# Mario5Gray/Stable-Diffusion-1.5-LCM-ONNX-RKNN2

Hardware: AMD Instinct MI355X
Metric: 512x512 4-step LCM images/sec (higher is better)
Workload: dtype f16; 1 GPU; SD1.5 LCM 512x512, 4 steps, guidance 1.0 (no CFG), batch 1 per GPU, fp16 (fp32 accumulate), hipGraph replay; seeded synthetic SD1.5-architecture weights; batch_per_gpu=1, global_batch=1, image=512x512, lcm_steps=4, parallelism=independent requests x1 (RCCL broadcast of prompt embeddings only)

## Files before the change

include/lcm_hip.h:

```cpp
#ifndef LCM_HIP_H
#define LCM_HIP_H
#include <stdint.h>
#ifdef __cplusplus
extern "C" {
#endif

#define LCM_OK 0
#define LCM_EINVAL (-1)
#define LCM_ENODEV (-2)
#define LCM_EUNSUPPORTED (-3)

#define LCM_EPI_NONE 0
#define LCM_EPI_GEGLU 1
#define LCM_EPI_QUICK_GELU 2
#define LCM_EPI_GELU 3

const char* lcm_last_error(void);
int lcm_version(void);
int lcm_device_info(int dev, char* arch_buf, int buf_len, int* cu_count, uint64_t* hbm_bytes);

int lcm_gemm_f16(const void* A, int lda, const void* A2, int lda2, int K1,
                 const void* W, const void* bias, const void* rowadd, int ld_rowadd, int rows_per_batch,
                 const void* res, int ldr, void* out, int ldo,
                 int M, int N, int K, int epilogue, float out_scale,
                 int batch, int64_t strideA, int64_t strideW, int64_t strideO, int img_rows,
                 void* stats_out, int64_t stats_bytes, int* slabs_per_image, void* stream);
int64_t lcm_stats_bytes(int M, int N, int img_rows);

int lcm_set_workspace(void* ptr, int64_t bytes);
int lcm_set_stream_workspace(void* stream, void* ptr, int64_t bytes);
int lcm_stream_create(void** stream_out);
int lcm_stream_destroy(void* stream);

int lcm_set_tuning(int target_wgs, int max_splits, int min_wgs);
int lcm_set_split_policy(int max_rows_per_image, int max_parts);
int lcm_set_seg_mode(int mode);

int lcm_plan_set(int kind, int M, int N, int K, int aux, int bm, int bn, int splits, int variant);
int lcm_plan_clear(void);
int lcm_canonical_splits(int kind, int m_img, int N, int K, int aux, int ph);

int lcm_gemm_ln_f16(const void* A, int lda, const void* W, const void* ln_g, const void* ln_c, float eps,
                    void* out, int ldo, int M, int N, int K, int epilogue, int img_rows, void* stream);

int lcm_mlp_geglu_f16(const void* x, int ldx, const void* W1, const void* ln_g, const void* ln_c, float eps,
                      const void* W2, const void* b2, void* out, int ldo, int M, int C, int img_rows, void* stream);
int lcm_ln_fold_refresh(const void* W, int N, int K, const void* c_base, const void* c_delta, float alpha,
                        void* g_out, void* c_out, void* stream);

int lcm_set_persist_n(int on);

int lcm_set_kernel_variant(int variant);

int lcm_gemm_tile_config(int M, int N, int batch);

int lcm_conv3x3_f16(const void* in, const void* W, const void* bias,
                    const void* rowadd, int ld_rowadd, const void* res, void* out,
                    int B, int Hin, int Win, int Cin, int Cout, int stride, int ups,
                    void* stats_out, int64_t stats_bytes, int* slabs_per_image, void* stream);

int lcm_conv3x3_down_f16(const void* in, const void* W, const void* bias, void* out, int B, int Hin, int Win, int Cin, int Cout,
                         void* stats_out, int64_t stats_bytes, int* slabs_per_image, void* stream);

int lcm_conv3x3_gn_f16(const void* in, int C1, const void* in2, int C2, const void* gn_scale, const void* gn_shift,
                       int silu, const void* W, const void* bias, const void* rowadd, int ld_rowadd, const void* res,
                       void* out, int B, int Hin, int Win, int Cout, int ups, void* stats_out, int64_t stats_bytes,
                       int* slabs_per_image, void* stream);
int lcm_groupnorm_affine_f16(const void* x, int C1, const void* x2, int C2, const void* gamma, const void* beta,
                             void* scale_out, void* shift_out, int B, int HW, int groups, float eps, void* ws,
                             void* stream);
int lcm_set_halo_pipe_threshold(int wgs);
int lcm_set_halo_prefetch(int on);
int lcm_set_staged_epilogue(int on);
int lcm_set_conv_impl(int impl);

int lcm_conv3x3_c4_f32in(const void* in, const void* pre_w, const void* pre_b, float in_scale,
                         const void* W, const void* bias, void* out, int B, int H, int Wd, int Cout, void* stream);

int lcm_conv3x3_c4_res_f32in(const void* in, const void* W, const void* bias, const void* res, void* out, int B, int H,
                             int Wd, int Cout, void* stream);

int lcm_hint_conv_u8(const void* in, const void* W, const void* bias, void* out, int B, int H, int Wd, int Cout, int silu,
                     void* stream);
int lcm_hint_conv_f16(const void* in, const void* W, const void* bias, void* out, int B, int H, int Wd, int Cin, int Cout,
                      int stride, int silu, void* stream);

int lcm_conv3x3_smalln(const void* in, const void* W, const void* bias, void* out, void* out_f32,
                       int B, int H, int Wd, int Cin, int Cout, int mode, void* stream);
int lcm_conv3x3_smalln_gn(const void* in, const void* gn_scale, const void* gn_shift, int silu, const void* W,
                          const void* bias, void* out, void* out_f32, int B, int H, int Wd, int Cin, int Cout,
                          int mode, void* stream);

int64_t lcm_groupnorm_ws_bytes(int B, int HW, int C, int groups);
int lcm_groupnorm_f16(const void* x, int C1, const void* x2, int C2, const void* gamma, const void* beta,
                      void* out, int B, int HW, int groups, float eps, int silu, void* ws, void* stream);

int lcm_set_gn_fused_bytes(int64_t bytes);
int lcm_groupnorm_from_stats_f16(const void* x, int C1, const void* x2, int C2, const void* stats1, int P1,
                                 const void* stats2, int P2, const void* gamma, const void* beta, void* out,
                                 int B, int HW, int groups, float eps, int silu, void* ws, void* stream);

int lcm_layernorm_f16(const void* x, const void* gamma, const void* beta, void* out, int M, int C, float eps,
                      void* stream);

int lcm_attention_f16(const void* Q, int ldq, const void* K, int ldk, const void* V, int ldv, void* out, int ldo,
                      int B, int heads, int Sq, int Sk, int d, float scale, int causal, void* stream);
int lcm_set_attention_waves(int waves);
int lcm_set_attention_impl(int impl);
int lcm_set_attention_ksplit(int on);

int lcm_embed_tokens_f16(const void* ids, const void* tok_emb, const void* pos_emb, void* out, int B, int S, int D,
                         int vocab, void* stream);

int lcm_softmax_rows_f16(void* x, int rows, int n, int ld, void* stream);
int lcm_transpose_f16(const void* in, int ldi, void* out, int ldo, int R, int C, int batch,
                      int64_t stride_in, int64_t stride_out, void* stream);

int lcm_linear_smallm_f16(const void* x, int ldx, const void* W, const void* bias, const void* res, int ldr,
                          void* out, int ldo, int M, int N, int K, int silu_in, int silu_out, void* stream);
int lcm_linear_rows_f16(const void* x, int ldx, int x_rows, const void* W, const void* bias, const void* res, int ldr,
                        int res_rows, void* out, int ldo, int M, int N, int K, int silu_in, int silu_out, void* stream);

int lcm_timestep_embedding(float t, void* out, int B, int dim, void* stream);
int lcm_timestep_embedding_steps(const float* t_host, int nsteps, void* out, int B, int dim, void* stream);

int lcm_scheduler_step(const void* eps, const void* eps_uncond, float guidance, void* lat, const void* noise,
                       const float* coef6, int last, int B, int h, int w, void* stream);
// ... 109 lines not shown
```

stable-diffusion-1.5-lcm-onnx-rknn2_amd/csrc/conv_halo.hip:

```cpp
#include "igemm_common.h"

struct HaloParams {
    IgemmParams g;
    int C1;
    const float* gn_scale;
    const float* gn_shift;
    int silu;
    int H, W;
    int tiles_y, tiles_x;
    int staged_epi;
};

static __device__ __attribute__((aligned(256))) half_t g_zero_page_h[128];

template <int TH, int TW, int PH>
__device__ __forceinline__ void halo_slabs(int (&slab_of)[TH * TW / 64], int wm, int bimg, int y0, int x0, int IH, int IW, int phase) {
    constexpr int RS = 32 / TW;
    const int sx = (IW + TW - 1) / TW, sy = (IH + RS - 1) / RS;
#pragma unroll
    for (int bp = 0; bp < TH * TW / 64; ++bp) {
        const int y = y0 + wm * (TH / 2) + bp * RS;
        const int idx = (bimg * sy + y / RS) * sx + x0 / TW;
        slab_of[bp] = y < IH ? (PH ? idx * 4 + phase : idx) : -1;
    }
// ... 133 lines not shown
            }
            {
                const half_t* wsrc = wptr + (long long)tap * p.Cin + cb;
#pragma unroll
                for (int i = 0; i < RW; ++i)
                    __builtin_amdgcn_global_load_lds((const __attribute__((address_space(1))) void*)(wsrc + (long long)(32 * i) * p.K),
                                                     (__attribute__((address_space(3))) void*)(wsm + (i * 32 + wave * 8) * 128),
                                                     16, 0, 0);
            }
            __syncthreads();

            const int dy = PH ? (tap >> 1) + py : tap / 3, dx = PH ? (tap & 1) + px : tap - (tap / 3) * 3;
            const int tapoff = dy * HWD + dx;
            const char* wsr = wsm + (wn * (BN / 2)) * 128;
#pragma unroll
            for (int kk = 0; kk < 2; ++kk) {
                h8 xf[TM], wf[TN];
                const int c = kk * 4 + fq;
#pragma unroll
                for (int b = 0; b < TM; ++b) {
                    const int r = rb0 + b * RB_STEP + tapoff;
                    xf[b] = *reinterpret_cast<const h8*>(xs + r * 128 + ((c ^ (r & 7)) << 4));
                }
#pragma unroll
                for (int a = 0; a < TN; ++a) {
                    const int r = a * 16 + frow;
                    wf[a] = *reinterpret_cast<const h8*>(wsr + r * 128 + ((c ^ (r & 7)) << 4));
                }
#pragma unroll
                for (int a = 0; a < TN; ++a)
#pragma unroll
                    for (int b = 0; b < TM; ++b)
                        acc[a][b] = __builtin_amdgcn_mfma_f32_16x16x32_f16(wf[a], xf[b], acc[a][b], 0, 0, 0);
            }
        }
    }

    int m_of[TM];
#pragma unroll
    for (int b = 0; b < TM; ++b) {
        const int q = (wm * TM + b) * 16 + frow;
        const int y = y0 + q / TW, x = x0 + q % TW;
        m_of[b] = (y < IH && x < IW) ? (PH ? (bimg * hp.H + 2 * y + py) * hp.W + 2 * x + px : (bimg * hp.H + y) * hp.W + x) : -1;
    }
    int slab_of[BM / 64];
    halo_slabs<TH, TW, PH>(slab_of, wm, bimg, y0, x0, IH, IW, phase);
    static_assert(XBYTES + BN * 128 >= BM * BN * 2, "the staged epilogue lays the output tile over the halo + weight buffers");
    if constexpr (EPI != 0) {
        tile_epilogue_staged<BM, BN>(p, acc, m_of, n_base, wm, wn, fq, slab_of, smem, [&](int q) {
            const int y = y0 + q / TW, x = x0 + q % TW;
            return (y < IH && x < IW) ? (PH ? (bimg * hp.H + 2 * y + py) * hp.W + 2 * x + px : (bimg * hp.H + y) * hp.W + x) : -1;
        });
    } else {
        igemm_epilogue<BM, BN>(p, acc, m_of, n_base + wn * (BN / 2), fq, 0, slab_of);
    }
}

template <int N>
__device__ __forceinline__ void halo_wait_vmcnt() {
    asm volatile("s_waitcnt vmcnt(%0)" ::"n"(N) : "memory");
}

template <int TH, int TW, int BN, int WS, int PH, int TPS, int SEG = 0, int EPI = 0>
__global__ __launch_bounds__(256, 2) void conv_halo_pipe_kernel(HaloParams hp) {
    constexpr int NT = PH ? 4 : 9;
    constexpr int G = NT / TPS;
    static_assert(TPS == 1 || TPS == (PH ? 2 : 3), "taps per step: 1 or one kernel row");
    constexpr int BM = TH * TW;
    constexpr int TM = BM / 32, TN = BN / 32, RW = BN / 32;
    constexpr int HWD = TW + 2, HROWS = (TH + 2) * HWD, HROWS_PAD = (HROWS + 7) / 8 * 8;
    constexpr int NV = (HROWS_PAD * 8 + 255) / 256;
    constexpr int XBYTES = HROWS_PAD * 128, WBYTES = BN * 128, SBYTES = TPS * WBYTES;
    extern __shared__ __attribute__((aligned(16))) char smem[];
    char* xs0 = smem;
    char* wsm0 = smem + 2 * XBYTES;

    const IgemmParams& p = hp.g;
    const int tid = threadIdx.x, lane = tid & 63;
    const int wave = __builtin_amdgcn_readfirstlane(tid >> 6);
    const int wm = wave & 1, wn = wave >> 1;
    const int tile = xcd_remap(blockIdx.x, p.mtiles * p.ntiles);
    const int mt4 = tile / p.ntiles, nt = tile - mt4 * p.ntiles;
    const int phase = PH ? (mt4 & 3) : 0, mt = PH ? (mt4 >> 2) : mt4;
    const int py = phase >> 1, px = phase & 1;
    const int IH = PH ? p.Hin : hp.H, IW = PH ? p.Win : hp.W;
    const int per_img = hp.tiles_y * hp.tiles_x;
    const int bimg = mt / per_img, tr = mt - bimg * per_img;
    const int ty = tr / hp.tiles_x, tx = tr - ty * hp.tiles_x;
    const int y0 = ty * TH, x0 = tx * TW;
    const int n_base = nt * BN;
    const int C2 = p.Cin - hp.C1;

    int h_pix[NV];
    const int pos = tid & 7;
#pragma unroll
    for (int i = 0; i < NV; ++i) {
        const int hr = (tid + 256 * i) >> 3;
        const int hy = hr / HWD, hx = hr - hy * HWD;
        int ly = y0 - 1 + hy, lx = x0 - 1 + hx;
        const bool ok = hr < HROWS && ly >= 0 && ly < IH && lx >= 0 && lx < IW;
        if (!PH && p.ups) { ly >>= 1; lx >>= 1; }
        h_pix[i] = ok ? (bimg * p.Hin + ly) * p.Win + lx : -1;
    }
    const int w_row0 = tid >> 3;
    const int w_schunk = (pos ^ (w_row0 & 7)) * 8;
    const half_t* wptr = p.W + (PH ? (long long)phase * p.N * p.K : 0ll) + (long long)(n_base + w_row0) * p.K + w_schunk;

    const int frow = lane & 15, fq = lane >> 4;
    const int q0 = wm * TM * 16 + frow;
    const int rb0 = (q0 / TW) * HWD + (q0 % TW);
    constexpr int RB_STEP = (16 / TW) * HWD;

    f4 acc[TN][TM];
#pragma unroll
    for (int a = 0; a < TN; ++a)
#pragma unroll
        for (int b = 0; b < TM; ++b) acc[a][b] = (f4){0.f, 0.f, 0.f, 0.f};

    const int nchunks = p.Cin >> 6;
    const int c_begin = (int)((long long)blockIdx.y * nchunks / p.splits);
    const int c_end = (int)((long long)(blockIdx.y + 1) * nchunks / p.splits);
    const int T = (c_end - c_begin) * G;

    auto issue_halo = [&](int c64, int hb) {
        const int cb = c64 << 6;
        const bool second = cb >= hp.C1;
        const half_t* src_base = second ? p.A2 : p.A;
        const int src_ld = second ? C2 : hp.C1;
        const int src_c = second ? cb - hp.C1 : cb;
        char* xs = xs0 + hb * XBYTES;
#pragma unroll
        for (int i = 0; i < NV; ++i) {
            if ((wave + 4 * i) * 64 < HROWS_PAD * 8) {
                const int hr = (tid + 256 * i) >> 3;
                const half_t* src = h_pix[i] >= 0
                    ? src_base + (long long)h_pix[i] * src_ld + src_c + ((pos ^ (hr & 7)) << 3)
                    : g_zero_page_h;
                __builtin_amdgcn_global_load_lds((const __attribute__((address_space(1))) void*)src,
                                                 (__attribute__((address_space(3))) void*)(xs + (wave + 4 * i) * 1024), 16, 0, 0);
            }
        }
    };
    auto issue_w = [&](int t, int wb) {
        const int c64 = c_begin + t / G, tg = t - (t / G) * G;
#pragma unroll
        for (int tp = 0; tp < TPS; ++tp) {
            const half_t* wsrc = wptr + (long long)(tg * TPS + tp) * p.Cin + (c64 << 6);
            char* wsm = wsm0 + wb * SBYTES + tp * WBYTES;
#pragma unroll
            for (int i = 0; i < RW; ++i)
                __builtin_amdgcn_global_load_lds((const __attribute__((address_space(1))) void*)(wsrc + (long long)(32 * i) * p.K),
                                                 (__attribute__((address_space(3))) void*)(wsm + (i * 32 + wave * 8) * 128), 16, 0, 0);
        }
    };

    if (T > 0) issue_halo(c_begin, 0);
#pragma unroll
    for (int s = 0; s < WS - 1; ++s)
        if (s < T) issue_w(s, s);

    f4 tot[SEG ? TN : 1][SEG ? TM : 1];
    int part = 0, kstep = 0, plen = T;
    if constexpr (SEG) {
#pragma unroll
        for (int a = 0; a < TN; ++a)
#pragma unroll
            for (int b = 0; b < TM; ++b) tot[a][b] = (f4){0.f, 0.f, 0.f, 0.f};
        plen = (int)((long long)nchunks / p.seg_parts) * G;
    }
    int wb = 0;
    constexpr int LPS = RW * TPS;
    for (int t = 0; t < T; ++t) {
        const int chunk = t / G, tg = t - chunk * G;
        const int newer = T - 1 - t;
// ... 47 lines not shown
                    const int r = a * 16 + frow;
                    wf[buf][a] = *reinterpret_cast<const h8*>(wsr + r * 128 + ((c ^ (r & 7)) << 4));
                }
            };
            load_half(0, 0);
#pragma unroll
            for (int h = 0; h < 2 * TPS; ++h) {
                if (h + 1 < 2 * TPS) load_half(h + 1, (h + 1) & 1);
                __builtin_amdgcn_sched_barrier(0);
#pragma unroll
                for (int a = 0; a < TN; ++a)
#pragma unroll
                    for (int b = 0; b < TM; ++b)
                        acc[a][b] = __builtin_amdgcn_mfma_f32_16x16x32_f16(wf[h & 1][a], xf[h & 1][b], acc[a][b], 0, 0, 0);
                __builtin_amdgcn_sched_barrier(0);
            }
        }
        wb = (wb + 1 == WS) ? 0 : wb + 1;
        if constexpr (SEG) {
            if (++kstep == plen) {
                kstep = 0;
#pragma unroll
                for (int a = 0; a < TN; ++a)
#pragma unroll
                    for (int b = 0; b < TM; ++b) {
                        tot[a][b][0] += acc[a][b][0]; tot[a][b][1] += acc[a][b][1];
                        tot[a][b][2] += acc[a][b][2]; tot[a][b][3] += acc[a][b][3];
                        acc[a][b] = (f4){0.f, 0.f, 0.f, 0.f};
                    }
                ++part;
                plen = ((int)((long long)(part + 1) * nchunks / p.seg_parts) - (int)((long long)part * nchunks / p.seg_parts)) * G;
            }
        }
    }

    int m_of[TM];
#pragma unroll
    for (int b = 0; b < TM; ++b) {
        const int q = (wm * TM + b) * 16 + frow;
        const int y = y0 + q / TW, x = x0 + q % TW;
        m_of[b] = (y < IH && x < IW) ? (PH ? (bimg * hp.H + 2 * y + py) * hp.W + 2 * x + px : (bimg * hp.H + y) * hp.W + x) : -1;
    }
    int slab_of[BM / 64];
    halo_slabs<TH, TW, PH>(slab_of, wm, bimg, y0, x0, IH, IW, phase);
    if constexpr (EPI != 0) {
        static_assert(2 * XBYTES + WS * SBYTES >= BM * BN * 2, "staged epilogue: the ring holds the tile");
        auto row_of = [&](int q) {
            const int y = y0 + q / TW, x = x0 + q % TW;
            return (y < IH && x < IW) ? (PH ? (bimg * hp.H + 2 * y + py) * hp.W + 2 * x + px : (bimg * hp.H + y) * hp.W + x) : -1;
        };
        if constexpr (SEG) tile_epilogue_staged<BM, BN>(p, tot, m_of, n_base, wm, wn, fq, slab_of, smem, row_of);
        else tile_epilogue_staged<BM, BN>(p, acc, m_of, n_base, wm, wn, fq, slab_of, smem, row_of);
    } else {
        if constexpr (SEG) igemm_epilogue<BM, BN>(p, tot, m_of, n_base + wn * (BN / 2), fq, 0, slab_of);
        else igemm_epilogue<BM, BN>(p, acc, m_of, n_base + wn * (BN / 2), fq, 0, slab_of);
    }
}

extern void lcm_launch_splitk_reduce(IgemmParams& p, hipStream_t s);
extern float* lcm_splitk_workspace(long long* bytes, hipStream_t s);
extern void lcm_tuning(int* target_wgs, int* max_splits, int* min_wgs);
extern int lcm_split_policy(int m_img, int sp);
extern bool lcm_plan_get(int kind, int M, int N, int K, int aux, int* bm, int* bn, int* splits, int* variant);

static int g_halo_pipe_below = 768;

extern "C" int lcm_set_halo_pipe_threshold(int wgs) { g_halo_pipe_below = wgs; return LCM_OK; }
static int g_halo_prefetch = 0;
extern "C" int lcm_set_halo_prefetch(int on) { g_halo_prefetch = on ? 1 : 0; return LCM_OK; }

template <int TH, int TW, int BN, int XFORM, int PH>
static void launch_halo(HaloParams& hp, hipStream_t s, int force) {
    constexpr int HROWS_PAD = ((TH + 2) * (TW + 2) + 7) / 8 * 8;
    hp.tiles_y = ((PH ? hp.g.Hin : hp.H) + TH - 1) / TH;
    hp.tiles_x = ((PH ? hp.g.Win : hp.W) + TW - 1) / TW;
    hp.g.ntiles = hp.g.N / BN;
    dim3 grid(hp.g.mtiles * hp.g.ntiles, hp.g.splits, 1);
    if constexpr (!XFORM) if (hp.g.seg_parts > 1) {
        constexpr int TPS = (BN <= 64) ? (PH ? 2 : 3) : 1;
        constexpr int WS = 3;
        constexpr int smem = 2 * HROWS_PAD * 128 + WS * TPS * BN * 128;
        static_assert(smem <= 160 * 1024, "halo ring exceeds LDS");
        static LcmDevOnce attr_once;
        if (auto once_guard = attr_once.first()) {
            once_guard.check(hipFuncSetAttribute(reinterpret_cast<const void*>(&conv_halo_pipe_kernel<TH, TW, BN, WS, PH, TPS, 1>),
                                      hipFuncAttributeMaxDynamicSharedMemorySize, smem));
        }
        char nm[80];
        if (hp.staged_epi && hp.g.res && hp.g.splits == 1) {
            static LcmDevOnce attr_once_e;
            if (auto once_guard = attr_once_e.first()) {
                once_guard.check(hipFuncSetAttribute(reinterpret_cast<const void*>(&conv_halo_pipe_kernel<TH, TW, BN, WS, PH, TPS, 1, 1>),
                                          hipFuncAttributeMaxDynamicSharedMemorySize, smem));
            }
            snprintf(nm, sizeof(nm), "conv_halo_pipe_kernel<%d, %d, %d, %d, %d, %d, 1, 1>", TH, TW, BN, WS, PH, TPS);
            lcm_prof_start(nm, s);
            hipLaunchKernelGGL((conv_halo_pipe_kernel<TH, TW, BN, WS, PH, TPS, 1, 1>), grid, dim3(256), smem, s, hp);
            lcm_prof_stop(s);
            return;
        }
        snprintf(nm, sizeof(nm), "conv_halo_pipe_kernel<%d, %d, %d, %d, %d, %d, 1>", TH, TW, BN, WS, PH, TPS);
        lcm_prof_start(nm, s);
        hipLaunchKernelGGL((conv_halo_pipe_kernel<TH, TW, BN, WS, PH, TPS, 1>), grid, dim3(256), smem, s, hp);
        lcm_prof_stop(s);
        return;
    }
    if constexpr (!XFORM && BN <= 128) if (force == 3) {
        constexpr int TPS = PH ? 2 : 3;
// ... 38 lines not shown
    }
    const bool staged = hp.staged_epi && hp.g.splits == 1 && hp.g.res != nullptr;
    snprintf(nm, sizeof(nm), "conv_halo_kernel<%d, %d, %d, %d, %d, 0, %d>%s", TH, TW, BN, XFORM, PH, staged ? 1 : 0, hp.g.splits > 1 ? " +splitk" : "");
    lcm_prof_start(nm, s);
    if (staged) hipLaunchKernelGGL((conv_halo_kernel<TH, TW, BN, XFORM, PH, 0, 1>), grid, dim3(256), smem, s, hp);
    else hipLaunchKernelGGL((conv_halo_kernel<TH, TW, BN, XFORM, PH>), grid, dim3(256), smem, s, hp);
    lcm_prof_stop(s);
}

struct HaloPick { int bm, bn, splits; };
static HaloPick halo_pick(int B, int IH, int IW, int PHM, int TW, long long M, int N, int nchunks, int fixed_splits) {
    int target, max_splits, min_wgs;
    lcm_tuning(&target, &max_splits, &min_wgs);
    const int cand[4][2] = {{128, 128}, {128, 64}, {64, 128}, {64, 64}};
    HaloPick best = {0, 0, fixed_splits > 0 ? fixed_splits : 1};
    long long best_wgs = -1;
    for (int c = 0; c < 4; ++c) {
        const int cbm = cand[c][0], cbn = cand[c][1];
        if (N % cbn) continue;
        if (TW == 8 && cbm == 128) continue;
        const int th = cbm / TW;
        const long long mt = (long long)B * ((IH + th - 1) / th) * ((IW + TW - 1) / TW) * PHM;
        if ((long long)mt * cbm > 2ll * M && cbm == 128) continue;
        const long long tiles = mt * (N / cbn);
        int sp = fixed_splits > 0 ? fixed_splits : 1;
        if (fixed_splits < 0 && tiles < min_wgs && nchunks >= 2) {
            sp = (int)((target + tiles - 1) / tiles);
            if (sp > nchunks) sp = nchunks;
            if (sp > max_splits) sp = max_splits;
        }
        const long long wgs = tiles * sp;
        if (wgs >= min_wgs) return {cbm, cbn, sp};
        if (wgs > best_wgs) { best_wgs = wgs; best = {cbm, cbn, sp}; }
    }
    return best;
}

static inline int halo_tw(int IW) { return (IW % 16 == 0 || IW > 16) ? 16 : 8; }

int lcm_canonical_splits_halo(int m_img, int N, int K, int IH, int IW, int W, int ph, int xform) {
    const int nchunks = (K / (ph ? 4 : 9)) >> 6;
    int pbm, pbn, psp, pv;
    (void)xform;
    int sp = lcm_plan_get(2, m_img, N, K, W << 1, &pbm, &pbn, &psp, &pv)
                 ? psp : halo_pick(1, IH, IW, ph ? 4 : 1, halo_tw(IW), m_img, N, nchunks, -1).splits;
    if (sp > nchunks) sp = nchunks;
    return lcm_split_policy(m_img, sp);
}

static int g_staged_epi = 1;
extern int g_staged_epi_gemm;
extern "C" int lcm_set_staged_epilogue(int on) { g_staged_epi = (on & 1) ? 1 : 0; g_staged_epi_gemm = (on & 2) ? 1 : 0; return LCM_OK; }

int lcm_conv_halo_launch(HaloParams& hp, int B, hipStream_t s, int* slabs_per_image) {
    IgemmParams& p = hp.g;
    hp.staged_epi = g_staged_epi;
    const bool ph = p.ups == 2;
    const int IH = ph ? p.Hin : hp.H, IW = ph ? p.Win : hp.W, PHM = ph ? 4 : 1;
    const int TW = halo_tw(IW);
    long long ws_bytes = 0;
    p.ws = lcm_splitk_workspace(&ws_bytes, s);
    const int nchunks = p.Cin >> 6;
    const int m_img = p.M / B;
    p.img_rows = m_img;
    const int splits = p.ws ? lcm_canonical_splits_halo(m_img, p.N, p.K, IH, IW, hp.W, ph ? 1 : 0, hp.gn_scale ? 1 : 0) : 1;
    HaloPick hk = halo_pick(B, IH, IW, PHM, TW, p.M, p.N, nchunks, splits);
    int bm = hk.bm, bn = hk.bn, force = 0;
    {
        int pbm, pbn, psp, pv;
        if (lcm_plan_get(2, p.M, p.N, p.K, (hp.W << 1) | (hp.gn_scale ? 1 : 0), &pbm, &pbn, &psp, &pv) && p.N % pbn == 0 &&
            !(TW == 8 && pbm == 128)) {
            bm = pbm; bn = pbn;
            force = (pv >= 1 && pv <= 3) ? pv : 0;
        }
    }
    if (!bm) return 1;
    const int th = bm / TW;
    p.mtiles = B * ((IH + th - 1) / th) * ((IW + TW - 1) / TW) * PHM;
    p.splits = splits;
    p.seg_parts = 1;
    if (splits > 1 && !hp.gn_scale) {
        extern int g_seg_mode;
        int tgt, mxs, min_wgs;
        lcm_tuning(&tgt, &mxs, &min_wgs);
        if (g_seg_mode == 1 || (g_seg_mode == 0 && (long long)p.mtiles * (p.N / bn) >= min_wgs)) { p.seg_parts = splits; p.splits = 1; }
    }
    if (p.splits > 1 && (long long)p.splits * p.M * p.N * 4 > ws_bytes) {
        lcm_set_error("split-K workspace too small: %d x %d x %d fp32 slabs need %lld MB, have %lld MB "
                      "(lcm_set_workspace / LCM_SPLITK_WS_MB)", p.splits, p.M, p.N,
                      ((long long)p.splits * p.M * p.N * 4 + (1 << 20) - 1) >> 20, ws_bytes >> 20);
        return LCM_EINVAL;
    }
    p.rg_kind = TW == 16 ? 1 : 2; p.rg_ph = ph ? 1 : 0; p.rg_IH = IH; p.rg_IW = IW; p.rg_OH = hp.H; p.rg_OW = hp.W;
    if (p.stats) {
        if (p.N > 2048) p.stats = nullptr;
        else {
            if (slabs_per_image) *slabs_per_image = halo_slabs_per_image(IH, IW, TW, ph);
            LCM_STATS_FIT(p, halo_slabs_per_image(IH, IW, TW, ph), B, "conv3x3");
        }
    }
    const bool xf = hp.gn_scale != nullptr;
    if (ph && xf) return 1;
#define HALO_CASE(TH_, TW_, BN_)                                                           \
    if (th == TH_ && TW == TW_ && bn == BN_) {                                             \
        if (ph) launch_halo<TH_, TW_, BN_, 0, 1>(hp, s, force);                            \
        else if (xf) launch_halo<TH_, TW_, BN_, 1, 0>(hp, s, force);                       \
        else launch_halo<TH_, TW_, BN_, 0, 0>(hp, s, force);                               \
    } else
    HALO_CASE(8, 16, 128) HALO_CASE(8, 16, 64) HALO_CASE(4, 16, 128) HALO_CASE(4, 16, 64)
    HALO_CASE(8, 8, 128) HALO_CASE(8, 8, 64) HALO_CASE(8, 16, 160) HALO_CASE(4, 16, 160) HALO_CASE(8, 8, 160) { return 1; }
#undef HALO_CASE
    if (p.splits > 1) lcm_launch_splitk_reduce(p, s);
    return 0;
}
```

stable-diffusion-1.5-lcm-onnx-rknn2_amd/csrc/igemm.hip:

```cpp
#include "igemm_common.h"

template <int BM, int BN, int MODE, int LN = 0>
__global__ __launch_bounds__(256, 2) void igemm_kernel(IgemmParams p) {
    constexpr int RA = BM / 32, RW = BN / 32;
    constexpr int TM = BM / 32, TN = BN / 32;
    constexpr int XBYTES = BM * 128, WBYTES = BN * 128, BUF = XBYTES + WBYTES;
    extern __shared__ __attribute__((aligned(16))) char smem[];

    const int tid = threadIdx.x, lane = tid & 63, wave = tid >> 6;
    const int wm = wave & 1, wn = wave >> 1;
    const int tile = xcd_remap(blockIdx.x, p.mtiles * p.ntiles);
    const int mt = tile / p.ntiles, nt = tile - mt * p.ntiles;
    const int m_base = mt * BM, n_base = nt * BN;
    const int z = blockIdx.z;

    const half_t* __restrict__ Ab = p.A + z * p.strideA;
    const half_t* __restrict__ A2b = p.A2 ? p.A2 + z * p.strideA : nullptr;
    const half_t* __restrict__ Wb = p.W + z * p.strideW;

    const int chunk = tid & 7, row0 = tid >> 3;
    const int swz = (chunk ^ (row0 & 7)) << 4;

    bool a_ok[RA];
    long long a_off[RA];
// ... 75 lines not shown
    for (int b = 0; b < TM; ++b) { ln_s[b] = 0.f; ln_q[b] = 0.f; }

    load_tile(kt0);
    store_tile(0);
    __syncthreads();

    for (int kt = kt0; kt < kt1; ++kt) {
        const int cur = (kt - kt0) & 1;
        if (kt + 1 < kt1) load_tile(kt + 1);
        const char* xs = smem + cur * BUF + (wm * (BM / 2)) * 128;
        const char* ws = smem + cur * BUF + XBYTES + (wn * (BN / 2)) * 128;
#pragma unroll
        for (int kk = 0; kk < 2; ++kk) {
            h8 xf[TM], wf[TN];
            const int c = kk * 4 + fq;
#pragma unroll
            for (int b = 0; b < TM; ++b) {
                const int r = b * 16 + frow;
                xf[b] = *reinterpret_cast<const h8*>(xs + r * 128 + ((c ^ (r & 7)) << 4));
            }
#pragma unroll
            for (int a = 0; a < TN; ++a) {
                const int r = a * 16 + frow;
                wf[a] = *reinterpret_cast<const h8*>(ws + r * 128 + ((c ^ (r & 7)) << 4));
            }
            if constexpr (ln) {
#pragma unroll
                for (int b = 0; b < TM; ++b) ln_accum(xf[b], ln_s[b], ln_q[b]);
            }
#pragma unroll
            for (int a = 0; a < TN; ++a)
#pragma unroll
                for (int b = 0; b < TM; ++b)
                    acc[a][b] = __builtin_amdgcn_mfma_f32_16x16x32_f16(wf[a], xf[b], acc[a][b], 0, 0, 0);
        }
        if (kt + 1 < kt1) store_tile(cur ^ 1);
        __syncthreads();
    }

    int m_of[TM];
#pragma unroll
    for (int b = 0; b < TM; ++b) {
        const int m = m_base + wm * (BM / 2) + b * 16 + frow;
        m_of[b] = m < p.M ? m : -1;
    }
    int slab_of[BM / 64];
#pragma unroll
    for (int bp = 0; bp < BM / 64; ++bp) {
        const int r = m_base + wm * (BM / 2) + bp * 32;
        slab_of[bp] = r < p.M ? (r >> 5) : -1;
    }
    if constexpr (ln) {
        ln_finish<TM>(ln_s, ln_q, p.K, p.ln_eps);
        igemm_epilogue<BM, BN>(p, acc, m_of, n_base + wn * (BN / 2), fq, z, slab_of, ln_s, ln_q);
    } else {
        igemm_epilogue<BM, BN>(p, acc, m_of, n_base + wn * (BN / 2), fq, z, slab_of);
    }
}

__device__ __attribute__((aligned(256))) half_t g_zero_page[128];

template <int N>
__device__ __forceinline__ void wait_vmcnt() {
    asm volatile("s_waitcnt vmcnt(%0)" ::"n"(N) : "memory");
}

template <int BM, int BN, int MODE, int S, int LN = 0, int SEG = 0, int EPI = 0>
__global__ __launch_bounds__(256, S == 1 ? (BM + BN < 256 ? 4 : 3) : 2) void igemm2_kernel(IgemmParams p) {
    static_assert(!EPI || (MODE == 0 && !LN && !SEG && S * (BM + BN) * 128 >= BM * BN * 2), "staged epilogue: plain GEMM whose ring holds the tile");
    static_assert(!SEG || (S >= 2 && !LN), "segmented accumulation: ring variants of the plain kernel");
    constexpr int RA = BM / 32, RW = BN / 32;
    constexpr int TM = BM / 32, TN = BN / 32;
    constexpr int XBYTES = BM * 128, WBYTES = BN * 128, BUF = XBYTES + WBYTES;
    constexpr int LPT = RA + RW;
    extern __shared__ __attribute__((aligned(16))) char smem[];

    const int tid = threadIdx.x, lane = tid & 63;
    const int wave = __builtin_amdgcn_readfirstlane(tid >> 6);
    const int wm = wave & 1, wn = wave >> 1;
    const int ngroups = p.ntiles / p.n_iters;
    const int tile = xcd_remap(blockIdx.x, p.mtiles * ngroups);
    const int mt = tile / ngroups, nt0 = (tile - mt * ngroups) * p.n_iters;
    const int m_base = mt * BM;
    const int z = blockIdx.z;

    const half_t* __restrict__ Ab = p.A + z * p.strideA;
    const half_t* __restrict__ A2b = p.A2 ? p.A2 + z * p.strideA : nullptr;
    const half_t* __restrict__ Wb = p.W + z * p.strideW;

    const int pos = tid & 7, row0 = tid >> 3;
    const int schunk = (pos ^ (row0 & 7)) * 8;

    bool a_ok[RA];
    long long a_off[RA];
    int a_b[RA], a_y[RA], a_x[RA];
#pragma unroll
    for (int i = 0; i < RA; ++i) {
        const int m = m_base + row0 + 32 * i;
        a_ok[i] = m < p.M;
        if (MODE == 0) {
            a_off[i] = (long long)m;
        } else {
            const int hw = p.Hout * p.Wout;
            const int b = m / hw, rem = m - b * hw;
            const int oy = rem / p.Wout;
            a_b[i] = b; a_y[i] = oy * p.stride - 1; a_x[i] = (rem - oy * p.Wout) * p.stride - 1;
        }
    }
    const half_t* wptr = Wb + (long long)row0 * p.K + schunk;
    const int nk_all = p.K >> 6;
    const int kt0 = (int)((long long)blockIdx.y * nk_all / p.splits);
    const int kt1 = (int)((long long)(blockIdx.y + 1) * nk_all / p.splits);
    const int nkr = kt1 - kt0;
    const int T = nkr * p.n_iters;

    auto issue_tile = [&](int t, int buf) {
        const int ni = t / nkr;
        const int kt = kt0 + (t - ni * nkr);
        const int n_base_i = (nt0 + ni) * BN;
        char* xs = smem + buf * BUF + wave * 8 * 128;
        char* ws = xs + XBYTES;
        if (MODE == 0) {
            const int k0 = kt << 6;
            const bool second = (A2b != nullptr) && (k0 >= p.K1);
            const half_t* base = second ? A2b : Ab;
            const long long ld = second ? p.lda2 : p.lda;
            const int kk = (second ? k0 - p.K1 : k0) + schunk;
#pragma unroll
            for (int i = 0; i < RA; ++i) {
                const half_t* src = a_ok[i] ? base + a_off[i] * ld + kk : g_zero_page;
                __builtin_amdgcn_global_load_lds((const __attribute__((address_space(1))) void*)src,
                                                 (__attribute__((address_space(3))) void*)(xs + i * 32 * 128), 16, 0, 0);
            }
        } else {
            const int cpt = p.Cin >> 6;
            const int tap = kt / cpt;
            const int c0 = ((kt - tap * cpt) << 6) + schunk;
            const int dy = tap / 3, dx = tap - dy * 3;
            const int Hl = p.ups ? p.Hin * 2 : p.Hin, Wl = p.ups ? p.Win * 2 : p.Win;
#pragma unroll
            for (int i = 0; i < RA; ++i) {
                int iy = a_y[i] + dy, ix = a_x[i] + dx;
                const bool ok = a_ok[i] && iy >= 0 && iy < Hl && ix >= 0 && ix < Wl;
                if (p.ups) { iy >>= 1; ix >>= 1; }
                const long long off = ((long long)(a_b[i] * p.Hin + iy) * p.Win + ix) * p.Cin + c0;
                const half_t* src = ok ? Ab + off : g_zero_page;
                __builtin_amdgcn_global_load_lds((const __attribute__((address_space(1))) void*)src,
                                                 (__attribute__((address_space(3))) void*)(xs + i * 32 * 128), 16, 0, 0);
            }
        }
#pragma unroll
        for (int i = 0; i < RW; ++i) {
            const half_t* src = wptr + (long long)(n_base_i + 32 * i) * p.K + (kt << 6);
            __builtin_amdgcn_global_load_lds((const __attribute__((address_space(1))) void*)src,
                                             (__attribute__((address_space(3))) void*)(ws + i * 32 * 128), 16, 0, 0);
        }
    };

    f4 acc[TN][TM];
#pragma unroll
    for (int a = 0; a < TN; ++a)
#pragma unroll
        for (int b = 0; b < TM; ++b) acc[a][b] = (f4){0.f, 0.f, 0.f, 0.f};

    const int frow = lane & 15, fq = lane >> 4;
    constexpr bool ln = LN != 0;
    float ln_s[TM], ln_q[TM];
#pragma unroll
    for (int b = 0; b < TM; ++b) { ln_s[b] = 0.f; ln_q[b] = 0.f; }

#pragma unroll
    for (int s = 0; s < S - 1; ++s)
        if (s < T) issue_tile(s, s);
    const __attribute__((address_space(3))) float* ln_lds = nullptr;
    if constexpr (ln) {
        float* t = reinterpret_cast<float*>(smem + S * BUF);
        if (tid < BN) { t[tid] = p.ln_g[nt0 * BN + tid]; t[BN + tid] = p.ln_c[nt0 * BN + tid]; }
        __syncthreads();
        ln_lds = (const __attribute__((address_space(3))) float*)t;
    }

    f4 tot[SEG ? TN : 1][SEG ? TM : 1];
    int part = 0, nkp = nkr;
    if constexpr (SEG) {
#pragma unroll
        for (int a = 0; a < TN; ++a)
#pragma unroll
            for (int b = 0; b < TM; ++b) tot[a][b] = (f4){0.f, 0.f, 0.f, 0.f};
        nkp = (int)((long long)nk_all / p.seg_parts);
    }
    int buf = 0, kstep = 0, ni_cur = 0;
    for (int t = 0; t < T; ++t) {
        const int newer = T - 1 - t;
        if (S == 1) {
            if (t > 0) __builtin_amdgcn_s_barrier();
            issue_tile(t, 0);
            wait_vmcnt<0>();
            __builtin_amdgcn_s_barrier();
        } else {
            if (S >= 6 && newer >= 4) wait_vmcnt<(S >= 6 ? 4 : 0) * LPT>();
            else if (S >= 5 && newer >= 3) wait_vmcnt<(S >= 5 ? 3 : 0) * LPT>();
            else if (S >= 4 && newer >= 2) wait_vmcnt<(S >= 4 ? 2 : 0) * LPT>();
            else if (S >= 3 && newer >= 1) wait_vmcnt<(S >= 3 ? 1 : 0) * LPT>();
            else wait_vmcnt<0>();
            __builtin_amdgcn_s_barrier();
            if (t + S - 1 < T) issue_tile(t + S - 1, (buf + S - 1) % S);
        }

        const char* xs = smem + buf * BUF + (wm * (BM / 2)) * 128;
        const char* ws = smem + buf * BUF + XBYTES + (wn * (BN / 2)) * 128;
#pragma unroll
        for (int kk = 0; kk < 2; ++kk) {
            h8 xf[TM], wf[TN];
            const int c = kk * 4 + fq;
#pragma unroll
            for (int b = 0; b < TM; ++b) {
                const int r = b * 16 + frow;
                xf[b] = *reinterpret_cast<const h8*>(xs + r * 128 + ((c ^ (r & 7)) << 4));
            }
#pragma unroll
            for (int a = 0; a < TN; ++a) {
                const int r = a * 16 + frow;
                wf[a] = *reinterpret_cast<const h8*>(ws + r * 128 + ((c ^ (r & 7)) << 4));
            }
            if constexpr (ln) {
#pragma unroll
                for (int b = 0; b < TM; ++b) ln_accum(xf[b], ln_s[b], ln_q[b]);
            }
#pragma unroll
            for (int a = 0; a < TN; ++a)
#pragma unroll
                for (int b = 0; b < TM; ++b)
                    acc[a][b] = __builtin_amdgcn_mfma_f32_16x16x32_f16(wf[a], xf[b], acc[a][b], 0, 0, 0);
        }
        buf = (buf + 1 == S) ? 0 : buf + 1;
        if constexpr (SEG) {
            if (++kstep == nkp) {
                kstep = 0;
#pragma unroll
                for (int a = 0; a < TN; ++a)
#pragma unroll
                    for (int b = 0; b < TM; ++b) {
                        tot[a][b][0] += acc[a][b][0]; tot[a][b][1] += acc[a][b][1];
                        tot[a][b][2] += acc[a][b][2]; tot[a][b][3] += acc[a][b][3];
                        acc[a][b] = (f4){0.f, 0.f, 0.f, 0.f};
                    }
                ++part;
                nkp = (int)((long long)(part + 1) * nk_all / p.seg_parts) - (int)((long long)part * nk_all / p.seg_parts);
            }
            continue;
        }
        if (++kstep == nkr) {
            kstep = 0;
            int m_of[TM];
#pragma unroll
            for (int b = 0; b < TM; ++b) {
                const int m = m_base + wm * (BM / 2) + b * 16 + frow;
                m_of[b] = m < p.M ? m : -1;
            }
            int slab_of[BM / 64];
#pragma unroll
            for (int bp = 0; bp < BM / 64; ++bp) {
                const int r = m_base + wm * (BM / 2) + bp * 32;
                slab_of[bp] = r < p.M ? (r >> 5) : -1;
            }
            if constexpr (ln) {
                ln_finish<TM>(ln_s, ln_q, p.K, p.ln_eps);
                igemm_epilogue<BM, BN, 0, (S >= 3)>(p, acc, m_of, (nt0 + ni_cur) * BN + wn * (BN / 2), fq, z, slab_of, ln_s, ln_q, ln_lds, nt0 * BN);
            } else if constexpr (EPI != 0) {
                tile_epilogue_staged<BM, BN>(p, acc, m_of, (nt0 + ni_cur) * BN, wm, wn, fq, slab_of, smem,
                                             [&](int q) { return m_base + q < p.M ? m_base + q : -1; });
            } else {
                igemm_epilogue<BM, BN, 0, (S >= 3)>(p, acc, m_of, (nt0 + ni_cur) * BN + wn * (BN / 2), fq, z, slab_of);
            }
            ++ni_cur;
#pragma unroll
            for (int a = 0; a < TN; ++a)
#pragma unroll
                for (int b = 0; b < TM; ++b) acc[a][b] = (f4){0.f, 0.f, 0.f, 0.f};
        }
    }
    if constexpr (SEG) {
        int m_of[TM];
#pragma unroll
        for (int b = 0; b < TM; ++b) {
            const int m = m_base + wm * (BM / 2) + b * 16 + frow;
            m_of[b] = m < p.M ? m : -1;
        }
        int slab_of[BM / 64];
#pragma unroll
        for (int bp = 0; bp < BM / 64; ++bp) {
            const int r = m_base + wm * (BM / 2) + bp * 32;
            slab_of[bp] = r < p.M ? (r >> 5) : -1;
        }
        igemm_epilogue<BM, BN, 0, (S >= 3)>(p, tot, m_of, nt0 * BN + wn * (BN / 2), fq, z, slab_of);
    }
}

__device__ __forceinline__ int reduce_pixel(const IgemmParams& p, int slab, int b, int l) {
    if (p.rg_kind == 0) {
        const int m = slab * 32 + b * 16 + l;
        return m < p.M ? m : -1;
    }
    const int TW = p.rg_kind == 1 ? 16 : 8, RS = 32 / TW;
    const int sx = (p.rg_IW + TW - 1) / TW, sy = (p.rg_IH + RS - 1) / RS;
    int phase = 0;
    if (p.rg_ph) { phase = slab & 3; slab >>= 2; }
    const int bimg = slab / (sy * sx), r = slab - bimg * (sy * sx);
    const int syi = r / sx, sxi = r - syi * sx;
    const int q = b * 16 + l;
    const int y = syi * RS + q / TW, x = sxi * TW + q % TW;
    if (y >= p.rg_IH || x >= p.rg_IW) return -1;
    if (p.rg_ph) return (bimg * p.rg_OH + 2 * y + (phase >> 1)) * p.rg_OW + 2 * x + (phase & 1);
    return (bimg * p.rg_OH + y) * p.rg_OW + x;
}

#define RED_BATCH 8
__global__ __launch_bounds__(256) void splitk_reduce_kernel(IgemmParams p, int total_slabs) {
#pragma clang fp contract(off)
    const int lane = threadIdx.x & 63, ncg = p.N >> 4;
    const long long wv = (long long)blockIdx.x * 4 + (threadIdx.x >> 6);
    const int slab = (int)(wv / ncg), cg = (int)(wv - (long long)slab * ncg);
    if (slab >= total_slabs) return;
    const int l = lane & 15, fq = lane >> 4;
    const int n = cg * 16 + fq * 4;
    const long long slab_stride = (long long)p.M * p.N;
    const int splits = p.splits;
    int m[2];
    bool live[2];
    const float* src[2];
#pragma unroll
    for (int b = 0; b < 2; ++b) {
        const int mm = reduce_pixel(p, slab, b, l);
        live[b] = mm >= 0;
        m[b] = live[b] ? mm : 0;
        src[b] = p.ws + (long long)m[b] * p.N + n;
    }
    f4 t[2][RED_BATCH];
#pragma unroll
    for (int b = 0; b < 2; ++b)
#pragma unroll
        for (int k = 0; k < RED_BATCH; ++k)
            if (k < splits) t[b][k] = *reinterpret_cast<const f4*>(src[b] + k * slab_stride);
    h4 hb = {}, ha[2] = {}, hr[2] = {};
    if (p.bias) hb = *reinterpret_cast<const h4*>(p.bias + n);
    if (p.rowadd) {
#pragma unroll
        for (int b = 0; b < 2; ++b) ha[b] = *reinterpret_cast<const h4*>(p.rowadd + (long long)(m[b] / p.rows_per_batch) * p.ld_rowadd + n);
    }
    if (p.res) {
#pragma unroll
        for (int b = 0; b < 2; ++b) hr[b] = *reinterpret_cast<const h4*>(p.res + (long long)m[b] * p.ldr + n);
    }
    f4 v[2];
    for (int s0 = 0;;) {
#pragma unroll
        for (int b = 0; b < 2; ++b)
#pragma unroll
            for (int k = 0; k < RED_BATCH; ++k) {
                if (s0 + k >= splits) continue;
                if (k == 0 && s0 == 0) { v[b] = t[b][0]; continue; }
                v[b][0] += t[b][k][0]; v[b][1] += t[b][k][1]; v[b][2] += t[b][k][2]; v[b][3] += t[b][k][3];
            }
        s0 += RED_BATCH;
        if (s0 >= splits) break;
#pragma unroll
        for (int b = 0; b < 2; ++b)
#pragma unroll
            for (int k = 0; k < RED_BATCH; ++k)
                if (s0 + k < splits) t[b][k] = *reinterpret_cast<const f4*>(src[b] + (s0 + k) * slab_stride);
    }
    const f4 bias4 = {(float)hb[0], (float)hb[1], (float)hb[2], (float)hb[3]};
    float ssum[4] = {0.f, 0.f, 0.f, 0.f}, ssq[4] = {0.f, 0.f, 0.f, 0.f};
#pragma unroll
    for (int b = 0; b < 2; ++b) {
        f4 w = v[b];
        w[0] += bias4[0]; w[1] += bias4[1]; w[2] += bias4[2]; w[3] += bias4[3];
        if (p.rowadd) { w[0] += (float)ha[b][0]; w[1] += (float)ha[b][1]; w[2] += (float)ha[b][2]; w[3] += (float)ha[b][3]; }
        w[0] *= p.out_scale; w[1] *= p.out_scale; w[2] *= p.out_scale; w[3] *= p.out_scale;
        if (p.res) { w[0] += (float)hr[b][0]; w[1] += (float)hr[b][1]; w[2] += (float)hr[b][2]; w[3] += (float)hr[b][3]; }
        h4 o = {(half_t)w[0], (half_t)w[1], (half_t)w[2], (half_t)w[3]};
        if (live[b]) {
            *reinterpret_cast<h4*>(p.out + (long long)m[b] * p.ldo + n) = o;
#pragma unroll
            for (int j = 0; j < 4; ++j) { const float f = (float)o[j]; ssum[j] += f; ssq[j] += f * f; }
        }
    }
    if (p.stats) {
row16_sum8(ssum, ssq);
        if (l == 0) {
            float* dst = p.stats + ((long long)slab * p.N + n) * 2;
            *reinterpret_cast<f4*>(dst) = (f4){ssum[0], ssq[0], ssum[1], ssq[1]};
            *reinterpret_cast<f4*>(dst + 4) = (f4){ssum[2], ssq[2], ssum[3], ssq[3]};
        }
    }
}

#include <map>
#include <mutex>
static float* g_ws[16] = {};
static long long g_ws_bytes[16] = {};
struct StreamWs { float* ptr; long long bytes; };
static std::map<hipStream_t, StreamWs> g_stream_ws;
static std::mutex g_ws_mu;

extern "C" int lcm_set_workspace(void* ptr, int64_t bytes) {
    int dev = 0;
    if (hipGetDevice(&dev) != hipSuccess || dev < 0 || dev >= 16) { lcm_set_error("set_workspace: no device"); return LCM_ENODEV; }
    std::lock_guard<std::mutex> lk(g_ws_mu);
    g_ws[dev] = (float*)ptr;
    g_ws_bytes[dev] = ptr ? bytes : 0;
    return LCM_OK;
}

extern "C" int lcm_set_stream_workspace(void* stream, void* ptr, int64_t bytes) {
    std::lock_guard<std::mutex> lk(g_ws_mu);
    auto it = g_stream_ws.find((hipStream_t)stream);
    if (ptr && bytes > 0) {
        if (it != g_stream_ws.end() && it->second.ptr != (float*)ptr) {
            lcm_set_error("set_stream_workspace: stream %p already carries the workspace %p of another owner (new %p): "
                          "every lane needs a stream of its own", stream, (void*)it->second.ptr, ptr);
            return LCM_EINVAL;
        }
        g_stream_ws[(hipStream_t)stream] = StreamWs{(float*)ptr, (long long)bytes};
    } else if (it != g_stream_ws.end() && (!ptr || it->second.ptr == (float*)ptr)) {
        g_stream_ws.erase(it);
    }
    return LCM_OK;
}

float* lcm_splitk_workspace(long long* bytes, hipStream_t s) {
    std::lock_guard<std::mutex> lk(g_ws_mu);
    auto it = g_stream_ws.find(s);
    if (it != g_stream_ws.end()) { *bytes = it->second.bytes; return it->second.ptr; }
    int dev = 0;
    (void)hipGetDevice(&dev);
    if (dev < 0 || dev >= 16) { *bytes = 0; return nullptr; }
    *bytes = g_ws[dev] ? g_ws_bytes[dev] : 0;
    return g_ws[dev];
}
int lcm_total_slabs(const IgemmParams& p) {
    if (p.rg_kind == 0) return (p.M + 31) / 32;
    const int TW = p.rg_kind == 1 ? 16 : 8, RS = 32 / TW;
    const int per_img = ((p.rg_IH + RS - 1) / RS) * ((p.rg_IW + TW - 1) / TW) * (p.rg_ph ? 4 : 1);
    return (p.M / (p.rg_OH * p.rg_OW)) * per_img;
}

void lcm_launch_splitk_reduce(IgemmParams& p, hipStream_t s) {
    const int total = lcm_total_slabs(p);
    const long long waves = (long long)total * (p.N >> 4);
    hipLaunchKernelGGL(splitk_reduce_kernel, dim3((unsigned)((waves + 3) / 4)), dim3(256), 0, s, p, total);
}

#include <tuple>
struct PlanVal { int bm, bn, splits, variant; };
static std::map<std::tuple<int, int, int, int, int>, PlanVal> g_plans;
static std::mutex g_plans_mu;

extern "C" int lcm_plan_set(int kind, int M, int N, int K, int aux, int bm, int bn, int splits, int variant) {
    if (!((bm == 128 || bm == 64) && (bn == 128 || bn == 64 || bn == 160) && splits >= 1 && splits <= 64 && variant >= -1 && variant <= 4)) {
        lcm_set_error("plan_set: bad plan %dx%d splits %d variant %d", bm, bn, splits, variant);
        return LCM_EINVAL;
    }
    std::lock_guard<std::mutex> lk(g_plans_mu);
    g_plans[std::make_tuple(kind, M, N, K, aux)] = PlanVal{bm, bn, splits, variant};
    return LCM_OK;
}

extern "C" int lcm_plan_clear(void) {
    std::lock_guard<std::mutex> lk(g_plans_mu);
    g_plans.clear();
    return LCM_OK;
}

bool lcm_plan_get(int kind, int M, int N, int K, int aux, int* bm, int* bn, int* splits, int* variant) {
    std::lock_guard<std::mutex> lk(g_plans_mu);
    auto it = g_plans.find(std::make_tuple(kind, M, N, K, aux));
    if (it == g_plans.end()) return false;
    *bm = it->second.bm; *bn = it->second.bn; *splits = it->second.splits; *variant = it->second.variant;
    return true;
}

struct TilePick { int bm, bn, splits; };
static int g_target_wgs = 384, g_max_splits = 16, g_min_wgs = 256;
static int g_split_max_rows = 4096, g_split_cap = 8;
int g_seg_mode = 0;
static int g_variant = -1;

void lcm_tuning(int* target_wgs, int* max_splits, int* min_wgs) {
    *target_wgs = g_target_wgs; *max_splits = g_max_splits; *min_wgs = g_min_wgs;
}

static int g_conv_impl = 1;

extern "C" int lcm_set_conv_impl(int impl) {
    if (impl != 0 && impl != 1) { lcm_set_error("conv_impl: %d", impl); return LCM_EINVAL; }
    g_conv_impl = impl;
    return LCM_OK;
}

extern "C" int lcm_set_kernel_variant(int variant) {
    if (variant < -1 || variant > 6) { lcm_set_error("kernel_variant: %d", variant); return LCM_EINVAL; }
    g_variant = variant;
    return LCM_OK;
// ... 120 lines not shown
        int ni = p.ntiles;
        while (ni > 1 && (p.ntiles % ni != 0 || (long long)p.mtiles * (p.ntiles / ni) < 384)) --ni;
        p.n_iters = ni;
    }
    dim3 grid(p.mtiles * (p.ntiles / p.n_iters), splits, batch);
    if (variant == 5) variant = (BM + BN <= 128) ? 4 : -1;
    if (variant == 6) variant = (BM + BN <= 128) ? 6 : -1;
    if (variant < 0) {
        const long long wgs = (long long)grid.x * grid.y * grid.z;
        variant = (wgs >= 1024 && p.n_iters == 1) ? 1 : ((BM + BN <= 128) ? 4 : 2);
    }
    if (p.n_iters > 1 && variant == 1) variant = 2;
    if (variant == 4 && BM + BN > 192) variant = 3;
    if constexpr (!LN) if (p.seg_parts > 1) {
        if (variant < 2 || variant > 4) variant = (BM + BN <= 128) ? 4 : 2;
        if (variant == 2) launch_v2<BM, BN, MODE, 2, 0, 1>(p, grid, s);
        else if (variant == 3) launch_v2<BM, BN, MODE, 3, 0, 1>(p, grid, s);
        else if constexpr (BM + BN <= 192) launch_v2<BM, BN, MODE, 4, 0, 1>(p, grid, s);
        else launch_v2<BM, BN, MODE, 3, 0, 1>(p, grid, s);
        LCM_CHECK_LAUNCH("igemm");
        return LCM_OK;
    }
    if (variant == 0) {
        const int smem = 2 * (BM + BN) * 128;
        static LcmDevOnce attr_once;
        if (auto once_guard = attr_once.first()) {
            once_guard.check(hipFuncSetAttribute(reinterpret_cast<const void*>(&igemm_kernel<BM, BN, MODE, LN>),
                                      hipFuncAttributeMaxDynamicSharedMemorySize, smem));
        }
        char nm[64];
        snprintf(nm, sizeof(nm), "igemm_kernel<%d, %d, %d, %d>%s", BM, BN, MODE, LN, p.splits > 1 ? " +splitk" : "");
        lcm_prof_start(nm, s);
        hipLaunchKernelGGL((igemm_kernel<BM, BN, MODE, LN>), grid, dim3(256), smem, s, p);
        lcm_prof_stop(s);
    } else if (variant == 1) {
        launch_v2<BM, BN, MODE, 1, LN>(p, grid, s);
    } else if (variant == 2) {
        launch_v2<BM, BN, MODE, 2, LN>(p, grid, s);
    } else if (variant == 3) {
        launch_v2<BM, BN, MODE, 3, LN>(p, grid, s);
    } else if (variant == 6) {
        if constexpr (BM + BN <= 128) launch_v2<BM, BN, MODE, 6, LN>(p, grid, s);
    } else {
        launch_v2<BM, BN, MODE, 4, LN>(p, grid, s);
    }
    LCM_CHECK_LAUNCH("igemm");
    if (splits > 1) {
        lcm_launch_splitk_reduce(p, s);
        LCM_CHECK_LAUNCH("splitk_reduce");
    }
    return LCM_OK;
}

template <int MODE>
static int launch_igemm(IgemmParams& p, int batch, hipStream_t s, int img_rows, bool allow_split, bool want_stats,
                        int* slabs_per_image) {
    long long wsb = 0;
    p.ws = lcm_splitk_workspace(&wsb, s);
    if (img_rows <= 0 || p.M % img_rows) img_rows = p.M;
    p.img_rows = img_rows;
    int splits = 1;
    if (allow_split && p.ws && p.epi == 0 && batch == 1) {
        splits = canonical_splits_gemm(MODE, img_rows, p.N, p.K);
    }
    TilePick t = pick_tile(p.M, p.N, p.K, batch, splits);
    int variant = -1, pbm, pbn, psp, pv;
    if (lcm_plan_get(MODE, p.M, p.N, p.K, batch, &pbm, &pbn, &psp, &pv) && p.N % pbn == 0 &&
        !(pbn == 160 && (MODE != 0 || p.epi == 1)) && !(pbm == 128 && p.M < 128)) {
        t.bm = pbm; t.bn = pbn;
        variant = pv;
    }
    if (slabs_per_image) *slabs_per_image = 0;
    p.stats = want_stats ? p.stats : nullptr;
    p.rg_kind = 0;
    if (p.stats) {
        const bool ok = p.epi == 0 && batch == 1 && p.N <= 2048 && img_rows % 32 == 0;
        if (ok && slabs_per_image) *slabs_per_image = img_rows / 32;
        if (!ok) p.stats = nullptr;
        else LCM_STATS_FIT(p, img_rows / 32, p.M / img_rows, "gemm");
    }
    p.seg_parts = 1;
    if (splits > 1) {
        const long long tiles = (long long)((p.M + t.bm - 1) / t.bm) * (p.N / t.bn) * batch;
        if (g_seg_mode == 1 || (g_seg_mode == 0 && tiles >= g_min_wgs)) { p.seg_parts = splits; splits = 1; }
    }
    if (splits > 1 && (long long)splits * p.M * p.N * 4 > wsb) {
        lcm_set_error("split-K workspace too small: %d x %d x %d fp32 slabs need %lld MB, have %lld MB "
                      "(lcm_set_workspace / LCM_SPLITK_WS_MB)", splits, p.M, p.N,
                      ((long long)splits * p.M * p.N * 4 + (1 << 20) - 1) >> 20, wsb >> 20);
        return LCM_EINVAL;
    }
    const int code = t.bm * 1000 + t.bn;
    if constexpr (MODE == 0) if (p.ln_g) {
        switch (code) {
            case 128128: return launch_cfg<128, 128, 0, 1>(p, batch, splits, variant, s);
            case 128064: return launch_cfg<128, 64, 0, 1>(p, batch, splits, variant, s);
            case 64128: return launch_cfg<64, 128, 0, 1>(p, batch, splits, variant, s);
            case 128160: return launch_cfg<128, 160, 0, 1>(p, batch, splits, variant, s);
            case 64160: return launch_cfg<64, 160, 0, 1>(p, batch, splits, variant, s);
            default: return launch_cfg<64, 64, 0, 1>(p, batch, splits, variant, s);
        }
    }
    switch (code) {
        case 128128: return launch_cfg<128, 128, MODE>(p, batch, splits, variant, s);
        case 128064: return launch_cfg<128, 64, MODE>(p, batch, splits, variant, s);
        case 64128: return launch_cfg<64, 128, MODE>(p, batch, splits, variant, s);
        case 128160: if constexpr (MODE == 0) return launch_cfg<128, 160, MODE>(p, batch, splits, variant, s);
        case 64160: if constexpr (MODE == 0) return launch_cfg<64, 160, MODE>(p, batch, splits, variant, s);
        default: return launch_cfg<64, 64, MODE>(p, batch, splits, variant, s);
    }
}

extern "C" int lcm_gemm_f16(const void* A, int lda, const void* A2, int lda2, int K1,
                            const void* W, const void* bias, const void* rowadd, int ld_rowadd, int rows_per_batch,
                            const void* res, int ldr, void* out, int ldo,
                            int M, int N, int K, int epilogue, float out_scale,
                            int batch, int64_t strideA, int64_t strideW, int64_t strideO, int img_rows,
                            void* stats_out, int64_t stats_bytes, int* slabs_per_image, void* stream) {
    LCM_REQUIRE(A && W && out, "gemm: null pointer");
    LCM_REQUIRE(M > 0 && N > 0 && K > 0 && batch > 0, "gemm: bad shape M=%d N=%d K=%d batch=%d", M, N, K, batch);
    LCM_REQUIRE(K % 64 == 0, "gemm: K=%d must be a multiple of 64", K);
    LCM_REQUIRE(N % 64 == 0, "gemm: N=%d must be a multiple of 64", N);
    LCM_REQUIRE(lda % 8 == 0 && ldo % 4 == 0, "gemm: lda=%d (%%8) / ldo=%d (%%4) misaligned", lda, ldo);
    if (A2) LCM_REQUIRE(K1 > 0 && K1 < K && K1 % 64 == 0 && lda2 % 8 == 0, "gemm: bad split K1=%d lda2=%d", K1, lda2);
    if (res) LCM_REQUIRE(ldr % 4 == 0, "gemm: ldr=%d misaligned", ldr);
    if (rowadd) LCM_REQUIRE(rows_per_batch > 0 && ld_rowadd % 4 == 0, "gemm: bad rowadd");
    LCM_REQUIRE(epilogue >= 0 && epilogue <= 3, "gemm: unknown epilogue %d", epilogue);
    if (epilogue == 1) LCM_REQUIRE(!rowadd && !res && !A2, "gemm: GEGLU epilogue takes bias only");
    IgemmParams p = {};
    p.A = (const half_t*)A; p.A2 = (const half_t*)A2; p.W = (const half_t*)W;
    p.bias = (const half_t*)bias; p.rowadd = (const half_t*)rowadd; p.res = (const half_t*)res;
    p.out = (half_t*)out;
    p.M = M; p.N = N; p.K = K; p.lda = lda; p.lda2 = lda2; p.K1 = A2 ? K1 : K;
    p.ldo = ldo; p.ldr = ldr; p.ld_rowadd = ld_rowadd; p.rows_per_batch = rows_per_batch > 0 ? rows_per_batch : 1;
    p.epi = epilogue; p.out_scale = out_scale;
    p.strideA = strideA; p.strideW = strideW; p.strideO = strideO;
    p.stats = (float*)stats_out; p.stats_cap = stats_bytes;
    LCM_REQUIRE(!stats_out || slabs_per_image, "gemm: stats_out needs slabs_per_image");
    const bool allow_split = batch == 1 && strideA == 0 && strideW == 0 && strideO == 0;
    return launch_igemm<0>(p, batch, (hipStream_t)stream, img_rows, allow_split, stats_out != nullptr, slabs_per_image);
}

extern "C" int lcm_gemm_ln_f16(const void* A, int lda, const void* W, const void* ln_g, const void* ln_c, float eps,
                               void* out, int ldo, int M, int N, int K, int epilogue, int img_rows, void* stream) {
    LCM_REQUIRE(A && W && out && ln_g && ln_c, "gemm_ln: null pointer");
    LCM_REQUIRE(M > 0 && N > 0 && K > 0, "gemm_ln: bad shape M=%d N=%d K=%d", M, N, K);
    LCM_REQUIRE(K % 64 == 0 && N % 64 == 0, "gemm_ln: N=%d K=%d must be multiples of 64", N, K);
    LCM_REQUIRE(lda % 8 == 0 && ldo % 4 == 0, "gemm_ln: lda=%d (%%8) / ldo=%d (%%4) misaligned", lda, ldo);
    LCM_REQUIRE(epilogue == 0 || epilogue == 1, "gemm_ln: epilogue %d (0 = none, 1 = GEGLU)", epilogue);
    IgemmParams p = {};
    p.A = (const half_t*)A; p.W = (const half_t*)W; p.out = (half_t*)out;
    p.M = M; p.N = N; p.K = K; p.lda = lda; p.K1 = K; p.ldo = ldo; p.rows_per_batch = 1;
    p.epi = epilogue; p.out_scale = 1.0f;
    p.ln_g = (const float*)ln_g; p.ln_c = (const float*)ln_c; p.ln_eps = eps;
    return launch_igemm<0>(p, 1, (hipStream_t)stream, img_rows, false, false, nullptr);
}

extern "C" int64_t lcm_stats_bytes(int M, int N, int img_rows) {
    if (M <= 0 || N <= 0) return 0;
    if (img_rows <= 0 || M % img_rows) img_rows = M;
    const long long per_img = (img_rows / 16 > 256 ? img_rows / 16 : 256) + 64;
    return (int64_t)(per_img * (M / img_rows) * N * 2 * (long long)sizeof(float));
}

struct HaloParams {
    IgemmParams g;
    int C1;
    const float* gn_scale;
    const float* gn_shift;
    int silu;
    int H, W;
    int tiles_y, tiles_x;
    int staged_epi;
};
int lcm_conv_halo_launch(HaloParams& hp, int B, hipStream_t s, int* slabs_per_image);

extern "C" int lcm_conv3x3_gn_f16(const void* in, int C1, const void* in2, int C2, const void* gn_scale,
                                  const void* gn_shift, int silu, const void* W, const void* bias, const void* rowadd,
                                  int ld_rowadd, const void* res, void* out, int B, int Hin, int Win, int Cout, int ups,
                                  void* stats_out, int64_t stats_bytes, int* slabs_per_image, void* stream) {
    LCM_REQUIRE(in && W && out, "conv3x3_gn: null pointer");
    if (!in2) C2 = 0;
    const int Cin = C1 + C2;
    LCM_REQUIRE(B > 0 && Hin > 0 && Win > 0, "conv3x3_gn: bad shape");
    LCM_REQUIRE(C1 % 64 == 0 && C2 % 64 == 0 && Cout % 64 == 0, "conv3x3_gn: C1=%d C2=%d Cout=%d must be multiples of 64", C1, C2, Cout);
    LCM_REQUIRE((gn_scale == nullptr) == (gn_shift == nullptr), "conv3x3_gn: scale/shift must come together");
    if (rowadd) LCM_REQUIRE(ld_rowadd % 4 == 0, "conv3x3_gn: ld_rowadd misaligned");
    HaloParams hp = {};
    IgemmParams& p = hp.g;
    p.A = (const half_t*)in; p.A2 = (const half_t*)in2; p.W = (const half_t*)W; p.bias = (const half_t*)bias;
    p.rowadd = (const half_t*)rowadd; p.res = (const half_t*)res; p.out = (half_t*)out;
    const int crop_h = (ups >> 2) & 1, crop_w = (ups >> 3) & 1;
    ups &= 3;
    LCM_REQUIRE(ups >= 0 && ups <= 2 && !(ups == 2 && gn_scale), "conv3x3_gn: ups=%d (2 = phase-packed weights, no fused GroupNorm)", ups);
    LCM_REQUIRE(ups == 1 || (!crop_h && !crop_w), "conv3x3_gn: an odd output size needs ups=1 (plain 3x3 weights), got ups=%d", ups);
    p.Hin = Hin; p.Win = Win; p.Cin = Cin; p.stride = 1; p.ups = ups;
    hp.H = ups ? 2 * Hin - crop_h : Hin; hp.W = ups ? 2 * Win - crop_w : Win;
    p.Hout = hp.H; p.Wout = hp.W;
    p.M = B * hp.H * hp.W; p.N = Cout; p.K = (ups == 2 ? 4 : 9) * Cin;
    p.ldo = Cout; p.ldr = Cout; p.ld_rowadd = ld_rowadd; p.rows_per_batch = hp.H * hp.W;
    p.epi = 0; p.out_scale = 1.0f; p.splits = 1;
    hp.C1 = C1; hp.gn_scale = (const float*)gn_scale; hp.gn_shift = (const float*)gn_shift; hp.silu = silu;
    p.stats = (float*)stats_out; p.stats_cap = stats_bytes;
    LCM_REQUIRE(!stats_out || slabs_per_image, "conv3x3_gn: stats_out needs slabs_per_image");
    if (slabs_per_image) *slabs_per_image = 0;
    const int hrc = lcm_conv_halo_launch(hp, B, (hipStream_t)stream, slabs_per_image);
    if (hrc < 0) return hrc;
    if (hrc != 0) {
        lcm_set_error("conv3x3_gn: no tile configuration for B=%d %dx%d Cin=%d Cout=%d", B, hp.H, hp.W, Cin, Cout);
        return LCM_EINVAL;
    }
    LCM_CHECK_LAUNCH("conv_halo");
    return LCM_OK;
}

extern "C" int lcm_conv3x3_f16(const void* in, const void* W, const void* bias,
                               const void* rowadd, int ld_rowadd, const void* res, void* out,
                               int B, int Hin, int Win, int Cin, int Cout, int stride, int ups,
                               void* stats_out, int64_t stats_bytes, int* slabs_per_image, void* stream) {
    LCM_REQUIRE(in && W && out, "conv3x3: null pointer");
    LCM_REQUIRE(B > 0 && Hin > 0 && Win > 0, "conv3x3: bad shape");
    LCM_REQUIRE(Cin % 64 == 0 && Cout % 64 == 0, "conv3x3: Cin=%d Cout=%d must be multiples of 64", Cin, Cout);
    LCM_REQUIRE(stride == 1 || stride == 2, "conv3x3: stride %d", stride);
    LCM_REQUIRE(!(ups && stride != 1), "conv3x3: upsample needs stride 1");
    if (rowadd) LCM_REQUIRE(ld_rowadd % 4 == 0, "conv3x3: ld_rowadd misaligned");
    if (stride == 1 && (g_conv_impl == 1 || (ups & 3) == 2 || (ups & 12)))
        return lcm_conv3x3_gn_f16(in, Cin, nullptr, 0, nullptr, nullptr, 0, W, bias, rowadd, ld_rowadd, res, out, B, Hin, Win,
                                  Cout, ups, stats_out, stats_bytes, slabs_per_image, stream);
    const int Hl = ups ? 2 * Hin : Hin, Wl = ups ? 2 * Win : Win;
    IgemmParams p = {};
    p.A = (const half_t*)in; p.W = (const half_t*)W; p.bias = (const half_t*)bias;
    p.rowadd = (const half_t*)rowadd; p.res = (const half_t*)res; p.out = (half_t*)out;
    p.Hin = Hin; p.Win = Win; p.Cin = Cin; p.stride = stride; p.ups = ups;
    p.Hout = (Hl + 2 - 3) / stride + 1; p.Wout = (Wl + 2 - 3) / stride + 1;
    p.M = B * p.Hout * p.Wout; p.N = Cout; p.K = 9 * Cin;
    p.ldo = Cout; p.ldr = Cout; p.ld_rowadd = ld_rowadd; p.rows_per_batch = p.Hout * p.Wout;
    p.epi = 0; p.out_scale = 1.0f;
    p.stats = (float*)stats_out; p.stats_cap = stats_bytes;
    LCM_REQUIRE(!stats_out || slabs_per_image, "conv3x3: stats_out needs slabs_per_image");
    return launch_igemm<1>(p, 1, (hipStream_t)stream, p.Hout * p.Wout, true, stats_out != nullptr, slabs_per_image);
}
```

stable-diffusion-1.5-lcm-onnx-rknn2_amd/csrc/igemm_common.h:

```cpp
#pragma once
#include "common.h"

struct IgemmParams {
    const half_t* A;
    const half_t* A2;
    const half_t* W;
    const half_t* bias;
    const half_t* rowadd;
    const half_t* res;
    half_t* out;
    int M, N, K;
    int lda, lda2, K1;
    int ldo, ldr, ld_rowadd, rows_per_batch;
    int epi;
    float out_scale;
    long long strideA, strideW, strideO;
    int Hin, Win, Cin, Hout, Wout, stride, ups;
    int mtiles, ntiles;
    int splits;
    float* ws;
    float* stats;
    int reduce_rows;
    int rg_kind, rg_ph, rg_IH, rg_IW, rg_OH, rg_OW;
    int seg_parts;
// ... 14 lines not shown
            return LCM_EINVAL;                                                                                             \
        }                                                                                                                  \
    } while (0)

__device__ __forceinline__ int xcd_remap(int bid, int nwg) {
    const int q = nwg >> 3, r = nwg & 7, xcd = bid & 7;
    return (xcd < r ? xcd * (q + 1) : r * (q + 1) + (xcd - r) * q) + (bid >> 3);
}

__device__ __forceinline__ void ln_accum(const h8& x, float& s, float& q) {
    const h2 one = {(half_t)1.0f, (half_t)1.0f};
#pragma unroll
    for (int i = 0; i < 4; ++i) {
        const h2 pr = {x[2 * i], x[2 * i + 1]};
        s = __builtin_amdgcn_fdot2(pr, one, s, false);
        q = __builtin_amdgcn_fdot2(pr, pr, q, false);
    }
}
template <int TM>
__device__ __forceinline__ void ln_finish(float (&s)[TM], float (&q)[TM], int K, float eps) {
    const float inv = 1.0f / (float)K;
#pragma unroll
    for (int b = 0; b < TM; ++b) {
        float ss = s[b], qq = q[b];
        ss += __shfl_xor(ss, 16, 64); qq += __shfl_xor(qq, 16, 64);
        ss += __shfl_xor(ss, 32, 64); qq += __shfl_xor(qq, 32, 64);
        const float mean = ss * inv;
        s[b] = mean;
        q[b] = rsqrtf(fmaxf(__builtin_fmaf(-mean, mean, qq * inv), 0.f) + eps);
    }
}

__device__ __forceinline__ h4 geglu_ln_quad(f4 x, f4 g, float ln_r, float ln_mu, const f4& gx, const f4& cx, const f4& gg, const f4& cg) {
#pragma clang fp contract(off)
    h4 o;
#pragma unroll
    for (int j = 0; j < 4; ++j) {
        const float xv = __builtin_fmaf(ln_r, __builtin_fmaf(-ln_mu, gx[j], x[j]), cx[j]);
        const float gv = __builtin_fmaf(ln_r, __builtin_fmaf(-ln_mu, gg[j], g[j]), cg[j]);
        o[j] = (half_t)(xv * gelu_erf_f(gv));
    }
    return o;
}

__device__ __forceinline__ int geglu_store_col(int P, int fq) { return 32 * (P >> 1) + 8 * fq + 4 * (P & 1); }

template <int CH>
__device__ __forceinline__ int stage_pos(int c, int q) { return (c + q) % CH; }
template <int CH>
__device__ __forceinline__ int stage_src(int cpos, int q) { return (cpos + CH - q % CH) % CH; }

template <int BM, int BN, int STAGED = 0, int BATCHED = 0>
__device__ __forceinline__ void igemm_epilogue(const IgemmParams& p, f4 (&acc)[BN / 32][BM / 32], const int (&m_of)[BM / 32],
                                               int n_wave, int fq, int z, const int (&slab_of)[BM / 64],
                                               const float* ln_mu = nullptr, const float* ln_r = nullptr,
                                               const __attribute__((address_space(3))) float* ln_lds = nullptr, int n_tile0 = 0,
                                               char* stage = nullptr, int q_wave = 0, int nl_wave = 0) {
#pragma clang fp contract(off)
    constexpr int TM = BM / 32, TN = BN / 32;
    if (p.splits > 1) {
        float* __restrict__ wsb = p.ws + (long long)blockIdx.y * p.M * p.N;
#pragma unroll
        for (int b = 0; b < TM; ++b) {
            const int m = m_of[b];
            if (m < 0) continue;
#pragma unroll
            for (int a = 0; a < TN; ++a) {
                const int n = n_wave + a * 16 + fq * 4;
                *reinterpret_cast<f4*>(wsb + (long long)m * p.N + n) = acc[a][b];
            }
        }
        return;
    }

    half_t* __restrict__ outb = p.out + z * p.strideO;
    const bool do_stats = p.stats != nullptr && p.epi == 0;
    const int lane = threadIdx.x & 63;
    if (p.epi != 1) {
        constexpr bool PRE = BATCHED != 0 && STAGED == 0;
        constexpr int NB = PRE ? (TM * TN <= 4 ? TN : 1) : 1;
        h4 pre_bias[NB], pre_add[NB][PRE ? TM : 1], pre_res[NB][PRE ? TM : 1];
        int mc[TM];
#pragma unroll
        for (int b = 0; b < TM; ++b) mc[b] = m_of[b] < 0 ? 0 : m_of[b];
#pragma unroll
        for (int a = 0; a < TN; ++a) {
            const int n = n_wave + a * 16 + fq * 4;
            if constexpr (PRE) {
                if (a % NB == 0) {
                    if (p.bias) {
#pragma unroll
                        for (int i = 0; i < NB; ++i) pre_bias[i] = *reinterpret_cast<const h4*>(p.bias + n + i * 16);
                    }
                    if (p.rowadd) {
#pragma unroll
                        for (int b = 0; b < TM; ++b) {
                            const half_t* row = p.rowadd + (long long)(mc[b] / p.rows_per_batch) * p.ld_rowadd + n;
#pragma unroll
                            for (int i = 0; i < NB; ++i) pre_add[i][b] = *reinterpret_cast<const h4*>(row + i * 16);
                        }
                    }
                    if (p.res) {
#pragma unroll
                        for (int b = 0; b < TM; ++b) {
                            const half_t* row = p.res + (long long)mc[b] * p.ldr + n;
#pragma unroll
                            for (int i = 0; i < NB; ++i) pre_res[i][b] = *reinterpret_cast<const h4*>(row + i * 16);
                        }
                    }
                }
            }
            f4 bias4 = {0.f, 0.f, 0.f, 0.f};
            if (p.bias) {
                h4 t;
// ... 79 lines not shown
            if (ln_mu) {
                if (ln_lds) {
                    const __attribute__((address_space(3))) float* gl = ln_lds + (n - n_tile0);
                    gx = *reinterpret_cast<const __attribute__((address_space(3))) f4*>(gl);
                    cx = *reinterpret_cast<const __attribute__((address_space(3))) f4*>(gl + BN);
                    gg = *reinterpret_cast<const __attribute__((address_space(3))) f4*>(gl + 16);
                    cg = *reinterpret_cast<const __attribute__((address_space(3))) f4*>(gl + BN + 16);
                } else {
                    gx = *reinterpret_cast<const f4*>(p.ln_g + n); cx = *reinterpret_cast<const f4*>(p.ln_c + n);
                    gg = *reinterpret_cast<const f4*>(p.ln_g + n + 16); cg = *reinterpret_cast<const f4*>(p.ln_c + n + 16);
                }
            }
#pragma unroll
            for (int b = 0; b < TM; ++b) {
                const int m = m_of[b];
                if (m < 0) continue;
                h4 o;
                if (ln_mu) {
                    o = geglu_ln_quad(acc[a][b], acc[a + 1][b], ln_r[b], ln_mu[b], gx, cx, gg, cg);
                } else {
                    const f4 x = acc[a][b], g = acc[a + 1][b];
#pragma unroll
                    for (int j = 0; j < 4; ++j) o[j] = (half_t)((x[j] + bx[j]) * gelu_erf_f(g[j] + bg[j]));
                }
                *reinterpret_cast<h4*>(outb + (long long)m * p.ldo + nout) = o;
            }
        }
    }
}

static __device__ __attribute__((aligned(256))) half_t g_zero_page_epi[128];

template <int BM, int BN, class RowOf>
__device__ __forceinline__ void tile_epilogue_staged(const IgemmParams& p, f4 (&acc)[BN / 32][BM / 32], const int (&m_of)[BM / 32],
                                                     int n_base, int wm, int wn, int fq, const int (&slab_of)[BM / 64],
                                                     char* stage, RowOf row_of) {
    constexpr int CH = BN / 8, PIECES = BM * CH, NV = (PIECES + 255) / 256;
    const int tid = threadIdx.x;
    const int wave = __builtin_amdgcn_readfirstlane(tid >> 6);
    __syncthreads();
    if (p.res) {
#pragma unroll
        for (int i = 0; i < NV; ++i) {
            if ((wave + 4 * i) * 64 < PIECES) {
                const int v = tid + 256 * i, q = v / CH, cpos = v - q * CH;
                const int m = row_of(q);
                const half_t* src = m >= 0 ? p.res + (long long)m * p.ldr + n_base + stage_src<CH>(cpos, q) * 8 : g_zero_page_epi;
                __builtin_amdgcn_global_load_lds((const __attribute__((address_space(1))) void*)src,
                                                 (__attribute__((address_space(3))) void*)(stage + (wave + 4 * i) * 1024), 16, 0, 0);
            }
        }
        __syncthreads();
    }
    igemm_epilogue<BM, BN, 1>(p, acc, m_of, n_base + wn * (BN / 2), fq, 0, slab_of, nullptr, nullptr, nullptr, 0,
                              stage, wm * (BM / 2), wn * (BN / 2));
    __syncthreads();
#pragma unroll
    for (int i = 0; i < NV; ++i) {
        const int v = tid + 256 * i;
        if (v < PIECES) {
            const int q = v / CH, cpos = v - q * CH;
            const int m = row_of(q);
            if (m >= 0) *reinterpret_cast<h8*>(p.out + (long long)m * p.ldo + n_base + stage_src<CH>(cpos, q) * 8) =
                            *reinterpret_cast<const h8*>(stage + v * 16);
        }
    }
}
```

stable-diffusion-1.5-lcm-onnx-rknn2_amd/csrc/mlp_fused.hip:

```cpp
#include "igemm_common.h"
#include <stdlib.h>

struct MlpParams {
    IgemmParams g;
    const half_t* X;
    int ldx;
    const half_t* W1;
    const float* ln_g;
    const float* ln_c;
    float eps;
    const half_t* W2;
};

template <int N>
__device__ __forceinline__ void mlp_wait_vmcnt() {
    asm volatile("s_waitcnt vmcnt(%0)" ::"n"(N) : "memory");
}

template <int C, int ABL = 0>
__global__ __launch_bounds__(512, 2) void mlp_geglu_kernel(MlpParams p) {
    static_assert(C % 64 == 0 && C <= 320, "register budget: C/16 accumulator tiles + C/32 x 2 operand fragments per lane");
    constexpr int KT1 = C / 64;
    constexpr int F = 4 * C;
    constexpr int NCH = F / 64;
// ... 141 lines not shown
            const f4 gg = *reinterpret_cast<const __attribute__((address_space(3))) f4*>(ln_lds + n + 16);
            const f4 cg = *reinterpret_cast<const __attribute__((address_space(3))) f4*>(ln_lds + 8 * C + n + 16);
#pragma unroll
            for (int b = 0; b < 2; ++b) {
                h4 o;
                if (ABL == 1) { for (int e = 0; e < 4; ++e) o[e] = (half_t)(acc1[2 * qq][b][e] * acc1[2 * qq + 1][b][e] + gx[e] + cg[e]); }
                else o = geglu_ln_quad(acc1[2 * qq][b], acc1[2 * qq + 1][b], ln_r[b], ln_mu[b], gx, cx, gg, cg);
#pragma unroll
                for (int e = 0; e < 4; ++e) gf[b][4 * qq + e] = o[e];
            }
        }
        *reinterpret_cast<h8*>(gmine) = gf[0];
        *reinterpret_cast<h8*>(gmine + 1024) = gf[1];
        __builtin_amdgcn_sched_barrier(0);
#pragma unroll
        for (int i = 0; i < 4; ++i) cur[i] = frag(w2s, i, 0);
        if (last) mlp_wait_vmcnt<0>(); else mlp_wait_vmcnt<3 * LPT1>();
        asm volatile("s_waitcnt lgkmcnt(0)" ::: "memory");
        __builtin_amdgcn_s_barrier();
        __builtin_amdgcn_sched_barrier(0);
        {
            const h8 q0 = *reinterpret_cast<const h8*>(gcell), q1 = *reinterpret_cast<const h8*>(gcell + 1024);
            const h8 r0 = *reinterpret_cast<const h8*>(gcell + 2048), r1 = *reinterpret_cast<const h8*>(gcell + 3072);
            h8 wv[2 * TN2 + 4];
#pragma unroll
            for (int i = 0; i < 4; ++i) wv[i] = cur[i];
#pragma unroll
            for (int i = 4; i < 2 * TN2; ++i) wv[i] = frag(w2s, i % TN2, i / TN2);
            if (!last) {
#pragma unroll
                for (int i = 0; i < 4; ++i) wv[2 * TN2 + i] = frag(w1tile(0), i, 0);
            }
#pragma unroll
            for (int i = 0; i < 2 * TN2; ++i) {
                const int a2 = i % TN2;
                if (ABL == 4) { acc2[a2][0][0] += (float)wv[i][0] * (float)q0[1]; acc2[a2][1][1] += (float)wv[i][1] * (float)r1[0]; continue; }
                acc2[a2][0] = __builtin_amdgcn_mfma_f32_16x16x32_f16(wv[i], i < TN2 ? q0 : r0, acc2[a2][0], 0, 0, 0);
                acc2[a2][1] = __builtin_amdgcn_mfma_f32_16x16x32_f16(wv[i], i < TN2 ? q1 : r1, acc2[a2][1], 0, 0, 0);
            }
            __builtin_amdgcn_sched_group_barrier(0x100, 4, 0);
#pragma unroll
            for (int i = 0; i < 2 * TN2; ++i) {
                __builtin_amdgcn_sched_group_barrier(0x008, 2, 0);
                __builtin_amdgcn_sched_group_barrier(0x100, 1, 0);
            }
            if (!last) {
#pragma unroll
                for (int i = 0; i < 4; ++i) cur[i] = wv[2 * TN2 + i];
            }
        }
    }
    __builtin_amdgcn_sched_barrier(0);
    const int slab_of[1] = {-1};
    igemm_epilogue<64, C>(p.g, acc2, m_of, (C / 2) * wn, fq, 0, slab_of);
}

extern "C" int lcm_canonical_splits(int kind, int m_img, int N, int K, int aux, int ph);

extern "C" int lcm_mlp_geglu_f16(const void* x, int ldx, const void* W1, const void* ln_g, const void* ln_c, float eps,
                                 const void* W2, const void* b2, void* out, int ldo, int M, int C, int img_rows, void* stream) {
    LCM_REQUIRE(x && W1 && ln_g && ln_c && W2 && out, "mlp_geglu: null pointer");
    LCM_REQUIRE(M > 0, "mlp_geglu: bad M=%d", M);
    LCM_REQUIRE(C == 320, "mlp_geglu: C=%d (register budget of the kernel: C = 320 only)", C);
    LCM_REQUIRE(ldx % 8 == 0 && ldo % 4 == 0, "mlp_geglu: ldx=%d (%%8) / ldo=%d (%%4) misaligned", ldx, ldo);
    if (img_rows <= 0 || M % img_rows) img_rows = M;
    const int parts = lcm_canonical_splits(0, img_rows, C, 4 * C, 1, 0);
    LCM_REQUIRE(parts == 1, "mlp_geglu: the canonical K partition of ff.net.2 at %d rows per image has %d parts; the fused "
                "kernel accumulates one (use the two-launch form)", img_rows, parts);
    MlpParams p = {};
    p.X = (const half_t*)x; p.ldx = ldx; p.W1 = (const half_t*)W1; p.ln_g = (const float*)ln_g; p.ln_c = (const float*)ln_c;
    p.eps = eps; p.W2 = (const half_t*)W2;
    p.g.out = (half_t*)out; p.g.ldo = ldo; p.g.bias = (const half_t*)b2; p.g.res = (const half_t*)x; p.g.ldr = ldx;
    p.g.M = M; p.g.N = C; p.g.K = 4 * C; p.g.splits = 1; p.g.epi = 0; p.g.out_scale = 1.0f; p.g.rows_per_batch = 1;
    constexpr int smem = 5 * 128 * 128 + 320 * 128 + 2 * 8 * 320 * 4 + 16 * 1024;
    static LcmDevOnce attr_once;
    if (auto once_guard = attr_once.first()) {
        once_guard.check(hipFuncSetAttribute(reinterpret_cast<const void*>(&mlp_geglu_kernel<320>),
                                             hipFuncAttributeMaxDynamicSharedMemorySize, smem));
    }
    hipStream_t s = (hipStream_t)stream;
    lcm_prof_start("mlp_geglu_kernel<320>", s);
    static const int abl = getenv("LCM_MLP_ABLATE") ? atoi(getenv("LCM_MLP_ABLATE")) : 0;
    const dim3 grid((M + 127) / 128);
    if (abl) {
        auto set = [&](const void* f) { (void)hipFuncSetAttribute(f, hipFuncAttributeMaxDynamicSharedMemorySize, smem); };
        if (abl == 1) { set((const void*)&mlp_geglu_kernel<320, 1>); hipLaunchKernelGGL((mlp_geglu_kernel<320, 1>), grid, dim3(512), smem, s, p); }
        else if (abl == 2) { set((const void*)&mlp_geglu_kernel<320, 2>); hipLaunchKernelGGL((mlp_geglu_kernel<320, 2>), grid, dim3(512), smem, s, p); }
        else if (abl == 3) { set((const void*)&mlp_geglu_kernel<320, 3>); hipLaunchKernelGGL((mlp_geglu_kernel<320, 3>), grid, dim3(512), smem, s, p); }
        else { set((const void*)&mlp_geglu_kernel<320, 4>); hipLaunchKernelGGL((mlp_geglu_kernel<320, 4>), grid, dim3(512), smem, s, p); }
    } else
    hipLaunchKernelGGL((mlp_geglu_kernel<320>), grid, dim3(512), smem, s, p);
    lcm_prof_stop(s);
    LCM_CHECK_LAUNCH("mlp_geglu");
    return LCM_OK;
}
```

stable-diffusion-1.5-lcm-onnx-rknn2_amd/csrc/vae_enc.hip:

```cpp
#include "igemm_common.h"

__global__ __launch_bounds__(256) void vae_enc_conv_in_u8_kernel(const uint8_t* __restrict__ in, const half_t* __restrict__ W,
                                                                 const half_t* __restrict__ bias, half_t* __restrict__ out,
                                                                 int B, int H, int Wd, int Cout) {
#pragma clang fp contract(off)
    extern __shared__ __attribute__((aligned(16))) char smem[];
    for (int i = threadIdx.x; i < Cout * 8; i += 256) {
        const int sg = i / Cout, co = i - sg * Cout;
        half_t e[8];
#pragma unroll
        for (int j = 0; j < 8; ++j) {
            const int k = sg * 8 + j;
            e[j] = k < 54 ? W[co * 27 + (k >= 27 ? k - 27 : k)] : (half_t)0;
        }
        *reinterpret_cast<h8*>(smem + (sg * Cout + co) * 16) = (h8){e[0], e[1], e[2], e[3], e[4], e[5], e[6], e[7]};
    }
    __syncthreads();
    const int lane = threadIdx.x & 63, wave = threadIdx.x >> 6;
    const int n = lane & 15, q = lane >> 4;
    const long long npix = (long long)B * H * Wd;
    const int ntile = (int)((npix + 15) >> 4), plane = H * Wd;
    for (int t = blockIdx.x * 4 + wave; t < ntile; t += gridDim.x * 4) {
        const long long pix = (long long)t * 16 + n;
        const bool live = pix < npix;
// ... 171 lines not shown
    };

    f4 acc[TN][TM];
#pragma unroll
    for (int a = 0; a < TN; ++a)
#pragma unroll
        for (int b = 0; b < TM; ++b) acc[a][b] = (f4){0.f, 0.f, 0.f, 0.f};

    const int frow = lane & 15, fq = lane >> 4;
    load_tile(kt0);
    store_tile(0);
    __syncthreads();
    for (int kt = kt0; kt < kt1; ++kt) {
        const int cur = (kt - kt0) & 1;
        if (kt + 1 < kt1) load_tile(kt + 1);
        const char* xs = smem + cur * BUF + (wm * (BM / 2)) * 128;
        const char* ws = smem + cur * BUF + XBYTES + (wn * (BN / 2)) * 128;
#pragma unroll
        for (int kk = 0; kk < 2; ++kk) {
            h8 xf[TM], wf[TN];
            const int c = kk * 4 + fq;
#pragma unroll
            for (int b = 0; b < TM; ++b) {
                const int r = b * 16 + frow;
                xf[b] = *reinterpret_cast<const h8*>(xs + r * 128 + ((c ^ (r & 7)) << 4));
            }
#pragma unroll
            for (int a = 0; a < TN; ++a) {
                const int r = a * 16 + frow;
                wf[a] = *reinterpret_cast<const h8*>(ws + r * 128 + ((c ^ (r & 7)) << 4));
            }
#pragma unroll
            for (int a = 0; a < TN; ++a)
#pragma unroll
                for (int b = 0; b < TM; ++b)
                    acc[a][b] = __builtin_amdgcn_mfma_f32_16x16x32_f16(wf[a], xf[b], acc[a][b], 0, 0, 0);
        }
        if (kt + 1 < kt1) store_tile(cur ^ 1);
        __syncthreads();
    }

    int m_of[TM];
#pragma unroll
    for (int b = 0; b < TM; ++b) {
        const int m = m_base + wm * (BM / 2) + b * 16 + frow;
        m_of[b] = m < p.M ? m : -1;
    }
    int slab_of[BM / 64];
#pragma unroll
    for (int bp = 0; bp < BM / 64; ++bp) {
        const int r = m_base + wm * (BM / 2) + bp * 32;
        slab_of[bp] = r < p.M ? (r >> 5) : -1;
    }
    igemm_epilogue<BM, BN>(p, acc, m_of, n_base + wn * (BN / 2), fq, 0, slab_of);
}

template <int BM, int BN>
static int launch_conv_down(IgemmParams& p, hipStream_t s) {
    constexpr int smem = 2 * (BM + BN) * 128;
    static LcmDevOnce attr_once;
    if (auto once_guard = attr_once.first()) {
        once_guard.check(hipFuncSetAttribute(reinterpret_cast<const void*>(&conv_down_kernel<BM, BN>),
                                             hipFuncAttributeMaxDynamicSharedMemorySize, smem));
    }
    p.mtiles = (p.M + BM - 1) / BM;
    p.ntiles = p.N / BN;
    char nm[64];
    snprintf(nm, sizeof(nm), "conv_down_kernel<%d, %d>%s", BM, BN, p.splits > 1 ? " +splitk" : "");
    lcm_prof_start(nm, s);
    hipLaunchKernelGGL((conv_down_kernel<BM, BN>), dim3(p.mtiles * p.ntiles, p.splits, 1), dim3(256), smem, s, p);
    lcm_prof_stop(s);
    LCM_CHECK_LAUNCH("conv3x3_down");
    if (p.splits > 1) {
        lcm_launch_splitk_reduce(p, s);
        LCM_CHECK_LAUNCH("splitk_reduce");
    }
    return LCM_OK;
}

extern "C" int lcm_conv3x3_down_f16(const void* in, const void* W, const void* bias, void* out, int B, int Hin, int Win, int Cin,
                                    int Cout, void* stats_out, int64_t stats_bytes, int* slabs_per_image, void* stream) {
    LCM_REQUIRE(in && W && out, "conv3x3_down: null pointer");
    LCM_REQUIRE(B > 0 && Hin >= 2 && Win >= 2, "conv3x3_down: bad shape B=%d %dx%d (each side >= 2)", B, Hin, Win);
    LCM_REQUIRE(Cin % 64 == 0 && Cout % 64 == 0 && Cin > 0 && Cout > 0, "conv3x3_down: Cin=%d Cout=%d must be multiples of 64", Cin, Cout);
    LCM_REQUIRE((long long)B * Hin * Win < (1ll << 30), "conv3x3_down: input too large");
    LCM_REQUIRE(!stats_out || slabs_per_image, "conv3x3_down: stats_out needs slabs_per_image");
    hipStream_t s = (hipStream_t)stream;
    IgemmParams p = {};
    p.A = (const half_t*)in; p.W = (const half_t*)W; p.bias = (const half_t*)bias; p.out = (half_t*)out;
    p.Hin = Hin; p.Win = Win; p.Cin = Cin; p.stride = 2; p.ups = 0;
    p.Hout = (Hin + 1 - 3) / 2 + 1; p.Wout = (Win + 1 - 3) / 2 + 1;
    const int img_rows = p.Hout * p.Wout;
    p.M = B * img_rows; p.N = Cout; p.K = 9 * Cin;
    p.ldo = Cout; p.ldr = Cout; p.rows_per_batch = img_rows; p.img_rows = img_rows;
    p.epi = 0; p.out_scale = 1.0f; p.n_iters = 1; p.seg_parts = 1; p.rg_kind = 0;
    long long wsb = 0;
    p.ws = lcm_splitk_workspace(&wsb, s);
    p.splits = 1;
    if (p.ws) {
        const int sp = lcm_canonical_splits(1, img_rows, p.N, p.K, 1, 0);
        if (sp < 0) return sp;
        p.splits = sp;
    }
    if (p.splits > 1 && (long long)p.splits * p.M * p.N * 4 > wsb) {
        lcm_set_error("conv3x3_down: split-K workspace too small: %d x %d x %d fp32 slabs need %lld MB, have %lld MB "
                      "(lcm_set_workspace / LCM_SPLITK_WS_MB)", p.splits, p.M, p.N,
                      ((long long)p.splits * p.M * p.N * 4 + (1 << 20) - 1) >> 20, wsb >> 20);
// ... 16 lines not shown
```

stable-diffusion-1.5-lcm-onnx-rknn2_amd/lib.py:

```python
from __future__ import annotations

import ctypes as C
import os
import subprocess

_HERE = os.path.dirname(os.path.abspath(__file__))
LIB_PATH = os.path.join(_HERE, "liblcmhip.so")


class LcmHipError(RuntimeError):
    pass


def build(verbose: bool = False) -> str:
    r = subprocess.run(["make", "-C", os.path.join(_HERE, "csrc"), "-j8"], capture_output=True, text=True)
    if verbose or r.returncode != 0:
        print(r.stdout[-4000:], r.stderr[-4000:])
    if r.returncode != 0:
        raise LcmHipError("building liblcmhip.so failed")
    return LIB_PATH


_vp, _i, _f, _i64 = C.c_void_p, C.c_int, C.c_float, C.c_int64

# ... 29 lines not shown
    "lcm_conv3x3_down_f16": [_vp, _vp, _vp, _vp, _i, _i, _i, _i, _i, _vp, _i64, C.POINTER(_i), _vp],
    "lcm_vae_enc_conv_in_u8": [_vp, _vp, _vp, _vp, _i, _i, _i, _i, _vp],
    "lcm_vae_posterior_renoise": [_vp, _vp, _vp, _vp, _vp, _vp, _f, _f, _f, _vp, _vp, _vp, _i, _i, _i, _i, _vp],
    "lcm_scheduler_step_handover": [_vp, _vp, _f, _vp, _vp, _vp, C.POINTER(C.c_float), _f, _f, _i, _i, _i, _i, _i, _vp],
    "lcm_inpaint_mask_prepare": [_vp, _vp, _i, _vp, _vp, _vp, _i, _i, _i, _vp],
    "lcm_scheduler_step_inpaint": [_vp, _vp, _f, _vp, _vp, _vp, _vp, _vp, C.POINTER(C.c_float), _i, _f, _f, _i, _i, _i, _i, _i, _vp],
    "lcm_inpaint_composite_rgb8": [_vp, _vp, _vp, _i, _i, _i, _vp],
    "lcm_canny_classes_u8": [_vp, _vp, _i, _i, _i, _i, _i, _vp],
    "lcm_canny_link": [_vp, _vp, _vp, C.c_longlong, _i, _i, _i, _vp],
    "lcm_canny_rgb8": [_vp, _vp, _vp, C.c_longlong, _i, _i, _i, _f, _f, _vp],
    "lcm_invert_u8": [_vp, _vp, C.c_longlong, _vp],
    "lcm_resize_lanczos_u8": [_vp, C.c_longlong, _i, _i, _i, _i, _i, _i, _i, _i, _i, _vp, C.c_longlong, _vp, C.c_longlong, _vp],
    "lcm_resize_tables": [_i, _i, _i, _i, _vp, C.c_longlong],
    "lcm_resize_plan_tables": [_i] * 8 + [_vp, C.c_longlong],
    "lcm_resize_span": [_i, _i, _i, _i, C.POINTER(_i), C.POINTER(_i)],
    "lcm_resize_ksize": [_i, _i],
    "lcm_resize_passes": [_i, _i, _i, _i],
    "lcm_resize_max_span": [_i, _i, _i, _i, _i],
    "lcm_png_encode_rgb8": [_vp, _i, _i, C.c_longlong, _i, _vp, C.c_longlong, C.POINTER(C.c_longlong)],
    "lcm_stream_create": [C.POINTER(_vp)],
    "lcm_stream_destroy": [_vp],
    "lcm_graph_begin": [_vp],
    "lcm_graph_end": [_vp, C.POINTER(_vp)],
    "lcm_graph_launch": [_vp, _vp],
    "lcm_graph_destroy": [_vp],
    "lcm_gemm_tile_config": [_i, _i, _i],
    "lcm_debug_spin": [_i, _vp],
    "lcm_debug_grid_barrier": [_i, _i, _vp, _vp],
    "lcm_axpy_f16": [_vp, _vp, _f, _vp, _i64, _vp],
    "lcm_vae_blend_f32": [_vp, _i, _i, _vp, _i, _i, _i, _i, _i, _vp],
    "lcm_vae_place_tile": [_vp, _i, _i, _vp, _vp, _i, _i, _i, _i, _i, _i, _i, _vp],
    "lcm_profile_begin": [_i],
    "lcm_profile_end": [C.c_char_p, _i64],
    "lcm_set_workspace": [_vp, _i64],
    "lcm_set_stream_workspace": [_vp, _vp, _i64],
    "lcm_set_tuning": [_i, _i, _i],
    "lcm_set_split_policy": [_i, _i],
    "lcm_set_seg_mode": [_i],
    "lcm_set_attention_waves": [_i],
    "lcm_set_attention_impl": [_i],
    "lcm_set_attention_ksplit": [_i],
    "lcm_set_kernel_variant": [_i],
    "lcm_set_conv_impl": [_i],
    "lcm_set_persist_n": [_i],
    "lcm_set_halo_pipe_threshold": [_i],
    "lcm_set_halo_prefetch": [_i],
    "lcm_set_staged_epilogue": [_i],
    "lcm_set_gn_fused_bytes": [_i64],
    "lcm_plan_set": [_i] * 9,
    "lcm_plan_clear": [],
    "lcm_canonical_splits": [_i] * 6,
    "lcm_conv3x3_gn_f16": [_vp, _i, _vp, _i, _vp, _vp, _i, _vp, _vp, _vp, _i, _vp, _vp, _i, _i, _i, _i, _i, _vp, _i64,
                           C.POINTER(_i), _vp],
    "lcm_groupnorm_affine_f16": [_vp, _i, _vp, _i, _vp, _vp, _vp, _vp, _i, _i, _i, _f, _vp, _vp],
    "lcm_device_info": [_i, C.c_char_p, _i, C.POINTER(_i), C.POINTER(C.c_uint64)],
    "lcm_sr_conv1": [_vp, _i, _i, _i, _i, _i, _i, _vp, _vp, _vp, _vp],
    "lcm_sr_conv3x3": [_vp, _i, _i, _i, _i, _vp, _vp, _vp, _vp],
    "lcm_sr_conv4_shuffle": [_vp, _i, _i, _i, _i, _i, _i, _vp, _vp, _i, _vp, _vp],
    "lcm_sr_chroma_h": [_vp, _i, _i, _i, _vp, _vp],
    "lcm_sr_merge": [_vp, _vp, _i, _i, _i, _vp, _vp],
    "lcm_jpeg_quant_tables": [_i, _vp],
    "lcm_jpeg_dct_rgb8": [_vp, _i, _i, C.c_longlong, _i, _vp, C.c_longlong, _vp],
    "lcm_jpeg_encode_coefs": [_vp, _i, _i, _i, _i, _vp, C.c_longlong, C.POINTER(C.c_longlong)],
    "lcm_jpeg_dec_info": [_vp, C.c_longlong, _vp],
    "lcm_jpeg_dec_coefs": [_vp, C.c_longlong, _i, _vp, C.c_longlong],
    "lcm_jpeg_idct_rgb8": [_vp, C.c_longlong, _vp, _vp, C.c_longlong, _vp, C.c_longlong, _vp],
}
EXPORTS = tuple(sorted(list(_SIGS) + ["lcm_last_error", "lcm_version", "lcm_groupnorm_ws_bytes", "lcm_stats_bytes", "lcm_png_bound",
                              "lcm_canny_ws_bytes", "lcm_jpeg_coef_bytes", "lcm_jpeg_bound", "lcm_resize_ws_bytes",
                              "lcm_resize_table_bytes", "lcm_resize_plan_table_bytes"]))

EUNSUPPORTED = -3


class JpegInfo(C.Structure):
    _fields_ = [("width", _i), ("height", _i), ("ncomp", _i), ("sampling", _i), ("restart_interval", _i), ("mcus_x", _i),
                ("mcus_y", _i), ("blocks_per_mcu", _i), ("coefs_bytes", C.c_longlong), ("work_bytes", C.c_longlong),
                ("qt", C.c_uint8 * 192)]


_lib = None


def load():
    global _lib
    if _lib is not None:
        return _lib
    if not os.path.exists(LIB_PATH):
        raise LcmHipError(f"{LIB_PATH} not built: run __graft_entry__.build() (make -C csrc); "
                          "there is no CPU fallback for the HIP path")
    import torch
    lib = C.CDLL(LIB_PATH)
    for name, sig in _SIGS.items():
        fn = getattr(lib, name)
        fn.argtypes = sig
        fn.restype = _i
    lib.lcm_last_error.restype = C.c_char_p
    lib.lcm_last_error.argtypes = []
    lib.lcm_version.restype = _i
    lib.lcm_groupnorm_ws_bytes.restype = _i64
    lib.lcm_groupnorm_ws_bytes.argtypes = [_i, _i, _i, _i]
    lib.lcm_stats_bytes.restype = _i64
    lib.lcm_png_bound.restype = C.c_longlong
    lib.lcm_png_bound.argtypes = [_i, _i, _i]
    lib.lcm_stats_bytes.argtypes = [_i, _i, _i]
    lib.lcm_canny_ws_bytes.restype = C.c_longlong
# ... 53 lines not shown
```

stable-diffusion-1.5-lcm-onnx-rknn2_amd/model.py:

```python
from __future__ import annotations

import torch

from . import ops
from .config import TEXT_SEQ_LEN, depth_at, heads_at, unet_config, vae_config
from .packing import pack_conv1x1, pack_conv3x3, pack_conv3x3_up2, pack_ff2_cols, pack_geglu


import os

VAE_FLASH_ATTN = os.environ.get("LCM_VAE_FLASH_ATTN", "1") != "0"
FUSE_GN_MIN_BYTES = int(os.environ.get("LCM_FUSE_GN_MIN_BYTES", str(64 << 20)))


def _fuse_gn_into_conv(M, Cin, Cout):
    if Cin % 64 or Cout % 64:
        return False
    ntiles = Cout // 160 if Cout % 160 == 0 else -(-Cout // 128)
    return M * Cin * 2 >= FUSE_GN_MIN_BYTES and ntiles <= (4 if Cout % 160 == 0 else 3)


class _Buffers:
    def __init__(self, device):
        self.device = device
# ... 37 lines not shown
        st = self._stats.get(key)
        if st is None:
            st = ops.Stats(torch.zeros(ops.stats_floats(M, C, hw), dtype=torch.float32, device=self.device))
            self._stats[key] = st
        return st

    def norm(self, x, gamma, beta, out, B, HW, C1, *, x_st=None, x2=None, C2=0, x2_st=None, eps=1e-5, silu=True):
        C = C1 + C2
        ws = self.gn_ws(B, HW, C)
        if x_st is not None and x_st.P > 0 and (x2 is None or (x2_st is not None and x2_st.P > 0)):
            ops.groupnorm_from_stats(x, gamma, beta, out, B, HW, C1, x_st, ws, x2=x2, C2=C2, st2=x2_st, eps=eps, silu=silu)
        else:
            ops.groupnorm(x, gamma, beta, out, B, HW, C1, ws, x2=x2, C2=C2, eps=eps, silu=silu)
        return out

    def _norm_conv_out(self, x, norm, st, hn, out, B, H, W, ch, cout, eps, *, mode, out_f32=None):
        wt = self.w
        if st is not None and st.P > 0 and ch % 64 == 0:
            sc_t, sh_t = ops.groupnorm_tables_from_stats(wt[norm + ".g"], wt[norm + ".b"], B, H * W, ch, st, self.gn_ws(B, H * W, ch), eps=eps)
            ops.conv3x3_smalln(x, wt["conv_out.w"], out, B, H, W, ch, cout, bias=wt["conv_out.b"], mode=mode, out_f32=out_f32,
                               gn_scale=sc_t, gn_shift=sh_t, silu=True)
        else:
            self.norm(x, wt[norm + ".g"], wt[norm + ".b"], hn, B, H * W, ch, x_st=st, eps=eps)
            ops.conv3x3_smalln(hn, wt["conv_out.w"], out, B, H, W, ch, cout, bias=wt["conv_out.b"], mode=mode, out_f32=out_f32)

    def gn_ws(self, B, HW, C):
        key = ("gn_ws", B, HW, C)
        t = self._stats.get(key)
        if t is None:
            t = torch.empty(max(ops.groupnorm_ws_bytes(B, HW, C) // 4, 1024), dtype=torch.float32, device=self.device)
            self._stats[key] = t
        return t

    def weight_bytes(self):
        return sum(t.numel() * t.element_size() for t in self.w.values())

    def _pack_resnet(self, sd, p, temb_list=None):
        for n in ("norm1", "norm2"):
            self._put(f"{p}.{n}.g", sd[f"{p}.{n}.weight"])
            self._put(f"{p}.{n}.b", sd[f"{p}.{n}.bias"])
        for n in ("conv1", "conv2"):
            self._put(f"{p}.{n}.w", pack_conv3x3(sd[f"{p}.{n}.weight"]))
            self._put(f"{p}.{n}.b", sd[f"{p}.{n}.bias"])
        if f"{p}.conv_shortcut.weight" in sd:
            self._put(f"{p}.sc.w", pack_conv1x1(sd[f"{p}.conv_shortcut.weight"]))
            self._put(f"{p}.sc.b", sd[f"{p}.conv_shortcut.bias"])
        if temb_list is not None:
            temb_list.append((p, sd[f"{p}.time_emb_proj.weight"], sd[f"{p}.time_emb_proj.bias"]))

    def resnet(self, p, x, C1, Cout, B, H, W, eps, x2=None, C2=0, rowadd=None, out_role="res_out", x_st=None, x2_st=None):
        HW, M, Cin = H * W, B * H * W, C1 + C2
        w = self.w
        have1 = x_st is not None and x_st.P > 0 and (x2 is None or (x2_st is not None and x2_st.P > 0))
        sc = x
        if (p + ".sc.w") in w:
            sc = self.buf.get("shortcut", M, Cout)
            ops.gemm(x, w[p + ".sc.w"], sc, bias=w[p + ".sc.b"], a2=x2, img_rows=HW)
        h1 = self.buf.get("conv1", M, Cout)
        h1_st = self.stats("conv1", M, Cout, HW)
        if have1 and C1 % 64 == 0 and C2 % 64 == 0 and _fuse_gn_into_conv(M, Cin, Cout):
            sc_t, sh_t = ops.groupnorm_tables_from_stats(w[p + ".norm1.g"], w[p + ".norm1.b"], B, HW, C1, x_st, self.gn_ws(B, HW, Cin),
                                                         C2=C2, st2=x2_st if x2 is not None else None, eps=eps)
            ops.conv3x3_gn(x, w[p + ".conv1.w"], h1, B, H, W, C1, Cout, x2=x2, C2=C2, gn_scale=sc_t, gn_shift=sh_t, silu=True,
                           bias=w[p + ".conv1.b"], rowadd=rowadd, stats=h1_st)
        else:
            hn = self.buf.get("gn", M, Cin)
            self.norm(x, w[p + ".norm1.g"], w[p + ".norm1.b"], hn, B, HW, C1, x_st=x_st, x2=x2, C2=C2, x2_st=x2_st, eps=eps)
            ops.conv3x3(hn, w[p + ".conv1.w"], h1, B, H, W, Cin, Cout, bias=w[p + ".conv1.b"], rowadd=rowadd, stats=h1_st)
        out = self.buf.get(out_role, M, Cout)
        out_st = self.stats(out_role, M, Cout, HW)
        if h1_st.P > 0 and _fuse_gn_into_conv(M, Cout, Cout):
            sc_t, sh_t = ops.groupnorm_tables_from_stats(w[p + ".norm2.g"], w[p + ".norm2.b"], B, HW, Cout, h1_st,
                                                         self.gn_ws(B, HW, Cout), eps=eps)
            ops.conv3x3_gn(h1, w[p + ".conv2.w"], out, B, H, W, Cout, Cout, gn_scale=sc_t, gn_shift=sh_t, silu=True,
                           bias=w[p + ".conv2.b"], res=sc, stats=out_st)
        else:
            hn2 = self.buf.get("gn", M, Cout)
            self.norm(h1, w[p + ".norm2.g"], w[p + ".norm2.b"], hn2, B, HW, Cout, x_st=h1_st, eps=eps)
            ops.conv3x3(hn2, w[p + ".conv2.w"], out, B, H, W, Cout, Cout, bias=w[p + ".conv2.b"], res=sc, stats=out_st)
        return out, out_st


class _UNetEncoder(_Net):

    def _init_encoder(self, cfg):
        self.cfg = cfg
        boc = cfg["block_out_channels"]
        self.ctx_dim = cfg["cross_attention_dim"]
        self.temb_dim = boc[0] * 4
        self.qs = {}
        self.has_cond = bool(cfg.get("time_cond_proj_dim"))
        self.has_added = bool(cfg.get("addition_time_embed_dim"))

    def _pack_head(self, sd):
        self._put("conv_in.w", pack_conv3x3(sd["conv_in.weight"]))
        self._put("conv_in.b", sd["conv_in.bias"])
        for n in ("linear_1", "linear_2"):
            self._put(f"te.{n}.w", sd[f"time_embedding.{n}.weight"])
            self._put(f"te.{n}.b", sd[f"time_embedding.{n}.bias"])
        if self.has_cond:
            self._put("te.cond.w", sd["time_embedding.cond_proj.weight"])

    def _pack_down_mid(self, sd, temb_list, kv_list):
        cfg = self.cfg
        nb = len(cfg["block_out_channels"])
        for i in range(nb):
            for j in range(cfg["layers_per_block"]):
                self._pack_resnet(sd, f"down_blocks.{i}.resnets.{j}", temb_list)
                if cfg["down_attn"][i]:
                    self._pack_transformer(sd, f"down_blocks.{i}.attentions.{j}", kv_list, depth_at(cfg, i), heads_at(cfg, i))
            if i < nb - 1:
                p = f"down_blocks.{i}.downsamplers.0.conv"
                self._put(p + ".w", pack_conv3x3(sd[p + ".weight"]))
                self._put(p + ".b", sd[p + ".bias"])
        self._pack_resnet(sd, "mid_block.resnets.0", temb_list)
        self._pack_transformer(sd, "mid_block.attentions.0", kv_list, depth_at(cfg, nb - 1), heads_at(cfg, nb - 1))
        self._pack_resnet(sd, "mid_block.resnets.1", temb_list)

    def _pack_tables(self, temb_list, kv_list):
        self.temb_off, off = {}, 0
        for p, wt, bt in temb_list:
# ... 615 lines not shown
```

stable-diffusion-1.5-lcm-onnx-rknn2_amd/ops.py:

```python
from __future__ import annotations

import ctypes as C

import torch

from . import lib as _lib


def _p(t):
    return None if t is None else C.c_void_p(t.data_ptr())


def _stream():
    return C.c_void_p(torch.cuda.current_stream().cuda_stream)


import contextlib
import functools
import threading

_hooks = threading.local()


def _record_list():
# ... 138 lines not shown
        return False
    m_img = img_rows if img_rows and M % img_rows == 0 else M
    return canonical_splits(0, m_img, C, 4 * C, 1, 0) == 1


def mlp_geglu(x, w1, ln_g, ln_c, w2, b2, out, *, eps=1e-5, img_rows=0):
    L = _lib.load()
    M, Cc = x.shape
    F = w2.shape[1]
    RECORD = _record_list()
    if RECORD is not None:
        RECORD.append((None, None, lambda: mlp_geglu(x, w1, ln_g, ln_c, w2, b2, out, eps=eps, img_rows=img_rows)))
    with _Timed("mlp", 2.0 * M * (2 * F) * Cc + 2.0 * M * Cc * F, 2.0 * (2 * M * Cc + 2 * F * Cc + Cc * F)):
        rc = L.lcm_mlp_geglu_f16(_p(x), x.stride(0), _p(w1), _p(ln_g), _p(ln_c), float(eps), _p(w2), _p(b2), _p(out),
                                 out.stride(0), M, Cc, int(img_rows), _stream())
    _lib.check(rc, "lcm_mlp_geglu_f16")
    return out


def ln_fold_refresh(w, g_out, c_base=None, c_delta=None, alpha=0.0, c_out=None):
    _lib.check(_lib.load().lcm_ln_fold_refresh(_p(w), w.shape[0], w.shape[1], _p(c_base), _p(c_delta), float(alpha), _p(g_out),
                                               _p(c_out), _stream()), "lcm_ln_fold_refresh")


def conv3x3(x, w, out, B, H, W, Cin, Cout, *, bias=None, rowadd=None, res=None, stride=1, ups=0, stats=None, out_hw=None):
    L = _lib.load()
    sbuf, sbytes, sp = _stats_args(stats)
    Ho, Wo = ((2 * H, 2 * W) if ups else ((H + 1) // 2, (W + 1) // 2) if stride == 2 else (H, W))
    flags = ups
    if out_hw is not None and tuple(out_hw) != (Ho, Wo):
        if ups != 1 or out_hw[0] not in (2 * H, 2 * H - 1) or out_hw[1] not in (2 * W, 2 * W - 1):
            raise _lib.LcmHipError(f"conv3x3: output size {tuple(out_hw)} from {H}x{W} needs ups=1 (plain 3x3 weights) and 2n / 2n-1 "
                                   f"targets, got ups={ups}")
        flags = ups | (4 if out_hw[0] == 2 * H - 1 else 0) | (8 if out_hw[1] == 2 * W - 1 else 0)
        Ho, Wo = out_hw
    Mo = B * Ho * Wo
    taps = 4 if ups == 2 else 9
    RECORD = _record_list()
    if RECORD is not None:
        kw = dict(bias=bias, rowadd=rowadd, res=res, stride=stride, ups=ups, stats=stats, out_hw=out_hw)
        key = (1, Mo, Cout, 9 * Cin, 1) if stride == 2 else (2, Mo, Cout, taps * Cin, (Wo << 1))
        RECORD.append((key, dict(halo=stride == 1, W=(W if ups == 2 else Wo), phases=4 if ups == 2 else 1, m_img=Mo // B, splittable=True),
                       lambda: conv3x3(x, w, out, B, H, W, Cin, Cout, **kw)))
    with _Timed("conv3x3", 2.0 * Mo * Cout * taps * Cin, 2.0 * (B * H * W * Cin + 9 * Cin * Cout + Mo * Cout)):
        rc = L.lcm_conv3x3_f16(_p(x), _p(w), _p(bias), _p(rowadd), rowadd.stride(0) if rowadd is not None else 0,
                               _p(res), _p(out), B, H, W, Cin, Cout, stride, flags, sbuf, sbytes,
                               C.byref(sp) if sp is not None else None, _stream())
    if stats is not None:
        stats.P = sp.value
    _lib.check(rc, "lcm_conv3x3_f16")
    return out


def conv3x3_down(x, w, out, B, H, W, Cin, Cout, *, bias=None, stats=None):
    L = _lib.load()
    sbuf, sbytes, sp = _stats_args(stats)
    Ho, Wo = (H - 2) // 2 + 1, (W - 2) // 2 + 1
    Mo = B * Ho * Wo
    RECORD = _record_list()
    if RECORD is not None:
        RECORD.append(((1, Mo, Cout, 9 * Cin, 1), dict(halo=False, W=Wo, phases=1, m_img=Mo // B, splittable=True),
                       lambda: conv3x3_down(x, w, out, B, H, W, Cin, Cout, bias=bias, stats=stats)))
    with _Timed("conv3x3", 2.0 * Mo * Cout * 9 * Cin, 2.0 * (B * H * W * Cin + 9 * Cin * Cout + Mo * Cout)):
        rc = L.lcm_conv3x3_down_f16(_p(x), _p(w), _p(bias), _p(out), B, H, W, Cin, Cout, sbuf, sbytes,
                                    C.byref(sp) if sp is not None else None, _stream())
    if stats is not None:
        stats.P = sp.value
    _lib.check(rc, "lcm_conv3x3_down_f16")
    return out


def conv3x3_gn(x, w, out, B, H, W, C1, Cout, *, x2=None, C2=0, gn_scale=None, gn_shift=None, silu=True, bias=None,
               rowadd=None, res=None, ups=0, stats=None):
    L = _lib.load()
    sbuf, sbytes, sp = _stats_args(stats)
    Cin = C1 + (C2 if x2 is not None else 0)
    Ho, Wo = (2 * H, 2 * W) if ups else (H, W)
    Mo = B * Ho * Wo
    RECORD = _record_list()
    if RECORD is not None:
        kw = dict(x2=x2, C2=C2, gn_scale=gn_scale, gn_shift=gn_shift, silu=silu, bias=bias, rowadd=rowadd, res=res, ups=ups,
                  stats=stats)
        RECORD.append(((2, Mo, Cout, 9 * Cin, (Wo << 1) | (1 if gn_scale is not None else 0)),
                       dict(halo=True, W=Wo, m_img=Mo // B, splittable=True), lambda: conv3x3_gn(x, w, out, B, H, W, C1, Cout, **kw)))
    with _Timed("conv3x3", 2.0 * Mo * Cout * 9 * Cin, 2.0 * (B * H * W * Cin + 9 * Cin * Cout + Mo * Cout)):
        rc = L.lcm_conv3x3_gn_f16(_p(x), C1, _p(x2), C2 if x2 is not None else 0, _p(gn_scale), _p(gn_shift),
                                  1 if silu else 0, _p(w), _p(bias), _p(rowadd),
                                  rowadd.stride(0) if rowadd is not None else 0, _p(res), _p(out), B, H, W, Cout, ups,
                                  sbuf, sbytes, C.byref(sp) if sp is not None else None, _stream())
    if stats is not None:
        stats.P = sp.value
    _lib.check(rc, "lcm_conv3x3_gn_f16")
    return out


def groupnorm_affine(x, gamma, beta, scale, shift, B, HW, C1, ws, *, x2=None, C2=0, groups=32, eps=1e-5):
    L = _lib.load()
    rc = L.lcm_groupnorm_affine_f16(_p(x), C1, _p(x2), C2 if x2 is not None else 0, _p(gamma), _p(beta), _p(scale),
                                    _p(shift), B, HW, groups, float(eps), _p(ws), _stream())
    _lib.check(rc, "lcm_groupnorm_affine_f16")


def set_halo_pipe_threshold(wgs):
    _lib.check(_lib.load().lcm_set_halo_pipe_threshold(int(wgs)), "lcm_set_halo_pipe_threshold")


# ... 345 lines not shown


def acquire_stream(device):
    import torch
    dev = torch.device(device)
    idx = dev.index if dev.index is not None else torch.cuda.current_device()
    idle = _OWN_STREAMS.setdefault(idx, [])
    if idle:
        return idle.pop()
    L = _lib.load()
    out = C.c_void_p()
    with torch.cuda.device(idx):
        _lib.check(L.lcm_stream_create(C.byref(out)), "lcm_stream_create")
    return torch.cuda.ExternalStream(out.value, device=torch.device("cuda", idx))


def release_stream(stream):
    if stream is not None:
        _OWN_STREAMS.setdefault(stream.device.index, []).append(stream)


def set_tuning(target_wgs=0, max_splits=0, min_wgs=0):
    _lib.check(_lib.load().lcm_set_tuning(int(target_wgs), int(max_splits), int(min_wgs)), "lcm_set_tuning")


def set_split_policy(max_rows_per_image=4096, max_parts=8):
    _lib.check(_lib.load().lcm_set_split_policy(int(max_rows_per_image), int(max_parts)), "lcm_set_split_policy")


def set_attention_waves(waves):
    _lib.check(_lib.load().lcm_set_attention_waves(int(waves)), "lcm_set_attention_waves")


def set_attention_impl(impl):
    _lib.check(_lib.load().lcm_set_attention_impl(int(impl)), "lcm_set_attention_impl")


def set_attention_ksplit(on):
    _lib.check(_lib.load().lcm_set_attention_ksplit(int(on)), "lcm_set_attention_ksplit")


def set_seg_mode(mode):
    _lib.check(_lib.load().lcm_set_seg_mode(int(mode)), "lcm_set_seg_mode")


def set_gn_fused_bytes(n):
    _lib.check(_lib.load().lcm_set_gn_fused_bytes(int(n)), "lcm_set_gn_fused_bytes")


def set_kernel_variant(v):
    _lib.check(_lib.load().lcm_set_kernel_variant(int(v)), "lcm_set_kernel_variant")


def profile_begin(max_launches=1 << 17):
    _lib.check(_lib.load().lcm_profile_begin(int(max_launches)), "lcm_profile_begin")


def profile_end():
    buf = C.create_string_buffer(1 << 24)
    n = _lib.load().lcm_profile_end(buf, len(buf))
    if n < 0:
        _lib.check(n, "lcm_profile_end")
    out = []
    for line in buf.value.decode().splitlines():
        name, ms = line.rsplit("\t", 1)
        out.append((name, float(ms)))
    return out


def axpy(base, delta, alpha, out):
    _lib.check(_lib.load().lcm_axpy_f16(_p(base), _p(delta), float(alpha), _p(out), base.numel(), _stream()), "lcm_axpy_f16")
    return out


def vae_blend(a, ah, aw, b, bh, bw, B, extent, vertical):
    _lib.check(_lib.load().lcm_vae_blend_f32(_p(a), ah, aw, _p(b), bh, bw, B, extent, 1 if vertical else 0, _stream()), "lcm_vae_blend_f32")


def vae_place_tile(tile, th, tw, out_u8, out_f32, H, W, B, oy, ox, ch, cw):
    _lib.check(_lib.load().lcm_vae_place_tile(_p(tile), th, tw, _p(out_u8), _p(out_f32), H, W, B, oy, ox, ch, cw, _stream()),
               "lcm_vae_place_tile")


def set_staged_epilogue(on):
    _lib.check(_lib.load().lcm_set_staged_epilogue(int(on)), "lcm_set_staged_epilogue")


def debug_spin(usec):
    _lib.check(_lib.load().lcm_debug_spin(int(usec), _stream()), "lcm_debug_spin")


class Graph:

    def __init__(self):
        self._exec = C.c_void_p()

    def __enter__(self):
        _lib.check(_lib.load().lcm_graph_begin(_stream()), "lcm_graph_begin")
        return self

    def __exit__(self, et, ev, tb):
        rc = _lib.load().lcm_graph_end(_stream(), C.byref(self._exec))
        if et is None:
            _lib.check(rc, "lcm_graph_end")
        return False

    def launch(self):
        _lib.check(_lib.load().lcm_graph_launch(self._exec, _stream()), "lcm_graph_launch")

    def close(self):
        if self._exec:
            _lib.load().lcm_graph_destroy(self._exec)
            self._exec = C.c_void_p()
# ... 7 lines not shown
```

Baseline: 52.49 images/s.

## Co-launch resnet shortcut GEMM with conv1 in one grid

Adds a combined kernel that runs the ResNet shortcut 1x1 GEMM and the conv1 3x3 halo convolution in a single launch. Block indices split the grid between the two bodies, and the split-K workspace is shared, with a paired reduce when needed. The goal is to fill idle CUs, since both ops are small at batch 1, and to remove one launch. The risk is heterogeneous blocks with mismatched LDS and occupancy, and the combined kernel is only taken for a few tile forms and in the non-fused GN path.

```diff
diff --git a/include/lcm_hip.h b/include/lcm_hip.h
--- a/include/lcm_hip.h
+++ b/include/lcm_hip.h
@@ -73,6 +73,18 @@
 int lcm_set_halo_prefetch(int on);
 int lcm_set_staged_epilogue(int on);
 int lcm_set_conv_impl(int impl);
+
+int lcm_conv3x3_with_gemm_f16(const void* in, const void* W, const void* bias, const void* rowadd, int ld_rowadd,
+                              const void* res, void* out, int B, int Hin, int Win, int Cin, int Cout, int stride, int ups,
+                              void* stats_out, int64_t stats_bytes, int* slabs_per_image,
+                              const void* A, int lda, const void* A2, int lda2, int K1, const void* gW, const void* gbias,
+                              const void* growadd, int g_ld_rowadd, int g_rows_per_batch, const void* gres, int ldr,
+                              void* gout, int ldo, int M, int N, int K, int epilogue, float out_scale, int img_rows,
+                              void* g_stats_out, int64_t g_stats_bytes, int* g_slabs_per_image, int* form, void* stream);
+int lcm_set_colaunch(int on, int max_wgs);
+int lcm_colaunch_layout(int conv_tiles, int conv_splits, int64_t conv_rows, int conv_n, int gemm_tiles, int gemm_splits,
+                        int64_t gemm_rows, int gemm_n, int64_t ws_floats, int max_wgs, int* conv_blocks, int* grid,
+                        int64_t* gemm_ws_offset);
 
 int lcm_conv3x3_c4_f32in(const void* in, const void* pre_w, const void* pre_b, float in_scale,
                          const void* W, const void* bias, void* out, int B, int H, int Wd, int Cout, void* stream);
diff --git a/stable-diffusion-1.5-lcm-onnx-rknn2_amd/csrc/conv_halo.hip b/stable-diffusion-1.5-lcm-onnx-rknn2_amd/csrc/conv_halo.hip
--- a/stable-diffusion-1.5-lcm-onnx-rknn2_amd/csrc/conv_halo.hip
+++ b/stable-diffusion-1.5-lcm-onnx-rknn2_amd/csrc/conv_halo.hip
@@ -209,7 +209,7 @@
             return (y < IH && x < IW) ? (PH ? (bimg * hp.H + 2 * y + py) * hp.W + 2 * x + px : (bimg * hp.H + y) * hp.W + x) : -1;
         });
     } else {
-        igemm_epilogue<BM, BN>(p, acc, m_of, n_base + wn * (BN / 2), fq, 0, slab_of);
+        igemm_epilogue<BM, BN>(p, acc, m_of, n_base + wn * (BN / 2), fq, 0, blockIdx.y, slab_of);
     }
 }
 
@@ -219,7 +219,7 @@
 }
 
 template <int TH, int TW, int BN, int WS, int PH, int TPS, int SEG = 0, int EPI = 0>
-__global__ __launch_bounds__(256, 2) void conv_halo_pipe_kernel(HaloParams hp) {
+__device__ __forceinline__ void conv_halo_pipe_body(const HaloParams& hp, const int bid, const int split) {
     constexpr int NT = PH ? 4 : 9;
     constexpr int G = NT / TPS;
     static_assert(TPS == 1 || TPS == (PH ? 2 : 3), "taps per step: 1 or one kernel row");
@@ -236,7 +236,7 @@
     const int tid = threadIdx.x, lane = tid & 63;
     const int wave = __builtin_amdgcn_readfirstlane(tid >> 6);
     const int wm = wave & 1, wn = wave >> 1;
-    const int tile = xcd_remap(blockIdx.x, p.mtiles * p.ntiles);
+    const int tile = xcd_remap(bid, p.mtiles * p.ntiles);
     const int mt4 = tile / p.ntiles, nt = tile - mt4 * p.ntiles;
     const int phase = PH ? (mt4 & 3) : 0, mt = PH ? (mt4 >> 2) : mt4;
     const int py = phase >> 1, px = phase & 1;
@@ -275,8 +275,8 @@
         for (int b = 0; b < TM; ++b) acc[a][b] = (f4){0.f, 0.f, 0.f, 0.f};
 
     const int nchunks = p.Cin >> 6;
-    const int c_begin = (int)((long long)blockIdx.y * nchunks / p.splits);
-    const int c_end = (int)((long long)(blockIdx.y + 1) * nchunks / p.splits);
+    const int c_begin = (int)((long long)split * nchunks / p.splits);
+    const int c_end = (int)((long long)(split + 1) * nchunks / p.splits);
     const int T = (c_end - c_begin) * G;
 
     auto issue_halo = [&](int c64, int hb) {
@@ -430,8 +430,27 @@
         if constexpr (SEG) tile_epilogue_staged<BM, BN>(p, tot, m_of, n_base, wm, wn, fq, slab_of, smem, row_of);
         else tile_epilogue_staged<BM, BN>(p, acc, m_of, n_base, wm, wn, fq, slab_of, smem, row_of);
     } else {
-        if constexpr (SEG) igemm_epilogue<BM, BN>(p, tot, m_of, n_base + wn * (BN / 2), fq, 0, slab_of);
-        else igemm_epilogue<BM, BN>(p, acc, m_of, n_base + wn * (BN / 2), fq, 0, slab_of);
+        if constexpr (SEG) igemm_epilogue<BM, BN>(p, tot, m_of, n_base + wn * (BN / 2), fq, 0, split, slab_of);
+        else igemm_epilogue<BM, BN>(p, acc, m_of, n_base + wn * (BN / 2), fq, 0, split, slab_of);
+    }
+}
+
+template <int TH, int TW, int BN, int WS, int PH, int TPS, int SEG = 0, int EPI = 0>
+__global__ __launch_bounds__(256, 2) void conv_halo_pipe_kernel(HaloParams hp) {
+    conv_halo_pipe_body<TH, TW, BN, WS, PH, TPS, SEG, EPI>(hp, blockIdx.x, blockIdx.y);
+}
+
+template <int TH, int TW, int BN, int WS, int PH, int TPS>
+__global__ __launch_bounds__(256, 2) void conv_gemm_colaunch_kernel(HaloParams hp, IgemmParams gp, int conv_blocks) {
+    const int b = blockIdx.x;
+    if (b < conv_blocks) {
+        const int tiles = hp.g.mtiles * hp.g.ntiles;
+        const int split = b / tiles;
+        conv_halo_pipe_body<TH, TW, BN, WS, PH, TPS>(hp, b - split * tiles, split);
+    } else {
+        const int g = b - conv_blocks, tiles = gp.mtiles * gp.ntiles;
+        const int split = g / tiles;
+        igemm2_body<64, 64, 0, 4>(gp, g - split * tiles, split, 0);
     }
 }
 
@@ -576,7 +595,9 @@
 extern int g_staged_epi_gemm;
 extern "C" int lcm_set_staged_epilogue(int on) { g_staged_epi = (on & 1) ? 1 : 0; g_staged_epi_gemm = (on & 2) ? 1 : 0; return LCM_OK; }
 
-int lcm_conv_halo_launch(HaloParams& hp, int B, hipStream_t s, int* slabs_per_image) {
+struct HaloCfg { int th, tw, bn, force; bool ph, xf; long long ws_bytes; };
+
+static int halo_prepare(HaloParams& hp, int B, hipStream_t s, int* slabs_per_image, HaloCfg& cfg) {
     IgemmParams& p = hp.g;
     hp.staged_epi = g_staged_epi;
     const bool ph = p.ups == 2;
@@ -625,6 +646,13 @@
     }
     const bool xf = hp.gn_scale != nullptr;
     if (ph && xf) return 1;
+    cfg = HaloCfg{th, TW, bn, force, ph, xf, ws_bytes};
+    return 0;
+}
+
+static int halo_dispatch(HaloParams& hp, hipStream_t s, const HaloCfg& cfg) {
+    const int th = cfg.th, TW = cfg.tw, bn = cfg.bn, force = cfg.force;
+    const bool ph = cfg.ph, xf = cfg.xf;
 #define HALO_CASE(TH_, TW_, BN_)                                                           \
     if (th == TH_ && TW == TW_ && bn == BN_) {                                             \
         if (ph) launch_halo<TH_, TW_, BN_, 0, 1>(hp, s, force);                            \
@@ -634,6 +662,109 @@
     HALO_CASE(8, 16, 128) HALO_CASE(8, 16, 64) HALO_CASE(4, 16, 128) HALO_CASE(4, 16, 64)
     HALO_CASE(8, 8, 128) HALO_CASE(8, 8, 64) HALO_CASE(8, 16, 160) HALO_CASE(4, 16, 160) HALO_CASE(8, 8, 160) { return 1; }
 #undef HALO_CASE
-    if (p.splits > 1) lcm_launch_splitk_reduce(p, s);
     return 0;
 }
+
+int lcm_conv_halo_launch(HaloParams& hp, int B, hipStream_t s, int* slabs_per_image) {
+    HaloCfg cfg;
+    int rc = halo_prepare(hp, B, s, slabs_per_image, cfg);
+    if (rc != 0) return rc;
+    rc = halo_dispatch(hp, s, cfg);
+    if (rc != 0) return rc;
+    if (hp.g.splits > 1) lcm_launch_splitk_reduce(hp.g, s);
+    return 0;
+}
+
+extern void lcm_launch_splitk_reduce_pair(IgemmParams& a, IgemmParams& b, hipStream_t s);
+
+static int g_colaunch = -1;
+static int g_colaunch_max_wgs = 1024;
+extern "C" int lcm_set_colaunch(int on, int max_wgs) {
+    g_colaunch = on ? 1 : 0;
+    if (max_wgs > 0) g_colaunch_max_wgs = max_wgs;
+    return LCM_OK;
+}
+bool lcm_colaunch_enabled() {
+    if (g_colaunch < 0) {
+        const char* e = getenv("LCM_COLAUNCH");
+        g_colaunch = (e && e[0] == '0' && !e[1]) ? 0 : 1;
+    }
+    return g_colaunch == 1;
+}
+
+extern "C" int lcm_colaunch_layout(int conv_tiles, int conv_splits, int64_t conv_rows, int conv_n, int gemm_tiles, int gemm_splits,
+                                   int64_t gemm_rows, int gemm_n, int64_t ws_floats, int max_wgs, int* conv_blocks, int* grid,
+                                   int64_t* gemm_ws_offset) {
+    if (conv_tiles <= 0 || gemm_tiles <= 0 || conv_splits < 1 || gemm_splits < 1) return 0;
+    const long long cb = (long long)conv_tiles * conv_splits, gb = (long long)gemm_tiles * gemm_splits;
+    if (cb + gb > (max_wgs > 0 ? max_wgs : g_colaunch_max_wgs)) return 0;
+    const long long conv_ws = conv_splits > 1 ? (long long)conv_splits * conv_rows * conv_n : 0;
+    const long long gemm_ws = gemm_splits > 1 ? (long long)gemm_splits * gemm_rows * gemm_n : 0;
+    if (conv_ws + gemm_ws > ws_floats) return 0;
+    if (conv_blocks) *conv_blocks = (int)cb;
+    if (grid) *grid = (int)(cb + gb);
+    if (gemm_ws_offset) *gemm_ws_offset = conv_ws;
+    return 1;
+}
+
+template <int TH, int TW, int TPS>
+static void launch_colaunch(HaloParams& hp, IgemmParams& gp, int conv_blocks, int grid, hipStream_t s) {
+    constexpr int HROWS_PAD = ((TH + 2) * (TW + 2) + 7) / 8 * 8;
+    constexpr int conv_smem = 2 * HROWS_PAD * 128 + 3 * TPS * 64 * 128, gemm_smem = 4 * (64 + 64) * 128;
+    constexpr int smem = conv_smem > gemm_smem ? conv_smem : gemm_smem;
+    static_assert(smem <= 160 * 1024, "co-launch ring exceeds LDS");
+    static LcmDevOnce attr_once;
+    if (auto once_guard = attr_once.first()) {
+        once_guard.check(hipFuncSetAttribute(reinterpret_cast<const void*>(&conv_gemm_colaunch_kernel<TH, TW, 64, 3, 0, TPS>),
+                                  hipFuncAttributeMaxDynamicSharedMemorySize, smem));
+    }
+    char nm[96];
+    snprintf(nm, sizeof(nm), "conv_gemm_colaunch_kernel<%d, %d, 64, 3, 0, %d>%s", TH, TW, TPS, (hp.g.splits > 1 || gp.splits > 1) ? " +splitk" : "");
+    lcm_prof_start(nm, s);
+    hipLaunchKernelGGL((conv_gemm_colaunch_kernel<TH, TW, 64, 3, 0, TPS>), dim3(grid), dim3(256), smem, s, hp, gp, conv_blocks);
+    lcm_prof_stop(s);
+}
+
+int lcm_conv_gemm_colaunch(HaloParams& hp, int B, IgemmParams& gp, hipStream_t s, int* conv_slabs_per_image) {
+    HaloCfg cfg;
+    if (halo_prepare(hp, B, s, conv_slabs_per_image, cfg) != 0) return 0;
+    IgemmParams& p = hp.g;
+    if (cfg.ph || cfg.xf || p.seg_parts > 1 || cfg.bn != 64) return 0;
+    p.ntiles = p.N / 64;
+    hp.tiles_y = (hp.H + cfg.th - 1) / cfg.th;
+    hp.tiles_x = (hp.W + cfg.tw - 1) / cfg.tw;
+    const int conv_tiles = p.mtiles * p.ntiles;
+    int tps = 0;
+    if (cfg.force == 3) tps = 3;
+    else if (cfg.force != 1 && (cfg.force == 2 || (long long)conv_tiles * p.splits < g_halo_pipe_below)) tps = 1;
+    const int form = cfg.th * 10000 + cfg.tw * 100 + tps;
+    if (form != 81603 && form != 80803 && form != 81601 && form != 41603 && form != 41601 && form != 80801) return 0;
+    gp.mtiles = (gp.M + 63) / 64;
+    gp.ntiles = gp.N / 64;
+    gp.n_iters = 1;
+    int conv_blocks = 0, grid = 0;
+    int64_t off = 0;
+    if (!lcm_colaunch_layout(conv_tiles, p.splits, p.M, p.N, gp.mtiles * gp.ntiles, gp.splits, gp.M, gp.N, cfg.ws_bytes / 4, 0,
+                             &conv_blocks, &grid, &off)) return 0;
+    if (gp.splits > 1) gp.ws = p.ws + off;
+    switch (form) {
+        case 81603: launch_colaunch<8, 16, 3>(hp, gp, conv_blocks, grid, s); break;
+        case 80803: launch_colaunch<8, 8, 3>(hp, gp, conv_blocks, grid, s); break;
+        case 81601: launch_colaunch<8, 16, 1>(hp, gp, conv_blocks, grid, s); break;
+        case 41601: launch_colaunch<4, 16, 1>(hp, gp, conv_blocks, grid, s); break;
+        case 80801: launch_colaunch<8, 8, 1>(hp, gp, conv_blocks, grid, s); break;
+        default: launch_colaunch<4, 16, 3>(hp, gp, conv_blocks, grid, s); break;
+    }
+    hipError_t e = hipGetLastError();
+    if (e == hipSuccess) {
+        if (p.splits > 1 && gp.splits > 1) lcm_launch_splitk_reduce_pair(p, gp, s);
+        else if (p.splits > 1) lcm_launch_splitk_reduce(p, s);
+        else if (gp.splits > 1) lcm_launch_splitk_reduce(gp, s);
+        e = hipGetLastError();
+    }
+    if (e != hipSuccess) {
+        lcm_set_error("conv_gemm_colaunch: launch failed: %s", hipGetErrorString(e));
+        return LCM_EINVAL;
+    }
+    return 1;
+}
diff --git a/stable-diffusion-1.5-lcm-onnx-rknn2_amd/csrc/igemm.hip b/stable-diffusion-1.5-lcm-onnx-rknn2_amd/csrc/igemm.hip
--- a/stable-diffusion-1.5-lcm-onnx-rknn2_amd/csrc/igemm.hip
+++ b/stable-diffusion-1.5-lcm-onnx-rknn2_amd/csrc/igemm.hip
@@ -151,249 +151,15 @@
     }
     if constexpr (ln) {
         ln_finish<TM>(ln_s, ln_q, p.K, p.ln_eps);
-        igemm_epilogue<BM, BN>(p, acc, m_of, n_base + wn * (BN / 2), fq, z, slab_of, ln_s, ln_q);
+        igemm_epilogue<BM, BN>(p, acc, m_of, n_base + wn * (BN / 2), fq, z, blockIdx.y, slab_of, ln_s, ln_q);
     } else {
-        igemm_epilogue<BM, BN>(p, acc, m_of, n_base + wn * (BN / 2), fq, z, slab_of);
-    }
-}
-
-__device__ __attribute__((aligned(256))) half_t g_zero_page[128];
-
-template <int N>
-__device__ __forceinline__ void wait_vmcnt() {
-    asm volatile("s_waitcnt vmcnt(%0)" ::"n"(N) : "memory");
+        igemm_epilogue<BM, BN>(p, acc, m_of, n_base + wn * (BN / 2), fq, z, blockIdx.y, slab_of);
+    }
 }
 
 template <int BM, int BN, int MODE, int S, int LN = 0, int SEG = 0, int EPI = 0>
 __global__ __launch_bounds__(256, S == 1 ? (BM + BN < 256 ? 4 : 3) : 2) void igemm2_kernel(IgemmParams p) {
-    static_assert(!EPI || (MODE == 0 && !LN && !SEG && S * (BM + BN) * 128 >= BM * BN * 2), "staged epilogue: plain GEMM whose ring holds the tile");
-    static_assert(!SEG || (S >= 2 && !LN), "segmented accumulation: ring variants of the plain kernel");
-    constexpr int RA = BM / 32, RW = BN / 32;
-    constexpr int TM = BM / 32, TN = BN / 32;
-    constexpr int XBYTES = BM * 128, WBYTES = BN * 128, BUF = XBYTES + WBYTES;
-    constexpr int LPT = RA + RW;
-    extern __shared__ __attribute__((aligned(16))) char smem[];
-
-    const int tid = threadIdx.x, lane = tid & 63;
-    const int wave = __builtin_amdgcn_readfirstlane(tid >> 6);
-    const int wm = wave & 1, wn = wave >> 1;
-    const int ngroups = p.ntiles / p.n_iters;
-    const int tile = xcd_remap(blockIdx.x, p.mtiles * ngroups);
-    const int mt = tile / ngroups, nt0 = (tile - mt * ngroups) * p.n_iters;
-    const int m_base = mt * BM;
-    const int z = blockIdx.z;
-
-    const half_t* __restrict__ Ab = p.A + z * p.strideA;
-    const half_t* __restrict__ A2b = p.A2 ? p.A2 + z * p.strideA : nullptr;
-    const half_t* __restrict__ Wb = p.W + z * p.strideW;
-
-    const int pos = tid & 7, row0 = tid >> 3;
-    const int schunk = (pos ^ (row0 & 7)) * 8;
-
-    bool a_ok[RA];
-    long long a_off[RA];
-    int a_b[RA], a_y[RA], a_x[RA];
-#pragma unroll
-    for (int i = 0; i < RA; ++i) {
-        const int m = m_base + row0 + 32 * i;
-        a_ok[i] = m < p.M;
-        if (MODE == 0) {
-            a_off[i] = (long long)m;
-        } else {
-            const int hw = p.Hout * p.Wout;
-            const int b = m / hw, rem = m - b * hw;
-            const int oy = rem / p.Wout;
-            a_b[i] = b; a_y[i] = oy * p.stride - 1; a_x[i] = (rem - oy * p.Wout) * p.stride - 1;
-        }
-    }
-    const half_t* wptr = Wb + (long long)row0 * p.K + schunk;
-    const int nk_all = p.K >> 6;
-    const int kt0 = (int)((long long)blockIdx.y * nk_all / p.splits);
-    const int kt1 = (int)((long long)(blockIdx.y + 1) * nk_all / p.splits);
-    const int nkr = kt1 - kt0;
-    const int T = nkr * p.n_iters;
-
-    auto issue_tile = [&](int t, int buf) {
-        const int ni = t / nkr;
-        const int kt = kt0 + (t - ni * nkr);
-        const int n_base_i = (nt0 + ni) * BN;
-        char* xs = smem + buf * BUF + wave * 8 * 128;
-        char* ws = xs + XBYTES;
-        if (MODE == 0) {
-            const int k0 = kt << 6;
-            const bool second = (A2b != nullptr) && (k0 >= p.K1);
-            const half_t* base = second ? A2b : Ab;
-            const long long ld = second ? p.lda2 : p.lda;
-            const int kk = (second ? k0 - p.K1 : k0) + schunk;
-#pragma unroll
-            for (int i = 0; i < RA; ++i) {
-                const half_t* src = a_ok[i] ? base + a_off[i] * ld + kk : g_zero_page;
-                __builtin_amdgcn_global_load_lds((const __attribute__((address_space(1))) void*)src,
-                                                 (__attribute__((address_space(3))) void*)(xs + i * 32 * 128), 16, 0, 0);
-            }
-        } else {
-            const int cpt = p.Cin >> 6;
-            const int tap = kt / cpt;
-            const int c0 = ((kt - tap * cpt) << 6) + schunk;
-            const int dy = tap / 3, dx = tap - dy * 3;
-            const int Hl = p.ups ? p.Hin * 2 : p.Hin, Wl = p.ups ? p.Win * 2 : p.Win;
-#pragma unroll
-            for (int i = 0; i < RA; ++i) {
-                int iy = a_y[i] + dy, ix = a_x[i] + dx;
-                const bool ok = a_ok[i] && iy >= 0 && iy < Hl && ix >= 0 && ix < Wl;
-                if (p.ups) { iy >>= 1; ix >>= 1; }
-                const long long off = ((long long)(a_b[i] * p.Hin + iy) * p.Win + ix) * p.Cin + c0;
-                const half_t* src = ok ? Ab + off : g_zero_page;
-                __builtin_amdgcn_global_load_lds((const __attribute__((address_space(1))) void*)src,
-                                                 (__attribute__((address_space(3))) void*)(xs + i * 32 * 128), 16, 0, 0);
-            }
-        }
-#pragma unroll
-        for (int i = 0; i < RW; ++i) {
-            const half_t* src = wptr + (long long)(n_base_i + 32 * i) * p.K + (kt << 6);
-            __builtin_amdgcn_global_load_lds((const __attribute__((address_space(1))) void*)src,
-                                             (__attribute__((address_space(3))) void*)(ws + i * 32 * 128), 16, 0, 0);
-        }
-    };
-
-    f4 acc[TN][TM];
-#pragma unroll
-    for (int a = 0; a < TN; ++a)
-#pragma unroll
-        for (int b = 0; b < TM; ++b) acc[a][b] = (f4){0.f, 0.f, 0.f, 0.f};
-
-    const int frow = lane & 15, fq = lane >> 4;
-    constexpr bool ln = LN != 0;
-    float ln_s[TM], ln_q[TM];
-#pragma unroll
-    for (int b = 0; b < TM; ++b) { ln_s[b] = 0.f; ln_q[b] = 0.f; }
-
-#pragma unroll
-    for (int s = 0; s < S - 1; ++s)
-        if (s < T) issue_tile(s, s);
-    const __attribute__((address_space(3))) float* ln_lds = nullptr;
-    if constexpr (ln) {
-        float* t = reinterpret_cast<float*>(smem + S * BUF);
-        if (tid < BN) { t[tid] = p.ln_g[nt0 * BN + tid]; t[BN + tid] = p.ln_c[nt0 * BN + tid]; }
-        __syncthreads();
-        ln_lds = (const __attribute__((address_space(3))) float*)t;
-    }
-
-    f4 tot[SEG ? TN : 1][SEG ? TM : 1];
-    int part = 0, nkp = nkr;
-    if constexpr (SEG) {
-#pragma unroll
-        for (int a = 0; a < TN; ++a)
-#pragma unroll
-            for (int b = 0; b < TM; ++b) tot[a][b] = (f4){0.f, 0.f, 0.f, 0.f};
-        nkp = (int)((long long)nk_all / p.seg_parts);
-    }
-    int buf = 0, kstep = 0, ni_cur = 0;
-    for (int t = 0; t < T; ++t) {
-        const int newer = T - 1 - t;
-        if (S == 1) {
-            if (t > 0) __builtin_amdgcn_s_barrier();
-            issue_tile(t, 0);
-            wait_vmcnt<0>();
-            __builtin_amdgcn_s_barrier();
-        } else {
-            if (S >= 6 && newer >= 4) wait_vmcnt<(S >= 6 ? 4 : 0) * LPT>();
-            else if (S >= 5 && newer >= 3) wait_vmcnt<(S >= 5 ? 3 : 0) * LPT>();
-            else if (S >= 4 && newer >= 2) wait_vmcnt<(S >= 4 ? 2 : 0) * LPT>();
-            else if (S >= 3 && newer >= 1) wait_vmcnt<(S >= 3 ? 1 : 0) * LPT>();
-            else wait_vmcnt<0>();
-            __builtin_amdgcn_s_barrier();
-            if (t + S - 1 < T) issue_tile(t + S - 1, (buf + S - 1) % S);
-        }
-
-        const char* xs = smem + buf * BUF + (wm * (BM / 2)) * 128;
-        const char* ws = smem + buf * BUF + XBYTES + (wn * (BN / 2)) * 128;
-#pragma unroll
-        for (int kk = 0; kk < 2; ++kk) {
-            h8 xf[TM], wf[TN];
-            const int c = kk * 4 + fq;
-#pragma unroll
-            for (int b = 0; b < TM; ++b) {
-                const int r = b * 16 + frow;
-                xf[b] = *reinterpret_cast<const h8*>(xs + r * 128 + ((c ^ (r & 7)) << 4));
-            }
-#pragma unroll
-            for (int a = 0; a < TN; ++a) {
-                const int r = a * 16 + frow;
-                wf[a] = *reinterpret_cast<const h8*>(ws + r * 128 + ((c ^ (r & 7)) << 4));
-            }
-            if constexpr (ln) {
-#pragma unroll
-                for (int b = 0; b < TM; ++b) ln_accum(xf[b], ln_s[b], ln_q[b]);
-            }
-#pragma unroll
-            for (int a = 0; a < TN; ++a)
-#pragma unroll
-                for (int b = 0; b < TM; ++b)
-                    acc[a][b] = __builtin_amdgcn_mfma_f32_16x16x32_f16(wf[a], xf[b], acc[a][b], 0, 0, 0);
-        }
-        buf = (buf + 1 == S) ? 0 : buf + 1;
-        if constexpr (SEG) {
-            if (++kstep == nkp) {
-                kstep = 0;
-#pragma unroll
-                for (int a = 0; a < TN; ++a)
-#pragma unroll
-                    for (int b = 0; b < TM; ++b) {
-                        tot[a][b][0] += acc[a][b][0]; tot[a][b][1] += acc[a][b][1];
-                        tot[a][b][2] += acc[a][b][2]; tot[a][b][3] += acc[a][b][3];
-                        acc[a][b] = (f4){0.f, 0.f, 0.f, 0.f};
-                    }
-                ++part;
-                nkp = (int)((long long)(part + 1) * nk_all / p.seg_parts) - (int)((long long)part * nk_all / p.seg_parts);
-            }
-            continue;
-        }
-        if (++kstep == nkr) {
-            kstep = 0;
-            int m_of[TM];
-#pragma unroll
-            for (int b = 0; b < TM; ++b) {
-                const int m = m_base + wm * (BM / 2) + b * 16 + frow;
-                m_of[b] = m < p.M ? m : -1;
-            }
-            int slab_of[BM / 64];
-#pragma unroll
-            for (int bp = 0; bp < BM / 64; ++bp) {
-                const int r = m_base + wm * (BM / 2) + bp * 32;
-                slab_of[bp] = r < p.M ? (r >> 5) : -1;
-            }
-            if constexpr (ln) {
-                ln_finish<TM>(ln_s, ln_q, p.K, p.ln_eps);
-                igemm_epilogue<BM, BN, 0, (S >= 3)>(p, acc, m_of, (nt0 + ni_cur) * BN + wn * (BN / 2), fq, z, slab_of, ln_s, ln_q, ln_lds, nt0 * BN);
-            } else if constexpr (EPI != 0) {
-                tile_epilogue_staged<BM, BN>(p, acc, m_of, (nt0 + ni_cur) * BN, wm, wn, fq, slab_of, smem,
-                                             [&](int q) { return m_base + q < p.M ? m_base + q : -1; });
-            } else {
-                igemm_epilogue<BM, BN, 0, (S >= 3)>(p, acc, m_of, (nt0 + ni_cur) * BN + wn * (BN / 2), fq, z, slab_of);
-            }
-            ++ni_cur;
-#pragma unroll
-            for (int a = 0; a < TN; ++a)
-#pragma unroll
-                for (int b = 0; b < TM; ++b) acc[a][b] = (f4){0.f, 0.f, 0.f, 0.f};
-        }
-    }
-    if constexpr (SEG) {
-        int m_of[TM];
-#pragma unroll
-        for (int b = 0; b < TM; ++b) {
-            const int m = m_base + wm * (BM / 2) + b * 16 + frow;
-            m_of[b] = m < p.M ? m : -1;
-        }
-        int slab_of[BM / 64];
-#pragma unroll
-        for (int bp = 0; bp < BM / 64; ++bp) {
-            const int r = m_base + wm * (BM / 2) + bp * 32;
-            slab_of[bp] = r < p.M ? (r >> 5) : -1;
-        }
-        igemm_epilogue<BM, BN, 0, (S >= 3)>(p, tot, m_of, nt0 * BN + wn * (BN / 2), fq, z, slab_of);
-    }
+    igemm2_body<BM, BN, MODE, S, LN, SEG, EPI>(p, blockIdx.x, blockIdx.y, blockIdx.z);
 }
 
 __device__ __forceinline__ int reduce_pixel(const IgemmParams& p, int slab, int b, int l) {
@@ -415,10 +181,10 @@
 }
 
 #define RED_BATCH 8
-__global__ __launch_bounds__(256) void splitk_reduce_kernel(IgemmParams p, int total_slabs) {
+__device__ __forceinline__ void splitk_reduce_body(const IgemmParams& p, const int total_slabs, const int bid) {
 #pragma clang fp contract(off)
     const int lane = threadIdx.x & 63, ncg = p.N >> 4;
-    const long long wv = (long long)blockIdx.x * 4 + (threadIdx.x >> 6);
+    const long long wv = (long long)bid * 4 + (threadIdx.x >> 6);
     const int slab = (int)(wv / ncg), cg = (int)(wv - (long long)slab * ncg);
     if (slab >= total_slabs) return;
     const int l = lane & 15, fq = lane >> 4;
@@ -494,6 +260,14 @@
         }
     }
 }
+__global__ __launch_bounds__(256) void splitk_reduce_kernel(IgemmParams p, int total_slabs) {
+    splitk_reduce_body(p, total_slabs, blockIdx.x);
+}
+__global__ __launch_bounds__(256) void splitk_reduce_colaunch_kernel(IgemmParams a, int slabs_a, IgemmParams b, int slabs_b) {
+    const int blocks_a = (int)(((long long)slabs_a * (a.N >> 4) + 3) / 4);
+    if ((int)blockIdx.x < blocks_a) splitk_reduce_body(a, slabs_a, blockIdx.x);
+    else splitk_reduce_body(b, slabs_b, (int)blockIdx.x - blocks_a);
+}
 
 #include <map>
 #include <mutex>
@@ -549,6 +323,11 @@
     const int total = lcm_total_slabs(p);
     const long long waves = (long long)total * (p.N >> 4);
     hipLaunchKernelGGL(splitk_reduce_kernel, dim3((unsigned)((waves + 3) / 4)), dim3(256), 0, s, p, total);
+}
+void lcm_launch_splitk_reduce_pair(IgemmParams& a, IgemmParams& b, hipStream_t s) {
+    const int ta = lcm_total_slabs(a), tb = lcm_total_slabs(b);
+    const long long ba = ((long long)ta * (a.N >> 4) + 3) / 4, bb = ((long long)tb * (b.N >> 4) + 3) / 4;
+    hipLaunchKernelGGL(splitk_reduce_colaunch_kernel, dim3((unsigned)(ba + bb)), dim3(256), 0, s, a, ta, b, tb);
 }
 
 #include <tuple>
@@ -775,9 +554,11 @@
     return LCM_OK;
 }
 
+struct GemmPick { TilePick t; int splits, variant; long long wsb; };
+
 template <int MODE>
-static int launch_igemm(IgemmParams& p, int batch, hipStream_t s, int img_rows, bool allow_split, bool want_stats,
-                        int* slabs_per_image) {
+static int prepare_igemm(IgemmParams& p, int batch, hipStream_t s, int img_rows, bool allow_split, bool want_stats,
+                         int* slabs_per_image, GemmPick& pk) {
     long long wsb = 0;
     p.ws = lcm_splitk_workspace(&wsb, s);
     if (img_rows <= 0 || p.M % img_rows) img_rows = p.M;
@@ -813,6 +594,18 @@
                       ((long long)splits * p.M * p.N * 4 + (1 << 20) - 1) >> 20, wsb >> 20);
         return LCM_EINVAL;
     }
+    pk = GemmPick{t, splits, variant, wsb};
+    return LCM_OK;
+}
+
+template <int MODE>
+static int launch_igemm(IgemmParams& p, int batch, hipStream_t s, int img_rows, bool allow_split, bool want_stats,
+                        int* slabs_per_image) {
+    GemmPick pk;
+    const int prc = prepare_igemm<MODE>(p, batch, s, img_rows, allow_split, want_stats, slabs_per_image, pk);
+    if (prc != LCM_OK) return prc;
+    const TilePick t = pk.t;
+    const int splits = pk.splits, variant = pk.variant;
     const int code = t.bm * 1000 + t.bn;
     if constexpr (MODE == 0) if (p.ln_g) {
         switch (code) {
@@ -834,12 +627,12 @@
     }
 }
 
-extern "C" int lcm_gemm_f16(const void* A, int lda, const void* A2, int lda2, int K1,
-                            const void* W, const void* bias, const void* rowadd, int ld_rowadd, int rows_per_batch,
-                            const void* res, int ldr, void* out, int ldo,
-                            int M, int N, int K, int epilogue, float out_scale,
-                            int batch, int64_t strideA, int64_t strideW, int64_t strideO, int img_rows,
-                            void* stats_out, int64_t stats_bytes, int* slabs_per_image, void* stream) {
+static int gemm_fill(IgemmParams& p, const void* A, int lda, const void* A2, int lda2, int K1,
+                     const void* W, const void* bias, const void* rowadd, int ld_rowadd, int rows_per_batch,
+                     const void* res, int ldr, void* out, int ldo,
+                     int M, int N, int K, int epilogue, float out_scale,
+                     int batch, int64_t strideA, int64_t strideW, int64_t strideO,
+                     void* stats_out, int64_t stats_bytes, int* slabs_per_image) {
     LCM_REQUIRE(A && W && out, "gemm: null pointer");
     LCM_REQUIRE(M > 0 && N > 0 && K > 0 && batch > 0, "gemm: bad shape M=%d N=%d K=%d batch=%d", M, N, K, batch);
     LCM_REQUIRE(K % 64 == 0, "gemm: K=%d must be a multiple of 64", K);
@@ -850,7 +643,7 @@
     if (rowadd) LCM_REQUIRE(rows_per_batch > 0 && ld_rowadd % 4 == 0, "gemm: bad rowadd");
     LCM_REQUIRE(epilogue >= 0 && epilogue <= 3, "gemm: unknown epilogue %d", epilogue);
     if (epilogue == 1) LCM_REQUIRE(!rowadd && !res && !A2, "gemm: GEGLU epilogue takes bias only");
-    IgemmParams p = {};
+    p = IgemmParams{};
     p.A = (const half_t*)A; p.A2 = (const half_t*)A2; p.W = (const half_t*)W;
     p.bias = (const half_t*)bias; p.rowadd = (const half_t*)rowadd; p.res = (const half_t*)res;
     p.out = (half_t*)out;
@@ -860,6 +653,19 @@
     p.strideA = strideA; p.strideW = strideW; p.strideO = strideO;
     p.stats = (float*)stats_out; p.stats_cap = stats_bytes;
     LCM_REQUIRE(!stats_out || slabs_per_image, "gemm: stats_out needs slabs_per_image");
+    return LCM_OK;
+}
+
+extern "C" int lcm_gemm_f16(const void* A, int lda, const void* A2, int lda2, int K1,
+                            const void* W, const void* bias, const void* rowadd, int ld_rowadd, int rows_per_batch,
+                            const void* res, int ldr, void* out, int ldo,
+                            int M, int N, int K, int epilogue, float out_scale,
+                            int batch, int64_t strideA, int64_t strideW, int64_t strideO, int img_rows,
+                            void* stats_out, int64_t stats_bytes, int* slabs_per_image, void* stream) {
+    IgemmParams p;
+    const int frc = gemm_fill(p, A, lda, A2, lda2, K1, W, bias, rowadd, ld_rowadd, rows_per_batch, res, ldr, out, ldo, M, N, K,
+                              epilogue, out_scale, batch, strideA, strideW, strideO, stats_out, stats_bytes, slabs_per_image);
+    if (frc != LCM_OK) return frc;
     const bool allow_split = batch == 1 && strideA == 0 && strideW == 0 && strideO == 0;
     return launch_igemm<0>(p, batch, (hipStream_t)stream, img_rows, allow_split, stats_out != nullptr, slabs_per_image);
 }
@@ -898,10 +704,10 @@
 };
 int lcm_conv_halo_launch(HaloParams& hp, int B, hipStream_t s, int* slabs_per_image);
 
-extern "C" int lcm_conv3x3_gn_f16(const void* in, int C1, const void* in2, int C2, const void* gn_scale,
-                                  const void* gn_shift, int silu, const void* W, const void* bias, const void* rowadd,
-                                  int ld_rowadd, const void* res, void* out, int B, int Hin, int Win, int Cout, int ups,
-                                  void* stats_out, int64_t stats_bytes, int* slabs_per_image, void* stream) {
+static int conv_gn_fill(HaloParams& hp, const void* in, int C1, const void* in2, int C2, const void* gn_scale,
+                        const void* gn_shift, int silu, const void* W, const void* bias, const void* rowadd,
+                        int ld_rowadd, const void* res, void* out, int B, int Hin, int Win, int Cout, int ups,
+                        void* stats_out, int64_t stats_bytes, int* slabs_per_image) {
     LCM_REQUIRE(in && W && out, "conv3x3_gn: null pointer");
     if (!in2) C2 = 0;
     const int Cin = C1 + C2;
@@ -909,7 +715,7 @@
     LCM_REQUIRE(C1 % 64 == 0 && C2 % 64 == 0 && Cout % 64 == 0, "conv3x3_gn: C1=%d C2=%d Cout=%d must be multiples of 64", C1, C2, Cout);
     LCM_REQUIRE((gn_scale == nullptr) == (gn_shift == nullptr), "conv3x3_gn: scale/shift must come together");
     if (rowadd) LCM_REQUIRE(ld_rowadd % 4 == 0, "conv3x3_gn: ld_rowadd misaligned");
-    HaloParams hp = {};
+    hp = HaloParams{};
     IgemmParams& p = hp.g;
     p.A = (const half_t*)in; p.A2 = (const half_t*)in2; p.W = (const half_t*)W; p.bias = (const half_t*)bias;
     p.rowadd = (const half_t*)rowadd; p.res = (const half_t*)res; p.out = (half_t*)out;
@@ -927,10 +733,21 @@
     p.stats = (float*)stats_out; p.stats_cap = stats_bytes;
     LCM_REQUIRE(!stats_out || slabs_per_image, "conv3x3_gn: stats_out needs slabs_per_image");
     if (slabs_per_image) *slabs_per_image = 0;
+    return LCM_OK;
+}
+
+extern "C" int lcm_conv3x3_gn_f16(const void* in, int C1, const void* in2, int C2, const void* gn_scale,
+                                  const void* gn_shift, int silu, const void* W, const void* bias, const void* rowadd,
+                                  int ld_rowadd, const void* res, void* out, int B, int Hin, int Win, int Cout, int ups,
+                                  void* stats_out, int64_t stats_bytes, int* slabs_per_image, void* stream) {
+    HaloParams hp;
+    const int frc = conv_gn_fill(hp, in, C1, in2, C2, gn_scale, gn_shift, silu, W, bias, rowadd, ld_rowadd, res, out, B, Hin, Win,
+                                 Cout, ups, stats_out, stats_bytes, slabs_per_image);
+    if (frc != LCM_OK) return frc;
     const int hrc = lcm_conv_halo_launch(hp, B, (hipStream_t)stream, slabs_per_image);
     if (hrc < 0) return hrc;
     if (hrc != 0) {
-        lcm_set_error("conv3x3_gn: no tile configuration for B=%d %dx%d Cin=%d Cout=%d", B, hp.H, hp.W, Cin, Cout);
+        lcm_set_error("conv3x3_gn: no tile configuration for B=%d %dx%d Cin=%d Cout=%d", B, hp.H, hp.W, hp.g.Cin, Cout);
         return LCM_EINVAL;
     }
     LCM_CHECK_LAUNCH("conv_halo");
@@ -963,3 +780,40 @@
     LCM_REQUIRE(!stats_out || slabs_per_image, "conv3x3: stats_out needs slabs_per_image");
     return launch_igemm<1>(p, 1, (hipStream_t)stream, p.Hout * p.Wout, true, stats_out != nullptr, slabs_per_image);
 }
+
+int lcm_conv_gemm_colaunch(HaloParams& hp, int B, IgemmParams& gp, hipStream_t s, int* conv_slabs_per_image);
+bool lcm_colaunch_enabled();
+
+extern "C" int lcm_conv3x3_with_gemm_f16(const void* in, const void* W, const void* bias, const void* rowadd, int ld_rowadd,
+                                         const void* res, void* out, int B, int Hin, int Win, int Cin, int Cout, int stride, int ups,
+                                         void* stats_out, int64_t stats_bytes, int* slabs_per_image,
+                                         const void* gA, int lda, const void* gA2, int lda2, int K1, const void* gW, const void* gbias,
+                                         const void* growadd, int g_ld_rowadd, int g_rows_per_batch, const void* gres, int ldr,
+                                         void* gout, int ldo, int M, int N, int K, int epilogue, float out_scale, int img_rows,
+                                         void* g_stats_out, int64_t g_stats_bytes, int* g_slabs_per_image, int* form, void* stream) {
+    if (form) *form = 0;
+    if (lcm_colaunch_enabled() && g_conv_impl == 1 && stride == 1 && ups == 0 && epilogue == 0 && in && gA) {
+        HaloParams hp;
+        IgemmParams gp;
+        int crc = conv_gn_fill(hp, in, Cin, nullptr, 0, nullptr, nullptr, 0, W, bias, rowadd, ld_rowadd, res, out, B, Hin, Win, Cout, 0,
+                               stats_out, stats_bytes, slabs_per_image);
+        if (crc == LCM_OK) crc = gemm_fill(gp, gA, lda, gA2, lda2, K1, gW, gbias, growadd, g_ld_rowadd, g_rows_per_batch, gres, ldr, gout,
+                                           ldo, M, N, K, 0, out_scale, 1, 0, 0, 0, g_stats_out, g_stats_bytes, g_slabs_per_image);
+        if (crc != LCM_OK) return crc;
+        GemmPick pk;
+        crc = prepare_igemm<0>(gp, 1, (hipStream_t)stream, img_rows, true, g_stats_out != nullptr, g_slabs_per_image, pk);
+        if (crc == LCM_OK && gp.seg_parts == 1) {
+            gp.splits = pk.splits;
+            const int rc = lcm_conv_gemm_colaunch(hp, B, gp, (hipStream_t)stream, slabs_per_image);
+            if (rc < 0) return rc;
+            if (rc == 1) { if (form) *form = 1; return LCM_OK; }
+        }
+        if (slabs_per_image) *slabs_per_image = 0;
+        if (g_slabs_per_image) *g_slabs_per_image = 0;
+    }
+    const int grc = lcm_gemm_f16(gA, lda, gA2, lda2, K1, gW, gbias, growadd, g_ld_rowadd, g_rows_per_batch, gres, ldr, gout, ldo, M, N, K,
+                                 epilogue, out_scale, 1, 0, 0, 0, img_rows, g_stats_out, g_stats_bytes, g_slabs_per_image, stream);
+    if (grc != LCM_OK) return grc;
+    return lcm_conv3x3_f16(in, W, bias, rowadd, ld_rowadd, res, out, B, Hin, Win, Cin, Cout, stride, ups, stats_out, stats_bytes,
+                           slabs_per_image, stream);
+}
diff --git a/stable-diffusion-1.5-lcm-onnx-rknn2_amd/csrc/igemm_common.h b/stable-diffusion-1.5-lcm-onnx-rknn2_amd/csrc/igemm_common.h
--- a/stable-diffusion-1.5-lcm-onnx-rknn2_amd/csrc/igemm_common.h
+++ b/stable-diffusion-1.5-lcm-onnx-rknn2_amd/csrc/igemm_common.h
@@ -90,14 +90,14 @@
 
 template <int BM, int BN, int STAGED = 0, int BATCHED = 0>
 __device__ __forceinline__ void igemm_epilogue(const IgemmParams& p, f4 (&acc)[BN / 32][BM / 32], const int (&m_of)[BM / 32],
-                                               int n_wave, int fq, int z, const int (&slab_of)[BM / 64],
+                                               int n_wave, int fq, int z, int split, const int (&slab_of)[BM / 64],
                                                const float* ln_mu = nullptr, const float* ln_r = nullptr,
                                                const __attribute__((address_space(3))) float* ln_lds = nullptr, int n_tile0 = 0,
                                                char* stage = nullptr, int q_wave = 0, int nl_wave = 0) {
 #pragma clang fp contract(off)
     constexpr int TM = BM / 32, TN = BN / 32;
     if (p.splits > 1) {
-        float* __restrict__ wsb = p.ws + (long long)blockIdx.y * p.M * p.N;
+        float* __restrict__ wsb = p.ws + (long long)split * p.M * p.N;
 #pragma unroll
         for (int b = 0; b < TM; ++b) {
             const int m = m_of[b];
@@ -283,7 +283,7 @@
         }
         __syncthreads();
     }
-    igemm_epilogue<BM, BN, 1>(p, acc, m_of, n_base + wn * (BN / 2), fq, 0, slab_of, nullptr, nullptr, nullptr, 0,
+    igemm_epilogue<BM, BN, 1>(p, acc, m_of, n_base + wn * (BN / 2), fq, 0, 0, slab_of, nullptr, nullptr, nullptr, 0,
                               stage, wm * (BM / 2), wn * (BN / 2));
     __syncthreads();
 #pragma unroll
@@ -297,3 +297,241 @@
         }
     }
 }
+
+static __device__ __attribute__((aligned(256))) half_t g_zero_page[128];
+
+template <int N>
+__device__ __forceinline__ void wait_vmcnt() {
+    asm volatile("s_waitcnt vmcnt(%0)" ::"n"(N) : "memory");
+}
+
+template <int BM, int BN, int MODE, int S, int LN = 0, int SEG = 0, int EPI = 0>
+__device__ __forceinline__ void igemm2_body(const IgemmParams& p, const int bid, const int split, const int z) {
+    static_assert(!EPI || (MODE == 0 && !LN && !SEG && S * (BM + BN) * 128 >= BM * BN * 2), "staged epilogue: plain GEMM whose ring holds the tile");
+    static_assert(!SEG || (S >= 2 && !LN), "segmented accumulation: ring variants of the plain kernel");
+    constexpr int RA = BM / 32, RW = BN / 32;
+    constexpr int TM = BM / 32, TN = BN / 32;
+    constexpr int XBYTES = BM * 128, WBYTES = BN * 128, BUF = XBYTES + WBYTES;
+    constexpr int LPT = RA + RW;
+    extern __shared__ __attribute__((aligned(16))) char smem[];
+
+    const int tid = threadIdx.x, lane = tid & 63;
+    const int wave = __builtin_amdgcn_readfirstlane(tid >> 6);
+    const int wm = wave & 1, wn = wave >> 1;
+    const int ngroups = p.ntiles / p.n_iters;
+    const int tile = xcd_remap(bid, p.mtiles * ngroups);
+    const int mt = tile / ngroups, nt0 = (tile - mt * ngroups) * p.n_iters;
+    const int m_base = mt * BM;
+
+    const half_t* __restrict__ Ab = p.A + z * p.strideA;
+    const half_t* __restrict__ A2b = p.A2 ? p.A2 + z * p.strideA : nullptr;
+    const half_t* __restrict__ Wb = p.W + z * p.strideW;
+
+    const int pos = tid & 7, row0 = tid >> 3;
+    const int schunk = (pos ^ (row0 & 7)) * 8;
+
+    bool a_ok[RA];
+    long long a_off[RA];
+    int a_b[RA], a_y[RA], a_x[RA];
+#pragma unroll
+    for (int i = 0; i < RA; ++i) {
+        const int m = m_base + row0 + 32 * i;
+        a_ok[i] = m < p.M;
+        if (MODE == 0) {
+            a_off[i] = (long long)m;
+        } else {
+            const int hw = p.Hout * p.Wout;
+            const int b = m / hw, rem = m - b * hw;
+            const int oy = rem / p.Wout;
+            a_b[i] = b; a_y[i] = oy * p.stride - 1; a_x[i] = (rem - oy * p.Wout) * p.stride - 1;
+        }
+    }
+    const half_t* wptr = Wb + (long long)row0 * p.K + schunk;
+    const int nk_all = p.K >> 6;
+    const int kt0 = (int)((long long)split * nk_all / p.splits);
+    const int kt1 = (int)((long long)(split + 1) * nk_all / p.splits);
+    const int nkr = kt1 - kt0;
+    const int T = nkr * p.n_iters;
+
+    auto issue_tile = [&](int t, int buf) {
+        const int ni = t / nkr;
+        const int kt = kt0 + (t - ni * nkr);
+        const int n_base_i = (nt0 + ni) * BN;
+        char* xs = smem + buf * BUF + wave * 8 * 128;
+        char* ws = xs + XBYTES;
+        if (MODE == 0) {
+            const int k0 = kt << 6;
+            const bool second = (A2b != nullptr) && (k0 >= p.K1);
+            const half_t* base = second ? A2b : Ab;
+            const long long ld = second ? p.lda2 : p.lda;
+            const int kk = (second ? k0 - p.K1 : k0) + schunk;
+#pragma unroll
+            for (int i = 0; i < RA; ++i) {
+                const half_t* src = a_ok[i] ? base + a_off[i] * ld + kk : g_zero_page;
+                __builtin_amdgcn_global_load_lds((const __attribute__((address_space(1))) void*)src,
+                                                 (__attribute__((address_space(3))) void*)(xs + i * 32 * 128), 16, 0, 0);
+            }
+        } else {
+            const int cpt = p.Cin >> 6;
+            const int tap = kt / cpt;
+            const int c0 = ((kt - tap * cpt) << 6) + schunk;
+            const int dy = tap / 3, dx = tap - dy * 3;
+            const int Hl = p.ups ? p.Hin * 2 : p.Hin, Wl = p.ups ? p.Win * 2 : p.Win;
+#pragma unroll
+            for (int i = 0; i < RA; ++i) {
+                int iy = a_y[i] + dy, ix = a_x[i] + dx;
+                const bool ok = a_ok[i] && iy >= 0 && iy < Hl && ix >= 0 && ix < Wl;
+                if (p.ups) { iy >>= 1; ix >>= 1; }
+                const long long off = ((long long)(a_b[i] * p.Hin + iy) * p.Win + ix) * p.Cin + c0;
+                const half_t* src = ok ? Ab + off : g_zero_page;
+                __builtin_amdgcn_global_load_lds((const __attribute__((address_space(1))) void*)src,
+                                                 (__attribute__((address_space(3))) void*)(xs + i * 32 * 128), 16, 0, 0);
+            }
+        }
+#pragma unroll
+        for (int i = 0; i < RW; ++i) {
+            const half_t* src = wptr + (long long)(n_base_i + 32 * i) * p.K + (kt << 6);
+            __builtin_amdgcn_global_load_lds((const __attribute__((address_space(1))) void*)src,
+                                             (__attribute__((address_space(3))) void*)(ws + i * 32 * 128), 16, 0, 0);
+        }
+    };
+
+    f4 acc[TN][TM];
+#pragma unroll
+    for (int a = 0; a < TN; ++a)
+#pragma unroll
+        for (int b = 0; b < TM; ++b) acc[a][b] = (f4){0.f, 0.f, 0.f, 0.f};
+
+    const int frow = lane & 15, fq = lane >> 4;
+    constexpr bool ln = LN != 0;
+    float ln_s[TM], ln_q[TM];
+#pragma unroll
+    for (int b = 0; b < TM; ++b) { ln_s[b] = 0.f; ln_q[b] = 0.f; }
+
+#pragma unroll
+    for (int s = 0; s < S - 1; ++s)
+        if (s < T) issue_tile(s, s);
+    const __attribute__((address_space(3))) float* ln_lds = nullptr;
+    if constexpr (ln) {
+        float* t = reinterpret_cast<float*>(smem + S * BUF);
+        if (tid < BN) { t[tid] = p.ln_g[nt0 * BN + tid]; t[BN + tid] = p.ln_c[nt0 * BN + tid]; }
+        __syncthreads();
+        ln_lds = (const __attribute__((address_space(3))) float*)t;
+    }
+
+    f4 tot[SEG ? TN : 1][SEG ? TM : 1];
+    int part = 0, nkp = nkr;
+    if constexpr (SEG) {
+#pragma unroll
+        for (int a = 0; a < TN; ++a)
+#pragma unroll
+            for (int b = 0; b < TM; ++b) tot[a][b] = (f4){0.f, 0.f, 0.f, 0.f};
+        nkp = (int)((long long)nk_all / p.seg_parts);
+    }
+    int buf = 0, kstep = 0, ni_cur = 0;
+    for (int t = 0; t < T; ++t) {
+        const int newer = T - 1 - t;
+        if (S == 1) {
+            if (t > 0) __builtin_amdgcn_s_barrier();
+            issue_tile(t, 0);
+            wait_vmcnt<0>();
+            __builtin_amdgcn_s_barrier();
+        } else {
+            if (S >= 6 && newer >= 4) wait_vmcnt<(S >= 6 ? 4 : 0) * LPT>();
+            else if (S >= 5 && newer >= 3) wait_vmcnt<(S >= 5 ? 3 : 0) * LPT>();
+            else if (S >= 4 && newer >= 2) wait_vmcnt<(S >= 4 ? 2 : 0) * LPT>();
+            else if (S >= 3 && newer >= 1) wait_vmcnt<(S >= 3 ? 1 : 0) * LPT>();
+            else wait_vmcnt<0>();
+            __builtin_amdgcn_s_barrier();
+            if (t + S - 1 < T) issue_tile(t + S - 1, (buf + S - 1) % S);
+        }
+
+        const char* xs = smem + buf * BUF + (wm * (BM / 2)) * 128;
+        const char* ws = smem + buf * BUF + XBYTES + (wn * (BN / 2)) * 128;
+#pragma unroll
+        for (int kk = 0; kk < 2; ++kk) {
+            h8 xf[TM], wf[TN];
+            const int c = kk * 4 + fq;
+#pragma unroll
+            for (int b = 0; b < TM; ++b) {
+                const int r = b * 16 + frow;
+                xf[b] = *reinterpret_cast<const h8*>(xs + r * 128 + ((c ^ (r & 7)) << 4));
+            }
+#pragma unroll
+            for (int a = 0; a < TN; ++a) {
+                const int r = a * 16 + frow;
+                wf[a] = *reinterpret_cast<const h8*>(ws + r * 128 + ((c ^ (r & 7)) << 4));
+            }
+            if constexpr (ln) {
+#pragma unroll
+                for (int b = 0; b < TM; ++b) ln_accum(xf[b], ln_s[b], ln_q[b]);
+            }
+#pragma unroll
+            for (int a = 0; a < TN; ++a)
+#pragma unroll
+                for (int b = 0; b < TM; ++b)
+                    acc[a][b] = __builtin_amdgcn_mfma_f32_16x16x32_f16(wf[a], xf[b], acc[a][b], 0, 0, 0);
+        }
+        buf = (buf + 1 == S) ? 0 : buf + 1;
+        if constexpr (SEG) {
+            if (++kstep == nkp) {
+                kstep = 0;
+#pragma unroll
+                for (int a = 0; a < TN; ++a)
+#pragma unroll
+                    for (int b = 0; b < TM; ++b) {
+                        tot[a][b][0] += acc[a][b][0]; tot[a][b][1] += acc[a][b][1];
+                        tot[a][b][2] += acc[a][b][2]; tot[a][b][3] += acc[a][b][3];
+                        acc[a][b] = (f4){0.f, 0.f, 0.f, 0.f};
+                    }
+                ++part;
+                nkp = (int)((long long)(part + 1) * nk_all / p.seg_parts) - (int)((long long)part * nk_all / p.seg_parts);
+            }
+            continue;
+        }
+        if (++kstep == nkr) {
+            kstep = 0;
+            int m_of[TM];
+#pragma unroll
+            for (int b = 0; b < TM; ++b) {
+                const int m = m_base + wm * (BM / 2) + b * 16 + frow;
+                m_of[b] = m < p.M ? m : -1;
+            }
+            int slab_of[BM / 64];
+#pragma unroll
+            for (int bp = 0; bp < BM / 64; ++bp) {
+                const int r = m_base + wm * (BM / 2) + bp * 32;
+                slab_of[bp] = r < p.M ? (r >> 5) : -1;
+            }
+            if constexpr (ln) {
+                ln_finish<TM>(ln_s, ln_q, p.K, p.ln_eps);
+                igemm_epilogue<BM, BN, 0, (S >= 3)>(p, acc, m_of, (nt0 + ni_cur) * BN + wn * (BN / 2), fq, z, split, slab_of, ln_s, ln_q, ln_lds, nt0 * BN);
+            } else if constexpr (EPI != 0) {
+                tile_epilogue_staged<BM, BN>(p, acc, m_of, (nt0 + ni_cur) * BN, wm, wn, fq, slab_of, smem,
+                                             [&](int q) { return m_base + q < p.M ? m_base + q : -1; });
+            } else {
+                igemm_epilogue<BM, BN, 0, (S >= 3)>(p, acc, m_of, (nt0 + ni_cur) * BN + wn * (BN / 2), fq, z, split, slab_of);
+            }
+            ++ni_cur;
+#pragma unroll
+            for (int a = 0; a < TN; ++a)
+#pragma unroll
+                for (int b = 0; b < TM; ++b) acc[a][b] = (f4){0.f, 0.f, 0.f, 0.f};
+        }
+    }
+    if constexpr (SEG) {
+        int m_of[TM];
+#pragma unroll
+        for (int b = 0; b < TM; ++b) {
+            const int m = m_base + wm * (BM / 2) + b * 16 + frow;
+            m_of[b] = m < p.M ? m : -1;
+        }
+        int slab_of[BM / 64];
+#pragma unroll
+        for (int bp = 0; bp < BM / 64; ++bp) {
+            const int r = m_base + wm * (BM / 2) + bp * 32;
+            slab_of[bp] = r < p.M ? (r >> 5) : -1;
+        }
+        igemm_epilogue<BM, BN, 0, (S >= 3)>(p, tot, m_of, nt0 * BN + wn * (BN / 2), fq, z, split, slab_of);
+    }
+}
diff --git a/stable-diffusion-1.5-lcm-onnx-rknn2_amd/csrc/mlp_fused.hip b/stable-diffusion-1.5-lcm-onnx-rknn2_amd/csrc/mlp_fused.hip
--- a/stable-diffusion-1.5-lcm-onnx-rknn2_amd/csrc/mlp_fused.hip
+++ b/stable-diffusion-1.5-lcm-onnx-rknn2_amd/csrc/mlp_fused.hip
@@ -217,7 +217,7 @@
     }
     __builtin_amdgcn_sched_barrier(0);
     const int slab_of[1] = {-1};
-    igemm_epilogue<64, C>(p.g, acc2, m_of, (C / 2) * wn, fq, 0, slab_of);
+    igemm_epilogue<64, C>(p.g, acc2, m_of, (C / 2) * wn, fq, 0, 0, slab_of);
 }
 
 extern "C" int lcm_canonical_splits(int kind, int m_img, int N, int K, int aux, int ph);
diff --git a/stable-diffusion-1.5-lcm-onnx-rknn2_amd/csrc/vae_enc.hip b/stable-diffusion-1.5-lcm-onnx-rknn2_amd/csrc/vae_enc.hip
--- a/stable-diffusion-1.5-lcm-onnx-rknn2_amd/csrc/vae_enc.hip
+++ b/stable-diffusion-1.5-lcm-onnx-rknn2_amd/csrc/vae_enc.hip
@@ -247,7 +247,7 @@
         const int r = m_base + wm * (BM / 2) + bp * 32;
         slab_of[bp] = r < p.M ? (r >> 5) : -1;
     }
-    igemm_epilogue<BM, BN>(p, acc, m_of, n_base + wn * (BN / 2), fq, 0, slab_of);
+    igemm_epilogue<BM, BN>(p, acc, m_of, n_base + wn * (BN / 2), fq, 0, blockIdx.y, slab_of);
 }
 
 template <int BM, int BN>
diff --git a/stable-diffusion-1.5-lcm-onnx-rknn2_amd/lib.py b/stable-diffusion-1.5-lcm-onnx-rknn2_amd/lib.py
--- a/stable-diffusion-1.5-lcm-onnx-rknn2_amd/lib.py
+++ b/stable-diffusion-1.5-lcm-onnx-rknn2_amd/lib.py
@@ -105,6 +105,11 @@
     "lcm_canonical_splits": [_i] * 6,
     "lcm_conv3x3_gn_f16": [_vp, _i, _vp, _i, _vp, _vp, _i, _vp, _vp, _vp, _i, _vp, _vp, _i, _i, _i, _i, _i, _vp, _i64,
                            C.POINTER(_i), _vp],
+    "lcm_conv3x3_with_gemm_f16": [_vp, _vp, _vp, _vp, _i, _vp, _vp, _i, _i, _i, _i, _i, _i, _i, _vp, _i64, C.POINTER(_i),
+                                  _vp, _i, _vp, _i, _i, _vp, _vp, _vp, _i, _i, _vp, _i, _vp, _i, _i, _i, _i, _i, _f, _i,
+                                  _vp, _i64, C.POINTER(_i), C.POINTER(_i), _vp],
+    "lcm_set_colaunch": [_i, _i],
+    "lcm_colaunch_layout": [_i, _i, _i64, _i, _i, _i, _i64, _i, _i64, _i, C.POINTER(_i), C.POINTER(_i), C.POINTER(_i64)],
     "lcm_groupnorm_affine_f16": [_vp, _i, _vp, _i, _vp, _vp, _vp, _vp, _i, _i, _i, _f, _vp, _vp],
     "lcm_device_info": [_i, C.c_char_p, _i, C.POINTER(_i), C.POINTER(C.c_uint64)],
     "lcm_sr_conv1": [_vp, _i, _i, _i, _i, _i, _i, _vp, _vp, _vp, _vp],
diff --git a/stable-diffusion-1.5-lcm-onnx-rknn2_amd/model.py b/stable-diffusion-1.5-lcm-onnx-rknn2_amd/model.py
--- a/stable-diffusion-1.5-lcm-onnx-rknn2_amd/model.py
+++ b/stable-diffusion-1.5-lcm-onnx-rknn2_amd/model.py
@@ -113,13 +113,16 @@
         HW, M, Cin = H * W, B * H * W, C1 + C2
         w = self.w
         have1 = x_st is not None and x_st.P > 0 and (x2 is None or (x2_st is not None and x2_st.P > 0))
+        has_sc = (p + ".sc.w") in w
+        fused1 = have1 and C1 % 64 == 0 and C2 % 64 == 0 and _fuse_gn_into_conv(M, Cin, Cout)
         sc = x
-        if (p + ".sc.w") in w:
+        if has_sc:
             sc = self.buf.get("shortcut", M, Cout)
-            ops.gemm(x, w[p + ".sc.w"], sc, bias=w[p + ".sc.b"], a2=x2, img_rows=HW)
+            if fused1:
+                ops.gemm(x, w[p + ".sc.w"], sc, bias=w[p + ".sc.b"], a2=x2, img_rows=HW)
         h1 = self.buf.get("conv1", M, Cout)
         h1_st = self.stats("conv1", M, Cout, HW)
-        if have1 and C1 % 64 == 0 and C2 % 64 == 0 and _fuse_gn_into_conv(M, Cin, Cout):
+        if fused1:
             sc_t, sh_t = ops.groupnorm_tables_from_stats(w[p + ".norm1.g"], w[p + ".norm1.b"], B, HW, C1, x_st, self.gn_ws(B, HW, Cin),
                                                          C2=C2, st2=x2_st if x2 is not None else None, eps=eps)
             ops.conv3x3_gn(x, w[p + ".conv1.w"], h1, B, H, W, C1, Cout, x2=x2, C2=C2, gn_scale=sc_t, gn_shift=sh_t, silu=True,
@@ -127,7 +130,11 @@
         else:
             hn = self.buf.get("gn", M, Cin)
             self.norm(x, w[p + ".norm1.g"], w[p + ".norm1.b"], hn, B, HW, C1, x_st=x_st, x2=x2, C2=C2, x2_st=x2_st, eps=eps)
-            ops.conv3x3(hn, w[p + ".conv1.w"], h1, B, H, W, Cin, Cout, bias=w[p + ".conv1.b"], rowadd=rowadd, stats=h1_st)
+            if has_sc:
+                ops.conv3x3_with_gemm(hn, w[p + ".conv1.w"], h1, B, H, W, Cin, Cout, bias=w[p + ".conv1.b"], rowadd=rowadd, stats=h1_st,
+                                      g_a=x, g_w=w[p + ".sc.w"], g_out=sc, g_bias=w[p + ".sc.b"], g_a2=x2, g_img_rows=HW)
+            else:
+                ops.conv3x3(hn, w[p + ".conv1.w"], h1, B, H, W, Cin, Cout, bias=w[p + ".conv1.b"], rowadd=rowadd, stats=h1_st)
         out = self.buf.get(out_role, M, Cout)
         out_st = self.stats(out_role, M, Cout, HW)
         if h1_st.P > 0 and _fuse_gn_into_conv(M, Cout, Cout):
diff --git a/stable-diffusion-1.5-lcm-onnx-rknn2_amd/ops.py b/stable-diffusion-1.5-lcm-onnx-rknn2_amd/ops.py
--- a/stable-diffusion-1.5-lcm-onnx-rknn2_amd/ops.py
+++ b/stable-diffusion-1.5-lcm-onnx-rknn2_amd/ops.py
@@ -214,6 +214,41 @@
     return out
 
 
+PAIR_SEPARATE, PAIR_COLAUNCHED = 0, 1
+
+
+def conv3x3_with_gemm(x, w, out, B, H, W, Cin, Cout, *, bias=None, rowadd=None, res=None, stats=None,
+                      g_a, g_w, g_out, g_bias=None, g_a2=None, g_stats=None, g_img_rows=0):
+    if _record_list() is not None or _profile_list() is not None or _brackets_on:
+        gemm(g_a, g_w, g_out, bias=g_bias, a2=g_a2, stats=g_stats, img_rows=g_img_rows)
+        conv3x3(x, w, out, B, H, W, Cin, Cout, bias=bias, rowadd=rowadd, res=res, stats=stats)
+        return PAIR_SEPARATE
+    L = _lib.load()
+    sbuf, sbytes, sp = _stats_args(stats)
+    gsbuf, gsbytes, gsp = _stats_args(g_stats)
+    M, N = g_a.shape[0], g_w.shape[0]
+    K1 = g_a.shape[-1] if g_a2 is not None else 0
+    K = g_a.shape[-1] + (g_a2.shape[-1] if g_a2 is not None else 0)
+    form = C.c_int(0)
+    rc = L.lcm_conv3x3_with_gemm_f16(_p(x), _p(w), _p(bias), _p(rowadd), rowadd.stride(0) if rowadd is not None else 0,
+                                     _p(res), _p(out), B, H, W, Cin, Cout, 1, 0, sbuf, sbytes,
+                                     C.byref(sp) if sp is not None else None,
+                                     _p(g_a), g_a.stride(-2), _p(g_a2), g_a2.stride(0) if g_a2 is not None else 0, K1, _p(g_w),
+                                     _p(g_bias), None, 0, 0, None, 0, _p(g_out), g_out.stride(-2), M, N, K, 0, 1.0,
+                                     int(g_img_rows), gsbuf, gsbytes, C.byref(gsp) if gsp is not None else None,
+                                     C.byref(form), _stream())
+    if stats is not None:
+        stats.P = sp.value
+    if g_stats is not None:
+        g_stats.P = gsp.value
+    _lib.check(rc, "lcm_conv3x3_with_gemm_f16")
+    return form.value
+
+
+def set_colaunch(on, max_wgs=0):
+    _lib.check(_lib.load().lcm_set_colaunch(1 if on else 0, int(max_wgs)), "lcm_set_colaunch")
+
+
 def conv3x3_down(x, w, out, B, H, W, Cin, Cout, *, bias=None, stats=None):
     L = _lib.load()
     sbuf, sbytes, sp = _stats_args(stats)
@@ -665,13 +700,20 @@
     _lib.check(_lib.load().lcm_set_kernel_variant(int(v)), "lcm_set_kernel_variant")
 
 
+_brackets_on = False
+
+
 def profile_begin(max_launches=1 << 17):
+    global _brackets_on
     _lib.check(_lib.load().lcm_profile_begin(int(max_launches)), "lcm_profile_begin")
+    _brackets_on = True
 
 
 def profile_end():
+    global _brackets_on
     buf = C.create_string_buffer(1 << 24)
     n = _lib.load().lcm_profile_end(buf, len(buf))
+    _brackets_on = False
     if n < 0:
         _lib.check(n, "lcm_profile_end")
     out = []
```

Measured after the change: 52.96 images/s (median of 6 runs). About the same (+0.9%).
